# datatypevoid/babble

Hardware: AMD Instinct MI355X
Metric: consensus-ordered events/sec at N=256 peers (1 GPU and 8-GPU batched sims) (higher is better)
Workload: dtype int32

## Files before the change

### babble_amd/_lib.py

```python
from __future__ import annotations

import ctypes as C
import os

import numpy as np

HERE = os.path.dirname(os.path.abspath(__file__))
LIB_PATH = os.path.join(HERE, os.environ.get("HGX_LIB", "libhgx.so"))

_L = None


class HgxError(RuntimeError):

    def __init__(self, code: int, msg: str):
        super().__init__(msg)
        self.code = code
        self.msg = msg


class hgx_error(C.Structure):
    _fields_ = [("code", C.c_int32), ("msg", C.c_char * 252)]


# ... 86 lines not shown
    _sig(L, "hgx_destroy", None, [p])
    _sig(L, "hgx_insert_events", i32, [p, C.POINTER(hgx_events), i64, C.POINTER(C.c_int64), E])
    _sig(L, "hgx_insert_events_device", i32, [p, C.POINTER(hgx_events), i64, C.POINTER(C.c_int64), E])
    _sig(L, "hgx_insert_and_run", i32, [p, C.POINTER(hgx_events), i64, C.POINTER(C.c_int64), E])
    for nm in ("hgx_insert_events32", "hgx_insert_and_run32"):
        _sig(L, nm, i32, [p, C.POINTER(hgx_events32), i64, C.POINTER(C.c_int64), E])
    for nm in ("hgx_insert_events_packed", "hgx_insert_and_run_packed"):
        _sig(L, nm, i32, [p, C.POINTER(hgx_events_packed), i64, C.POINTER(C.c_int64), E])
    _sig(L, "hgx_pack_events32", i32, [C.POINTER(hgx_events32), i64, i64, p, p, p, p, p, p, i64,
                                       C.POINTER(C.c_int64), E])
    _sig(L, "hgx_host_alloc", p, [i64])
    _sig(L, "hgx_host_free", None, [p])
    _sig(L, "hgx_set_participant_keys", i32, [p, p, E])
    for nm in ("hgx_insert_events_verified", "hgx_insert_events_verified_device"):
        _sig(L, nm, i32, [p, C.POINTER(hgx_events), p, p, i64, C.POINTER(C.c_int64), E])
    _sig(L, "hgx_insert_event_bodies", i32, [p, C.POINTER(hgx_event_bodies), i64, p, C.POINTER(C.c_int64), E])
    _sig(L, "hgx_insert_event_bodies_ext", i32, [p, C.POINTER(hgx_event_bodies), p, i64, p, C.POINTER(C.c_int64), E])
    _sig(L, "hgx_event_json_batch", i32, [i32, C.POINTER(hgx_event_bodies), i64, p, i32, p, p, p, i64, p, E])
    _sig(L, "hgx_batch_levels", i32, [p, p, i64, i64, p, C.POINTER(C.c_int32), E])
    _sig(L, "hgx_reset_consensus", i32, [p])
    _sig(L, "hgx_save", i32, [p, C.c_char_p, E])
    _sig(L, "hgx_save_ex", i32, [p, C.c_char_p, p, p, E])
    _sig(L, "hgx_get_event_id", i32, [p, i64, p, E])
    _sig(L, "hgx_get_event_payload", i32, [p, i64, p, i64, C.POINTER(C.c_int64), E])
    _sig(L, "hgx_checksum", u64, [p, i64])
    _sig(L, "hgx_bootstrap", i32, [p, C.c_char_p, E])
    _sig(L, "hgx_clear", i32, [p])
    for nm in ("hgx_divide_rounds", "hgx_decide_fame", "hgx_find_order", "hgx_run_consensus"):
        _sig(L, nm, i32, [p, E])
    _sig(L, "hgx_num_events", i64, [p])
    _sig(L, "hgx_super_majority", i32, [p])
    _sig(L, "hgx_num_undetermined", i64, [p, i32])
    _sig(L, "hgx_undecided_rounds", i32, [p, i32, p, i32])
    _sig(L, "hgx_last_consensus_round", i32, [p, i32, C.POINTER(C.c_int32)])
    _sig(L, "hgx_last_commited_round_events", i32, [p, i32])
    _sig(L, "hgx_consensus_transactions", i64, [p, i32])
    _sig(L, "hgx_pending_loaded_events", i64, [p, i32])
    _sig(L, "hgx_last_round", i32, [p, i32])
    _sig(L, "hgx_round_event_count", i32, [p, i32, i32])
    _sig(L, "hgx_round_witnesses", i32, [p, i32, i32, p, i32])
    _sig(L, "hgx_known", i32, [p, i32, p])
    _sig(L, "hgx_consensus_events_count", i64, [p, i32])
    _sig(L, "hgx_consensus_events", i32, [p, i32, i64, i64, p])
    _sig(L, "hgx_num_blocks", i64, [p, i32])
    _sig(L, "hgx_block_info", i32, [p, i32, i64, p, p, p, p, p, p])
    _sig(L, "hgx_get_block", i32, [p, i32, i32, p, E])
    _sig(L, "hgx_consensus_received", i32, [p, i32, i64, i64, p, p, p])
    _sig(L, "hgx_last_from", i32, [p, i32, p, p, E])
    _sig(L, "hgx_participant_events", i32, [p, i32, i64, p, i64, p, E])
    _sig(L, "hgx_participant_event", i32, [p, i32, i64, p, E])
    _sig(L, "hgx_get_root", i32, [p, i32, p, p, p, p, E])
    _sig(L, "hgx_get_event", i32, [p, i64, p, p, p, p, p, p, p, E])
    _sig(L, "hgx_wire_info", i32, [p, i64, i64, p, p, p])
    _sig(L, "hgx_read_wire_info", i32, [p, i32, i64, i32, i64, p, p, E])
    _sig(L, "hgx_diff_wire", i32, [p, i32, p, i64, p, i64, C.POINTER(C.c_int64), C.POINTER(C.c_int32), E])
    _sig(L, "hgx_get_rounds", i32, [p, i64, i64, p, p, p])
    _sig(L, "hgx_get_received", i32, [p, i64, i64, p, p])
    _sig(L, "hgx_get_coords", i32, [p, i64, p, p])
    for nm in ("hgx_ancestor", "hgx_self_ancestor", "hgx_see", "hgx_strongly_see", "hgx_round", "hgx_witness"):
        _sig(L, nm, i32, [p, i64, i64] if nm not in ("hgx_round", "hgx_witness") else [p, i64])
    _sig(L, "hgx_oldest_self_ancestor_to_see", i64, [p, i64, i64])
    _sig(L, "hgx_block_hash", i32, [i64, i32, p, p, i32, p])
    _sig(L, "hgx_sha256_batch", i32, [i32, p, p, i64, p, p])
    _sig(L, "hgx_sha256_batch_device", i32, [p, p, i64, p, p])
    _sig(L, "hgx_p256_verify_batch", i32, [i32, p, i32, p, p, p, p, i64, p, p])
    _sig(L, "hgx_p256_verify_bench", i32, [i32, p, i32, p, p, p, p, i64, i32, i32, p, C.POINTER(C.c_double)])
    _sig(L, "hgx_sha256_bench", i32, [i32, i64, i32, i32, C.c_uint64, i32, i32, C.POINTER(C.c_double),
                                      C.POINTER(C.c_int64), C.POINTER(C.c_int64), i64, p])
    _sig(L, "hgx_phase_times", i32, [p, p, i32])
    _sig(L, "hgx_kernel_stats", i32, [p, i32, C.c_char_p, i32, C.POINTER(C.c_double), C.POINTER(C.c_int64),
                                      C.POINTER(C.c_double)])
    _sig(L, "hgx_reset_stats", i32, [p])
    _sig(L, "hgx_set_kernel_timing", i32, [p, i32])
    _sig(L, "hgx_set_coord_storage", i32, [p, i32])
    _sig(L, "hgx_set_fame_tally", i32, [p, i32])
    _sig(L, "hgx_set_round_kernel", i32, [p, i32])
    _sig(L, "hgx_set_sort_kernel", i32, [p, i32])
    _sig(L, "hgx_set_round_shards", i32, [p, i32])
    _sig(L, "hgx_set_shard_remote", i32, [p, i32])
    _sig(L, "hgx_exchange_floor_bench", i32, [i32, i32, i32, i32, C.POINTER(C.c_double)])
    _sig(L, "hgx_set_cts_kernel", i32, [p, i32])
    _sig(L, "hgx_set_root_others", i32, [p, p, i64, p])
    _sig(L, "hgx_set_la_kernel", i32, [p, i32])
    _sig(L, "hgx_set_incremental", i32, [p, i32])
    _sig(L, "hgx_find_order_begin", i32, [p, p])
    _sig(L, "hgx_find_order_end", i32, [p, p])
    _sig(L, "hgx_set_shard", i32, [p, i32, i32])
    _sig(L, "hgx_reset", i32, [p, p, p, p, p])
    _sig(L, "hgx_insert_wire_events", i32, [p, p, i64, p, p])
    _sig(L, "hgx_set_commit_callback", i32, [p, C.c_void_p, p])
    _sig(L, "hgx_get_frame", i32, [p, p, i64, p, p, p, p, p, p, p, i64, p, p])
    _sig(L, "hgx_prune_to_frame", i32, [p, p, i64, C.POINTER(C.c_int64), E])
    _sig(L, "hgx_get_root_ids", i32, [p, i32, p, C.POINTER(C.c_int32), p, C.POINTER(C.c_int32), E])
    _sig(L, "hgx_get_root_others", i32, [p, p, p, i64, C.POINTER(C.c_int64), E])
    _sig(L, "hgx_set_root_ids", i32, [p, p, p, p, p, p, p, i64, E])
    _sig(L, "hgx_shard_values", i64, [p, i32])
    _sig(L, "hgx_shard_export", i32, [p, p, i32])
    _sig(L, "hgx_shard_import", i32, [p, i32, p, i32])
    _sig(L, "hgx_reserve_rounds", i32, [p, i32])
    _sig(L, "hgx_device_alloc", i32, [i32, i64, C.POINTER(C.c_void_p)])
    _sig(L, "hgx_device_free", i32, [i32, p])
    _sig(L, "hgx_device_copy", i32, [i32, p, p, i64, i32])
    _L = L
    return L


def check(rc: int, err: hgx_error):
    if rc != 0:
        raise HgxError(int(err.code or rc), err.msg.decode(errors="replace"))
```

### babble_amd/csrc/hgx_api.cpp

```cpp
#include <algorithm>
#include <array>
#include <chrono>
#include <cstdio>
#include <cstring>
#include <mutex>
#include <tuple>
#include <set>
#include <new>
#include <cstdlib>
#include <string>
#include <thread>
#include <vector>

#include "hgx.h"
#include "hgx_bodies.h"
#include "hgx_diff.h"
#include "hgx_engine.h"

namespace {

struct Block {
    int32_t rr;
    int64_t first;
    int32_t nev;
// ... 489 lines not shown
    if (rc) return rc;
    return hgx_find_order(c, err);
}

static bool bad_events32(const hgx_events32* ev, int64_t count) {
    return !ev || count < 0 ||
           (count > 0 && (!ev->creator || !ev->index || !ev->self_parent || !ev->other_parent || !ev->timestamp_ns ||
                          !ev->coin || !ev->sig_s || !ev->ntx));
}

static int32_t insert_events32_one(hgx_ctx* c, const hgx_events32* ev, int64_t count, int64_t* n_inserted, hgx_error* err) {
    if (n_inserted) *n_inserted = 0;
    if (!c || bad_events32(ev, count)) {
        set_err(err, HGX_ERR_INVALID, "hgx_insert_events32: bad arguments");
        return HGX_ERR_INVALID;
    }
    if (c->rooted) {
        set_err(err, HGX_ERR_INVALID, "hgx_insert_events32: a reset context checks Root.Others by event id: use hgx_insert_events");
        return HGX_ERR_INVALID;
    }
    DeviceGuard dg(c);
    hgx::InsertIn in{};
    if (count > 0) {
        hipError_t e = c->eng.stage_host32(ev->creator, ev->index, ev->self_parent, ev->other_parent, ev->timestamp_ns,
                                           ev->coin, ev->sig_s, ev->ntx, count, in);
        if (e != hipSuccess) return dev_err(err, e, "hgx_insert_events32");
    }
    hgx::InsertOut out;
    hipError_t e = c->eng.insert(in, count, out);
    if (e != hipSuccess) return dev_err(err, e, "hgx_insert_events32");
    return finish_insert(c, out, n_inserted, err);
}

int32_t hgx_insert_events32(hgx_ctx* c, const hgx_events32* ev, int64_t count, int64_t* n_inserted, hgx_error* err) {
    if (c && c->grp)
        return on_shards(c, err, [&](hgx_ctx* x, hgx_error* e) {
            return insert_events32_one(x, ev, count, x == c ? n_inserted : nullptr, e);
        });
    return insert_events32_one(c, ev, count, n_inserted, err);
}

static int32_t run_after_split32(hgx_ctx* c, int64_t E0, hgx::InsertOut& out, int64_t* n_inserted, hgx_error* err,
                                 const char* who) {
    hipError_t e;
    struct WaitS {
        hgx::Engine& eng;
        ~WaitS() { (void)eng.payload_wait_S(); }
    } wait_s{c->eng};
    hgx::InsertOut head = out;
    head.graph_loaded.assign(c->g_loaded.begin(), c->g_loaded.end());
    hgx_error ins_err{};
    const int32_t ins_rc = finish_insert(c, head, n_inserted, &ins_err);
    int32_t rc = ins_rc ? ins_rc : hgx_divide_rounds(c, err);
    const bool laid_out = ins_rc == 0 && rc == 0;
    std::vector<uint64_t> loaded;
    e = c->eng.payload_end(E0, out.accepted, laid_out, c->rh.r_lo, loaded);
    if (e != hipSuccess) return dev_err(err, e, who);
    for (int g = 0; g < c->G; g++) {
        const int64_t l = (int64_t)loaded[g];
        c->gs[g].pending_loaded += l - c->g_loaded[g];
        c->g_loaded[g] = l;
    }
    c->mirror_ok = false;
    if (ins_rc) {
        if (err) *err = ins_err;
        return ins_rc;
    }
    if (rc) return rc;
    rc = hgx_decide_fame(c, err);
    if (rc) return rc;
    rc = hgx_find_order(c, err);
    if (rc) return rc;
    e = c->eng.payload_wait_S();
    if (e != hipSuccess) return dev_err(err, e, who);
    return ok(err);
}

int32_t hgx_insert_and_run32(hgx_ctx* c, const hgx_events32* ev, int64_t count, int64_t* n_inserted, hgx_error* err) {
    if (n_inserted) *n_inserted = 0;
    if (!c || bad_events32(ev, count)) {
        set_err(err, HGX_ERR_INVALID, "hgx_insert_and_run32: bad arguments");
        return HGX_ERR_INVALID;
    }
    if (count < 65536 || c->rooted || c->shard_world > 1) {
        int32_t rc = hgx_insert_events32(c, ev, count, n_inserted, err);
        if (rc) return rc;
        return hgx_run_consensus(c, err);
    }
    DeviceGuard dg(c);
    const int64_t E0 = c->eng.E;
    hgx::InsertOut out;
    hipError_t e = c->eng.insert_split_begin32(ev->creator, ev->index, ev->self_parent, ev->other_parent, count, out);
    if (e != hipSuccess) return dev_err(err, e, "hgx_insert_and_run32");
    e = c->eng.payload_begin32(ev->timestamp_ns, ev->coin, ev->sig_s, ev->ntx, out.accepted);
    if (e != hipSuccess) return dev_err(err, e, "hgx_insert_and_run32");
    return run_after_split32(c, E0, out, n_inserted, err, "hgx_insert_and_run32");
}

static bool bad_packed(const hgx_events_packed* ev, int64_t count) {
    if (!ev || count < 0) return true;
    if (count == 0) return false;
    if (!ev->creator || !ev->index || !ev->self_parent_back || !ev->other_parent_back || !ev->timestamp_ns ||
        !ev->coin || !ev->sig_s || !ev->ntx || ev->n_exc < 0 || ev->n_exc > count)
        return true;
    if (ev->n_exc == 0) return false;
    if (!ev->exc_pos || !ev->exc_self_parent || !ev->exc_other_parent) return true;
    std::vector<int64_t> p(ev->exc_pos, ev->exc_pos + ev->n_exc);
    std::sort(p.begin(), p.end());
    return p.front() < 0 || p.back() >= count || std::adjacent_find(p.begin(), p.end()) != p.end();
}

static hgx::Engine::Packed packed_of(const hgx_events_packed* ev) {
    return hgx::Engine::Packed{ev->creator, ev->index, ev->self_parent_back, ev->other_parent_back,
                               ev->n_exc, ev->exc_pos, ev->exc_self_parent, ev->exc_other_parent};
}

static int32_t insert_events_packed_one(hgx_ctx* c, const hgx_events_packed* ev, int64_t count, int64_t* n_inserted,
                                        hgx_error* err) {
    if (n_inserted) *n_inserted = 0;
    if (c->rooted) {
        set_err(err, HGX_ERR_INVALID, "hgx_insert_events_packed: a reset context checks Root.Others by event id: use hgx_insert_events");
        return HGX_ERR_INVALID;
    }
    DeviceGuard dg(c);
    hgx::InsertIn in{};
    if (count > 0) {
        hipError_t e = c->eng.stage_packed(packed_of(ev), count, in, ev->timestamp_ns, ev->coin, ev->sig_s, ev->ntx);
        if (e != hipSuccess) return dev_err(err, e, "hgx_insert_events_packed");
    }
    hgx::InsertOut out;
    hipError_t e = c->eng.insert(in, count, out);
    if (e != hipSuccess) return dev_err(err, e, "hgx_insert_events_packed");
    return finish_insert(c, out, n_inserted, err);
}

int32_t hgx_insert_events_packed(hgx_ctx* c, const hgx_events_packed* ev, int64_t count, int64_t* n_inserted,
                                 hgx_error* err) {
    if (n_inserted) *n_inserted = 0;
    if (!c || bad_packed(ev, count)) {
        set_err(err, HGX_ERR_INVALID, "hgx_insert_events_packed: bad arguments");
        return HGX_ERR_INVALID;
    }
    if (c->grp)
        return on_shards(c, err, [&](hgx_ctx* x, hgx_error* e) {
            return insert_events_packed_one(x, ev, count, x == c ? n_inserted : nullptr, e);
        });
    return insert_events_packed_one(c, ev, count, n_inserted, err);
}

int32_t hgx_insert_and_run_packed(hgx_ctx* c, const hgx_events_packed* ev, int64_t count, int64_t* n_inserted,
                                  hgx_error* err) {
    if (n_inserted) *n_inserted = 0;
    if (!c || bad_packed(ev, count)) {
        set_err(err, HGX_ERR_INVALID, "hgx_insert_and_run_packed: bad arguments");
        return HGX_ERR_INVALID;
    }
    if (count < 65536 || c->rooted || c->shard_world > 1) {
        int32_t rc = hgx_insert_events_packed(c, ev, count, n_inserted, err);
        if (rc) return rc;
        return hgx_run_consensus(c, err);
    }
    DeviceGuard dg(c);
    const int64_t E0 = c->eng.E;
    hgx::InsertOut out;
    hipError_t e = c->eng.insert_split_begin_packed(packed_of(ev), count, out);
    if (e != hipSuccess) return dev_err(err, e, "hgx_insert_and_run_packed");
    e = c->eng.payload_begin32(ev->timestamp_ns, ev->coin, ev->sig_s, ev->ntx, out.accepted);
    if (e != hipSuccess) return dev_err(err, e, "hgx_insert_and_run_packed");
    return run_after_split32(c, E0, out, n_inserted, err, "hgx_insert_and_run_packed");
}

int32_t hgx_pack_events32(const hgx_events32* ev, int64_t count, int64_t base, uint16_t* creator16, uint16_t* sp_back,
                          uint16_t* op_back, int64_t* exc_pos, int32_t* exc_sp, int32_t* exc_op, int64_t exc_cap,
                          int64_t* n_exc, hgx_error* err) {
    if (n_exc) *n_exc = 0;
// ... 1727 lines not shown
            }
            famous[k] = f;
        }
    }
    return HGX_OK;
}

int32_t hgx_get_received(hgx_ctx* c, int64_t first, int64_t count, int32_t* rr, int64_t* cts) {
    if (!c || first < 0 || count < 0 || first + count > c->E) return HGX_ERR_INVALID;
    DeviceGuard dg(c);
    if (ensure_received(c)) return HGX_ERR_DEVICE;
    for (int64_t k = 0; k < count; k++) {
        const size_t x = (size_t)(first + k);
        const bool have = x < c->rr_cache.size();
        if (rr) rr[k] = have ? c->rr_cache[x] : -1;
        if (cts) cts[k] = (have && c->rr_cache[x] >= 0) ? c->cts_cache[x] : 0;
    }
    return HGX_OK;
}

int32_t hgx_get_coords(hgx_ctx* c, int64_t gid, int32_t* la, int32_t* fd) {
    if (!c || gid < 0 || gid >= c->E_div || !c->divided) return HGX_ERR_INVALID;
    DeviceGuard dg(c);
    return c->eng.get_coords(gid, la, fd) == hipSuccess ? HGX_OK : HGX_ERR_DEVICE;
}

static bool known_div(hgx_ctx* c, int64_t x) { return c && x >= 0 && x < c->E_div && c->divided; }
static bool same_graph(hgx_ctx* c, int64_t x, int64_t y) { return graph_of(c, x) == graph_of(c, y); }

int32_t hgx_ancestor(hgx_ctx* c, int64_t x, int64_t y) {
    if (x == y) return 1;
    if (!known_div(c, x) || !known_div(c, y)) return 0;
    DeviceGuard dg(c);
    if (ensure_mirror(c) || !same_graph(c, x, y)) return 0;
    std::vector<int32_t> la(c->n), fd(c->n);
    if (c->eng.get_coords(x, la.data(), fd.data()) != hipSuccess) return 0;
    return la[c->creator[(size_t)y] % c->n] >= c->index32[(size_t)y] ? 1 : 0;
}
int32_t hgx_self_ancestor(hgx_ctx* c, int64_t x, int64_t y) {
    if (x == y) return 1;
    if (!c || x < 0 || y < 0 || x >= c->E || y >= c->E) return 0;
    DeviceGuard dg(c);
    if (ensure_mirror(c)) return 0;
    return (c->creator[(size_t)x] == c->creator[(size_t)y] && c->index32[(size_t)x] >= c->index32[(size_t)y]) ? 1 : 0;
}
int32_t hgx_see(hgx_ctx* c, int64_t x, int64_t y) { return hgx_ancestor(c, x, y); }
int32_t hgx_strongly_see(hgx_ctx* c, int64_t x, int64_t y) {
    if (!known_div(c, x) || !known_div(c, y)) return 0;
    DeviceGuard dg(c);
    if (ensure_mirror(c) || !same_graph(c, x, y)) return 0;
    std::vector<int32_t> lx(c->n), fx(c->n), ly(c->n), fy(c->n);
    if (c->eng.get_coords(x, lx.data(), fx.data()) != hipSuccess) return 0;
    if (c->eng.get_coords(y, ly.data(), fy.data()) != hipSuccess) return 0;
    int cnt = 0;
    for (int i = 0; i < c->n; i++) cnt += lx[i] >= fy[i];
    return cnt >= c->sm ? 1 : 0;
}
int64_t hgx_oldest_self_ancestor_to_see(hgx_ctx* c, int64_t x, int64_t y) {
    if (!known_div(c, x) || !known_div(c, y)) return -1;
    DeviceGuard dg(c);
    if (ensure_chains(c) || !same_graph(c, x, y)) return -1;
    std::vector<int32_t> la(c->n), fd(c->n);
    if (c->eng.get_coords(y, la.data(), fd.data()) != hipSuccess) return -1;
    const int cx = c->creator[(size_t)x];
    const int32_t a = fd[cx % c->n];
    if (a <= c->index32[(size_t)x]) return c->chain_gids[cx][(size_t)(a - c->chain_base[cx])];
    return -1;
}
int32_t hgx_round(hgx_ctx* c, int64_t x) {
    if (!c) return -1;
    DeviceGuard dg(c);
    if (ensure_rounds(c)) return -1;
    return round_of(c, x);
}
int32_t hgx_witness(hgx_ctx* c, int64_t x) {
    if (!c) return 0;
    DeviceGuard dg(c);
    if (ensure_rounds(c) || ensure_mirror(c)) return 0;
    return witness_of(c, x);
}

int32_t hgx_phase_times(hgx_ctx* c, double* out, int32_t cap) {
    if (!c || !out) return 0;
    const int32_t m = std::min<int32_t>(cap, 22);
    double v[22] = {c->eng.phase_ms[0], c->eng.phase_ms[1], c->eng.phase_ms[2], c->eng.phase_ms[3],
                    (double)c->eng.la_sweeps, (double)c->eng.R, (double)c->eng.compact,
                    (double)c->eng.la_rows, c->eng.last_rebuild ? 1.0 : 0.0, (double)c->rh.r_lo,
                    c->eng.la_wave_used ? 1.0 : 0.0, (double)c->eng.la_wave_fallbacks,
                    (double)(c->eng.la_wave_used ? c->eng.la_wave_segs : 0), (double)c->eng.round_p_runs,
                    (double)c->eng.round_p_fallbacks, (double)c->eng.round_p_ovf,
                    (double)c->eng.round_p_fail_round, (double)c->eng.round_p_fail_chain,
                    (double)c->eng.round_g_runs, c->eng.la_small_used ? 1.0 : 0.0,
                    c->eng.la_verified ? 1.0 : 0.0, (double)c->eng.sort_seg_runs};
    for (int32_t i = 0; i < m; i++) out[i] = v[i];
    return m;
}

static const char* kKernelNames[hgx::K_NUM] = {"layout", "la_sweep", "fd_build", "round_gather", "round_search",
                                              "fame", "threshold", "round_received", "cts_median", "order_sort"};

int32_t hgx_kernel_stats(hgx_ctx* c, int32_t k, char* name, int32_t name_cap, double* ms, int64_t* launches,
                         double* bytes) {
    if (!c || k < 0 || k >= hgx::K_NUM) return HGX_ERR_INVALID;
    if (name && name_cap > 0) std::snprintf(name, (size_t)name_cap, "%s", kKernelNames[k]);
    const hgx::KernelStat& ks = c->eng.kstat[k];
    if (ms) *ms = (ks.timed > 0 && ks.timed < ks.launches) ? ks.ms * (double)ks.launches / (double)ks.timed : ks.ms;
    if (launches) *launches = c->eng.kstat[k].launches;
    if (bytes) *bytes = c->eng.kstat[k].bytes;
    return HGX_OK;
}

int32_t hgx_reset_stats(hgx_ctx* c) {
    if (!c) return HGX_ERR_INVALID;
    for (auto& s : c->eng.kstat) s = hgx::KernelStat();
    return HGX_OK;
}

int32_t hgx_set_coord_storage(hgx_ctx* c, int32_t mode) {
    if (!c || mode < 0 || mode > 1) return HGX_ERR_INVALID;
    each_shard(c, [&](hgx_ctx* x) { x->eng.force_coord32 = mode == 1; });
    return HGX_OK;
}

int32_t hgx_set_kernel_timing(hgx_ctx* c, int32_t on) {
    if (!c) return HGX_ERR_INVALID;
    each_shard(c, [&](hgx_ctx* x) { x->eng.time_mask = (uint32_t)on; });
    return HGX_OK;
}

int32_t hgx_set_fame_tally(hgx_ctx* c, int32_t mode) {
    if (!c || mode < 0 || mode > 2) return HGX_ERR_INVALID;
    each_shard(c, [&](hgx_ctx* x) { x->eng.fame_tally = mode; });
    return HGX_OK;
}

int32_t hgx_device_alloc(int32_t device, int64_t bytes, void** ptr) {
    if (!ptr || bytes < 0) return HGX_ERR_INVALID;
    *ptr = nullptr;
    int prev = -1;
    (void)hipGetDevice(&prev);
    if (hipSetDevice(device) != hipSuccess) return HGX_ERR_DEVICE;
    const hipError_t e = hipMalloc(ptr, (size_t)std::max<int64_t>(bytes, 1));
    if (prev >= 0 && prev != device) (void)hipSetDevice(prev);
    return e == hipSuccess ? HGX_OK : HGX_ERR_DEVICE;
}

int32_t hgx_device_free(int32_t device, void* ptr) {
    int prev = -1;
    (void)hipGetDevice(&prev);
    if (hipSetDevice(device) != hipSuccess) return HGX_ERR_DEVICE;
    const hipError_t e = ptr ? hipFree(ptr) : hipSuccess;
    if (prev >= 0 && prev != device) (void)hipSetDevice(prev);
    return e == hipSuccess ? HGX_OK : HGX_ERR_DEVICE;
}

int32_t hgx_device_copy(int32_t device, void* dst, const void* src, int64_t bytes, int32_t to_device) {
    if (bytes < 0 || (bytes > 0 && (!dst || !src))) return HGX_ERR_INVALID;
    int prev = -1;
    (void)hipGetDevice(&prev);
    if (hipSetDevice(device) != hipSuccess) return HGX_ERR_DEVICE;
    const hipError_t e = bytes ? hipMemcpy(dst, src, (size_t)bytes, to_device ? hipMemcpyHostToDevice
                                                                               : hipMemcpyDeviceToHost)
                               : hipSuccess;
    if (prev >= 0 && prev != device) (void)hipSetDevice(prev);
    return e == hipSuccess ? HGX_OK : HGX_ERR_DEVICE;
}

int32_t hgx_set_la_kernel(hgx_ctx* c, int32_t mode) {
    if (!c || mode < 0 || mode > 1026) return HGX_ERR_INVALID;
    each_shard(c, [&](hgx_ctx* x) {
        x->eng.la_kernel = mode == 1 ? 1 : 0;
        x->eng.la_segs_override = (mode >= 2 && mode <= 1024) ? mode : 0;
        x->eng.la_small_override = mode == 1025 ? 0 : -1;
        x->eng.la_verify_always = mode == 1026;
    });
    return HGX_OK;
}

int32_t hgx_set_root_others(hgx_ctx* c, const uint8_t* event_hash32, int64_t count, hgx_error* err) {
    if (!c || count < 0 || (count > 0 && !event_hash32)) {
        set_err(err, HGX_ERR_INVALID, "hgx_set_root_others: bad arguments");
        return HGX_ERR_INVALID;
    }
    if (group_only_one(c, err, "hgx_set_root_others")) return HGX_ERR_INVALID;
    if (!c->rooted && count > 0) {
        set_err(err, HGX_ERR_INVALID, "hgx_set_root_others: no roots installed (hgx_reset)");
        return HGX_ERR_INVALID;
    }
    DeviceGuard dg(c);
    const hipError_t e = c->eng.set_root_others(event_hash32, count);
    if (e != hipSuccess) return dev_err(err, e, "hgx_set_root_others");
    c->others_keys.assign(event_hash32, event_hash32 + (size_t)count * 32);
    return ok(err);
}

int32_t hgx_set_sort_kernel(hgx_ctx* c, int32_t mode) {
    if (!c || mode < 0 || mode > 1) return HGX_ERR_INVALID;
    each_shard(c, [&](hgx_ctx* x) { x->eng.sort_seg_enabled = mode == 0; });
    return HGX_OK;
}

int32_t hgx_set_round_kernel(hgx_ctx* c, int32_t mode) {
    if (!c || mode < 0 || mode > 5) return HGX_ERR_INVALID;
    each_shard(c, [&](hgx_ctx* x) {
        x->eng.round_kernel = mode == 5 ? 0 : mode;
        x->eng.round_pb_enabled = mode != 5;
    });
    return HGX_OK;
}

static int32_t shard_split(int32_t C, int32_t W, int32_t k) {
    return (int32_t)((int64_t)C * k / W);
}

static int32_t setup_group(hgx_ctx* c, int32_t W, const int32_t* devs, hgx_error* err) {
    auto bad = [&](const std::string& why) {
        set_err(err, HGX_ERR_INVALID, "chain-sharded context: " + why);
        return HGX_ERR_INVALID;
    };
    if (W < 1 || W > hgx::kMaxShards) return bad("1 to 8 shards");
    if (c->E != 0) return bad("shards are set up on an empty context (before the first insert)");
    if (W == 1) {
        drop_group(c);
        return ok(err);
    }
    if (c->G != 1) return bad("one graph per context (hgx_create)");
    if (c->rooted) return bad("not after a Reset");
    if (W > c->C || c->n > 256) return bad("at most one shard per chain and n <= 256 (the persistent recurrence)");
    int ndev = 0;
    if (hipGetDeviceCount(&ndev) != hipSuccess) return bad("no HIP device");
    if (devs[0] != c->eng.dev) return bad("shard 0 runs on the context's own device");
    const char* qenv = std::getenv("GPU_MAX_HW_QUEUES");
    const int queues = qenv ? std::max(1, std::atoi(qenv)) : 4;
    for (int k = 0; k < W; k++) {
        if (devs[k] < 0 || devs[k] >= ndev) return bad("invalid device ordinal " + std::to_string(devs[k]));
        int same = 0;
        for (int j = 0; j < W; j++) same += devs[j] == devs[k];
        if (same > 1 && same > queues - 2)
            return bad(std::to_string(same) + " shards on device " + std::to_string(devs[k]) +
                       " need GPU_MAX_HW_QUEUES >= " + std::to_string(same + 2) + " (set before the HIP runtime starts)");
    }
    int prev = -1;
    (void)hipGetDevice(&prev);
    for (int a = 0; a < W; a++)
        for (int b = 0; b < W; b++) {
            if (devs[a] == devs[b]) continue;
            int can = 0;
            if (hipDeviceCanAccessPeer(&can, devs[a], devs[b]) != hipSuccess || !can) {
// ... 117 lines not shown
```

### babble_amd/csrc/hgx_engine.cpp

```cpp
#include "hgx_engine.h"

#include <algorithm>
#include <array>
#include <chrono>
#include <cstdio>
#include <cstdlib>
#include <cstring>
#include <functional>

namespace hgx {

#define HGX_TRY(x)                              \
    do {                                        \
        hipError_t _e = (x);                    \
        if (_e != hipSuccess) return _e;        \
    } while (0)

template <typename T>
hipError_t DBuf<T>::alloc(size_t count) {
    release();
    if (count == 0) count = 1;
    hipError_t e = hipMalloc((void**)&p, count * sizeof(T));
    if (e == hipSuccess) n = count; else p = nullptr;
    return e;
// ... 27 lines not shown
template struct DBuf<uint8_t>;
template struct DBuf<int8_t>;
template struct DBuf<uint32_t>;
template struct DBuf<uint64_t>;
template struct DBuf<unsigned long long>;

static int bitlen(uint64_t v) {
    int b = 0;
    while (v) { b++; v >>= 1; }
    return b;
}

bool ShardGroup::wait() {
    std::unique_lock<std::mutex> lk(m);
    if (broken) return false;
    const uint64_t g = gen;
    if (++count == W) {
        count = 0;
        gen++;
        cv.notify_all();
        return true;
    }
    if (!cv.wait_for(lk, std::chrono::seconds(120), [&] { return gen != g || broken; })) broken = true;
    if (broken) cv.notify_all();
    return !broken;
}

void ShardGroup::fail() {
    std::lock_guard<std::mutex> lk(m);
    broken = true;
    cv.notify_all();
}

void ShardGroup::rearm() {
    std::lock_guard<std::mutex> lk(m);
    broken = false;
    count = 0;
}

hipError_t Engine::share_round_rows(int32_t r_a, int32_t r_b) {
    if (!grp || grp->W < 2) return hipSuccess;
    const int lo = grp->c_split[shard], hi = grp->c_split[shard + 1];
    if (hi <= lo || r_b < r_a) return hipSuccess;
    const int32_t r_s = std::min(r_b, r_cap - 1);
    const size_t Cz = (size_t)C, w = (size_t)(hi - lo);
    for (int k = 0; k < grp->W; k++) {
        if (k == shard) continue;
        Engine* q = grp->eng[k];
        if (q->r_cap != r_cap) return hipErrorInvalidValue;
        HGX_TRY(hipMemcpy2DAsync(q->Bm.p + (size_t)r_a * Cz + lo, Cz * 4, Bm.p + (size_t)r_a * Cz + lo, Cz * 4, w * 4,
                                 (size_t)(r_b - r_a + 1), hipMemcpyDefault, stream));
        if (r_s >= r_a) {
            const size_t rows = (size_t)(r_s - r_a + 1);
            HGX_TRY(hipMemcpy2DAsync(q->Smat.p + ((size_t)r_a * Cz + lo) * nw, Cz * nw * 8, Smat.p + ((size_t)r_a * Cz + lo) * nw,
                                     Cz * nw * 8, w * nw * 8, rows, hipMemcpyDefault, stream));
            HGX_TRY(hipMemcpy2DAsync(q->wstat.p + (size_t)r_a * Cz + lo, Cz, wstat.p + (size_t)r_a * Cz + lo, Cz, w, rows,
                                     hipMemcpyDefault, stream));
            HGX_TRY(hipMemcpy2DAsync(q->wflag.p + (size_t)r_a * Cz + lo, Cz, wflag.p + (size_t)r_a * Cz + lo, Cz, w, rows,
                                     hipMemcpyDefault, stream));
        }
    }
    return hipStreamSynchronize(stream);
}

Engine::~Engine() {
    free_ev_scratch(ev_scratch);
    if (pay_thread.joinable()) pay_thread.join();
    if (stream2) (void)hipStreamSynchronize(stream2);
    if (ev_pay) (void)hipEventDestroy(ev_pay);
    if (stream2) (void)hipStreamDestroy(stream2);
    if (stream) (void)hipStreamSynchronize(stream);
    for (auto e : kev) (void)hipEventDestroy(e);
    if (ph0) (void)hipEventDestroy(ph0);
    if (ph1) (void)hipEventDestroy(ph1);
    if (ph2) (void)hipEventDestroy(ph2);
    if (h_small) (void)hipHostFree(h_small);
    if (h_pack) (void)hipHostFree(h_pack);
    if (h_stage) (void)hipHostFree(h_stage);
    if (h_ins) (void)hipHostFree(h_ins);
    if (h_cpar) (void)hipHostFree(h_cpar);
    if (h_flag) (void)hipHostFree(h_flag);
    if (h_segc) (void)hipHostFree(h_segc);
    if (df_host) (void)hipHostFree(df_host);
    if (stream_o) (void)hipStreamSynchronize(stream_o);
    for (auto e : ev_o)
        if (e) (void)hipEventDestroy(e);
    if (stream_o) (void)hipStreamDestroy(stream_o);
    for (auto e : flag_ev)
        if (e) (void)hipEventDestroy(e);
    for (auto e : la_ev)
        if (e) (void)hipEventDestroy(e);
    drop_step_graph();
    if (stream) (void)hipStreamDestroy(stream);
}

hipError_t Engine::init(int device, int n_graphs, int n_part, int64_t cap_events, std::string& why) {
    int count = 0;
    hipError_t e = hipGetDeviceCount(&count);
    if (e != hipSuccess || count <= 0) {
        why = "no HIP device available (libhgx has no CPU fallback)";
        return e != hipSuccess ? e : hipErrorNoDevice;
    }
    if (device < 0 || device >= count) {
        why = "invalid HIP device ordinal";
        return hipErrorInvalidDevice;
    }
    hipDeviceProp_t prop;
    HGX_TRY(hipGetDeviceProperties(&prop, device));
    num_cus = std::max(1, prop.multiProcessorCount);
    if (std::strncmp(prop.gcnArchName, "gfx950", 6) != 0) {
        why = std::string("device is ") + prop.gcnArchName + ", libhgx is built for gfx950 (MI355X) only";
        return hipErrorInvalidDeviceFunction;
    }
    dev = device;
    HGX_TRY(hipSetDevice(dev));
    HGX_TRY(hipStreamCreateWithFlags(&stream, hipStreamNonBlocking));
    HGX_TRY(hipEventCreate(&ph0));
    HGX_TRY(hipEventCreate(&ph1));
    HGX_TRY(hipEventCreate(&ph2));
    G = n_graphs;
    n = n_part;
    C = G * n;
    sm = 2 * n / 3 + 1;
    shard_lo = 0;
    shard_hi = C;
    nw = (n + 63) / 64;
    cap = std::max<int64_t>(cap_events, 1);
    const size_t P = (size_t)cap;
    Ppos = cap + std::max<int64_t>(cap / 2, (int64_t)256 * C);
    const size_t PP = (size_t)Ppos;
    HGX_TRY(g_creator.alloc(P)); HGX_TRY(g_index.alloc(P)); HGX_TRY(g_sp.alloc(P)); HGX_TRY(g_op.alloc(P));
    HGX_TRY(g_ntx.alloc(P)); HGX_TRY(g_rr.alloc(P)); HGX_TRY(g_pos.alloc(P)); HGX_TRY(g_ts.alloc(P));
    HGX_TRY(g_cts.alloc(P)); HGX_TRY(g_ck.alloc(P)); HGX_TRY(g_S.alloc(P * 32)); HGX_TRY(g_coin.alloc(P)); HGX_TRY(g_loaded.alloc(P));
    HGX_TRY(g_txnil.alloc(P)); HGX_TRY(g_id.alloc(P * 32));
    HGX_TRY(succ.alloc(P)); HGX_TRY(first_none.alloc(C));
    ins_gl_off = ((size_t)3 * C + 1) & ~(size_t)1;
    HGX_TRY(ins_blk.alloc(ins_gl_off + (size_t)2 * G));
    last_gid_d.view(ins_blk.p, C);
    last_index_d.view(ins_blk.p + C, C);
    chain_base_d.view(ins_blk.p + 2 * C, C);
    graph_loaded_d.view((unsigned long long*)(ins_blk.p + ins_gl_off), G);
    HGX_TRY(ins_fail.alloc(1));
    HGX_TRY(hipMemsetAsync(ins_fail.p, 0xFF, 8, stream));
    HGX_TRY(hipHostMalloc((void**)&h_ins, ins_blk.n * sizeof(int32_t), hipHostMallocDefault));
    HGX_TRY(cpar_blk.alloc((size_t)3 * C));
    HGX_TRY(hipHostMalloc((void**)&h_cpar, (size_t)3 * C * sizeof(int32_t), hipHostMallocDefault));
    HGX_TRY(hipMemsetAsync(succ.p, 0xFF, P * 4, stream));
    HGX_TRY(hipMemsetAsync(first_none.p, 0xFF, (size_t)C * 4, stream));
    HGX_TRY(hipMemsetAsync(last_gid_d.p, 0xFF, (size_t)C * 8, stream));
    HGX_TRY(hipMemsetAsync(chain_base_d.p, 0, (ins_blk.n - (size_t)2 * C) * 4, stream));
    HGX_TRY(c_off.alloc(C + 1));
    c_len.view(cpar_blk.p, C);
    c_base.view(cpar_blk.p + C, C);
    c_old.view(cpar_blk.p + 2 * C, C);
    HGX_TRY(fu.alloc(C)); HGX_TRY(rcnt.alloc(C));
    HGX_TRY(root_round_d.alloc(C)); HGX_TRY(root_y_ext_d.alloc(C));
    HGX_TRY(hipMemsetAsync(root_round_d.p, 0xFF, (size_t)C * 4, stream));
    HGX_TRY(hipMemsetAsync(root_y_ext_d.p, 0, (size_t)C, stream));
    HGX_TRY(p_gid.alloc(PP)); HGX_TRY(p_chain.alloc(PP)); HGX_TRY(p_op.alloc(PP)); HGX_TRY(p_opu.alloc(PP));
    HGX_TRY(p_opk.alloc(PP));
    HGX_TRY(p_round.alloc(PP)); HGX_TRY(p_rr.alloc(PP)); HGX_TRY(p_ts.alloc(PP)); HGX_TRY(p_cts.alloc(PP));
    fd_ld = (Ppos + 31) & ~(int64_t)31;
    HGX_TRY(LA.alloc(PP * n));
    HGX_TRY(FDT.alloc((size_t)fd_ld * n + 128));
    HGX_TRY(recv_list.alloc(P)); HGX_TRY(counters.alloc(8 + 4 * kLaRing));
    HGX_TRY(hipMemsetAsync(counters.p, 0, (8 + 4 * kLaRing) * 4, stream)); HGX_TRY(order_gid.alloc(P));
// ... 465 lines not shown
        if (e == hipSuccess) e = hipEventRecord(ev_pay, stream2);
        pay_err_a = e;
        pay_stage.store(1, std::memory_order_release);
        if (c && e == hipSuccess) e = hipMemcpyAsync(S_dst, S, c * 32, hipMemcpyHostToDevice, stream2);
        if (e == hipSuccess) e = hipEventRecord(ev_pay_S, stream2);
        if (e == hipSuccess) e = hipStreamSynchronize(stream2);
        pay_err = e;
    });
    return hipSuccess;
}

hipError_t Engine::payload_begin(const int64_t* ts, const uint8_t* hash, const uint8_t* S, const int32_t* ntx,
                                 const int32_t* nil, int64_t m_ok) {
    if (!stream2) {
        HGX_TRY(hipStreamCreateWithFlags(&stream2, hipStreamNonBlocking));
        HGX_TRY(hipEventCreateWithFlags(&ev_pay, hipEventDisableTiming));
    }
    const size_t c = (size_t)m_ok;
    if (st_ts.n < c) HGX_TRY(st_ts.alloc(c));
    if (st_hash.n < 32 * c) HGX_TRY(st_hash.alloc(32 * c));
    if (st_S.n < 32 * c) HGX_TRY(st_S.alloc(32 * c));
    if (st_ntx.n < c) HGX_TRY(st_ntx.alloc(c));
    if (st_nil.n < c) HGX_TRY(st_nil.alloc(c));
    if (pay_thread.joinable()) pay_thread.join();
    pay_err = hipSuccess;
    pay32 = false;
    pay_S_pending = false;
    pay_thread = std::thread([=]() {
        hipError_t e = hipSetDevice(dev);
        if (c && e == hipSuccess) e = hipMemcpyAsync(st_ts.p, ts, c * 8, hipMemcpyHostToDevice, stream2);
        if (c && e == hipSuccess) e = hipMemcpyAsync(st_hash.p, hash, c * 32, hipMemcpyHostToDevice, stream2);
        if (c && e == hipSuccess) e = hipMemcpyAsync(st_S.p, S, c * 32, hipMemcpyHostToDevice, stream2);
        if (c && e == hipSuccess) e = hipMemcpyAsync(st_ntx.p, ntx, c * 4, hipMemcpyHostToDevice, stream2);
        if (c && e == hipSuccess) e = hipMemcpyAsync(st_nil.p, nil, c * 4, hipMemcpyHostToDevice, stream2);
        if (e == hipSuccess) e = hipEventRecord(ev_pay, stream2);
        if (e == hipSuccess) e = hipStreamSynchronize(stream2);
        pay_err = e;
    });
    return hipSuccess;
}

hipError_t Engine::payload_end(int64_t E0, int64_t m_ok, bool laid_out_new, int32_t wcoin_r0,
                               std::vector<uint64_t>& loaded) {
    if (pay_S_pending) {
        while (pay_stage.load(std::memory_order_acquire) == 0) std::this_thread::yield();
        HGX_TRY(pay_err_a);
    } else {
        if (pay_thread.joinable()) pay_thread.join();
        HGX_TRY(pay_err);
    }
    HGX_TRY(hipStreamWaitEvent(stream, ev_pay, 0));
    InsertIn in{};
    in.creator = st_creator.p; in.ts = st_ts.p; in.S = pay_S_pending ? nullptr : st_S.p; in.ntx = st_ntx.p;
    if (split32) { in.index32 = st_index32.p; in.sp32 = st_sp32.p; in.op32 = st_op32.p; }
    else { in.index = st_index.p; in.sp = st_sp.p; in.op = st_op.p; }
    if (pay32) in.coin = st_coin.p;
    else { in.hash = st_hash.p; in.nil = st_nil.p; }
    split32 = false;
    launch_insert_commit(stream, m_ok, nullptr, nullptr, E0, n, in, insert_state(), kCommitPayload);
    if (laid_out_new) {
        launch_ts_to_pos(stream, E0, m_ok, g_pos.p, g_ts.p, p_ts.p);
        if (R > wcoin_r0) launch_wcoin(stream, arrays(), wcoin_r0, R, C);
    }
    HGX_TRY(hipGetLastError());
    HGX_TRY(hipMemcpyAsync(h_ins, ins_blk.p, ins_blk.n * sizeof(int32_t), hipMemcpyDeviceToHost, stream));
    HGX_TRY(hipStreamSynchronize(stream));
    loaded.resize(G);
    std::memcpy(loaded.data(), h_ins + ins_gl_off, (size_t)G * 8);
    return hipSuccess;
}

hipError_t Engine::payload_wait_S() {
    if (!pay_S_pending) return hipSuccess;
    pay_S_pending = false;
    if (pay_thread.joinable()) pay_thread.join();
    HGX_TRY(pay_err);
    return hipStreamWaitEvent(stream, ev_pay_S, 0);
}

hipError_t Engine::insert_impl(const InsertIn& in, int64_t count, InsertOut& out, const unsigned long long* fail_sig,
                               int commit_mode) {
    out = InsertOut();
    const int64_t E0 = E;
    InsertState st = insert_state();
    if (count > 0) {
        if (!launch_insert_fused(stream, count, fail_sig, E0, cap, C, n, in, st, commit_mode)) {
            launch_insert_claim(stream, count, E0, cap, C, in, st);
            launch_insert_check(stream, count, E0, cap, C, n, in, st);
            launch_insert_commit(stream, count, ins_fail.p, fail_sig, E0, n, in, st, commit_mode);
            launch_insert_unclaim(stream, count, ins_fail.p, fail_sig, E0, cap, C, in, st);
        }
        HGX_TRY(copy_to_pinned(h_small, ins_fail.p, 8, 0xFF));
        if (fail_sig) HGX_TRY(copy_to_pinned(h_small + 2, fail_sig, 8));
    }
    out.last_gid.resize(C);
    out.last_index.resize(C);
    out.chain_base.resize(C);
    out.graph_loaded.resize(G);
    HGX_TRY(copy_to_pinned(h_ins, ins_blk.p, ins_blk.n * sizeof(int32_t)));
    HGX_TRY(stage_issue());
    HGX_TRY(hipStreamSynchronize(stream));
    if (count > 0) {
        unsigned long long fail = 0, fsig = ~0ull;
        std::memcpy(&fail, h_small, 8);
        if (fail_sig) std::memcpy(&fsig, h_small + 2, 8);
        if ((fsig >> 8) <= (fail >> 8) && fsig != ~0ull) fail = fsig;
        const int64_t m_ok = (fail == ~0ull) ? count : (int64_t)(fail >> 8);
        out.accepted = m_ok;
        out.code = (fail == ~0ull) ? 0 : (int)(fail & 0xFF);
        if (out.code) {
            HGX_TRY(hipMemcpyAsync(&out.fail_creator, in.creator + m_ok, 4, hipMemcpyDeviceToHost, stream));
            if (in.index32) {
                int32_t fi = 0;
                HGX_TRY(hipMemcpyAsync(&fi, in.index32 + m_ok, 4, hipMemcpyDeviceToHost, stream));
                HGX_TRY(hipStreamSynchronize(stream));
                out.fail_index = fi;
            } else {
                HGX_TRY(hipMemcpyAsync(&out.fail_index, in.index + m_ok, 8, hipMemcpyDeviceToHost, stream));
            }
            HGX_TRY(hipStreamSynchronize(stream));
        }
        E = E0 + m_ok;
    }
    std::memcpy(out.last_gid.data(), h_ins, (size_t)C * 4);
    std::memcpy(out.last_index.data(), h_ins + C, (size_t)C * 4);
    std::memcpy(out.chain_base.data(), h_ins + 2 * C, (size_t)C * 4);
    std::memcpy(out.graph_loaded.data(), h_ins + ins_gl_off, (size_t)G * 8);
    return hipSuccess;
}

hipError_t Engine::clear() {
    HGX_TRY(payload_wait_S());
    if (E > 0) HGX_TRY(hipMemsetAsync(succ.p, 0xFF, (size_t)E * 4, stream));
    HGX_TRY(hipMemsetAsync(first_none.p, 0xFF, (size_t)C * 4, stream));
    HGX_TRY(hipMemsetAsync(last_gid_d.p, 0xFF, (size_t)C * 8, stream));
    HGX_TRY(hipMemsetAsync(chain_base_d.p, 0, (ins_blk.n - (size_t)2 * C) * 4, stream));
    E = 0;
    E_div = 0;
    R = 0;
    laid_out = false;
    ids_known = true;
    return hipStreamSynchronize(stream);
}

hipError_t Engine::prune_stage(const std::vector<int32_t>& cut, int64_t n_kept, PruneOut& out) {
    out = PruneOut();
    pr_count = -1;
    if ((int)cut.size() != C || n_kept < 0 || n_kept > E || !ids_known) return hipErrorInvalidValue;
    HGX_TRY(payload_wait_S());
    const size_t Ez = (size_t)E, K = (size_t)std::max<int64_t>(n_kept, 1), Cz = (size_t)C;
    const size_t nparts = (Ez + 2047) / 2048 + 1;
    size_t total = 0;
    auto take = [&](size_t bytes) {
        const size_t off = total;
        total += (bytes + 255) & ~(size_t)255;
        return off;
    };
    const size_t o_scan = take(Ez * 4), o_part = take(nparts * 4), o_cut = take(Cz * 4), o_first = take(Cz * 4),
                 o_cnt = take(8), o_cr = take(K * 4), o_idx = take(K * 4), o_sp = take(K * 4), o_op = take(K * 4),
                 o_ntx = take(K * 4), o_old = take(K * 4), o_ts = take(K * 8), o_hash = take(K * 32),
                 o_S = take(K * 32), o_on = take(K * 4), o_oo = take(K * 4), o_ok = take(K * 32),
                 o_opid = take(K * 32), o_rsp = take(Cz * 4), o_rop = take(Cz * 4), o_rid = take(Cz * 96);
    if (pr_buf.n < total) HGX_TRY(pr_buf.alloc(total));
    uint8_t* b = pr_buf.p;
    PruneArgs a{};
    a.E = E; a.n_kept = n_kept; a.C = C;
    a.g_creator = g_creator.p; a.g_index = g_index.p; a.g_sp = g_sp.p; a.g_op = g_op.p; a.g_ntx = g_ntx.p;
    a.g_ts = g_ts.p; a.g_S = g_S.p; a.g_id = g_id.p; a.g_txnil = g_txnil.p;
    a.cut = (const int32_t*)(b + o_cut); a.scan = (uint32_t*)(b + o_scan); a.first_gid = (int32_t*)(b + o_first);
    a.kept_total = (uint32_t*)(b + o_cnt); a.oth_count = (uint32_t*)(b + o_cnt) + 1;
    a.st_creator = (int32_t*)(b + o_cr); a.st_index = (int32_t*)(b + o_idx); a.st_sp = (int32_t*)(b + o_sp);
    a.st_op = (int32_t*)(b + o_op); a.st_ntx = (int32_t*)(b + o_ntx); a.old_gid = (int32_t*)(b + o_old);
    a.st_ts = (int64_t*)(b + o_ts); a.st_hash = b + o_hash; a.st_S = b + o_S;
    a.oth_new = (int32_t*)(b + o_on); a.oth_op = (int32_t*)(b + o_oo); a.oth_key = b + o_ok; a.oth_pid = b + o_opid;
    a.root_sp = (int32_t*)(b + o_rsp); a.root_op = (int32_t*)(b + o_rop); a.root_ids = b + o_rid;
    out.old_gid.resize((size_t)n_kept);
    out.root_sp.resize(Cz);
    out.root_op.resize(Cz);
    out.root_ids.resize(Cz * 96);
    HGX_TRY(hipMemcpyAsync(b + o_cut, cut.data(), Cz * 4, hipMemcpyHostToDevice, stream));
    HGX_TRY(hipMemsetAsync(b + o_first, 0xFF, Cz * 4, stream));
    HGX_TRY(hipMemsetAsync(b + o_cnt, 0, 8, stream));
    launch_prune(stream, a, (uint32_t*)(b + o_part));
    HGX_TRY(hipGetLastError());
    uint32_t cnt[2] = {0, 0};
    HGX_TRY(hipMemcpyAsync(cnt, b + o_cnt, 8, hipMemcpyDeviceToHost, stream));
    if (n_kept) HGX_TRY(hipMemcpyAsync(out.old_gid.data(), a.old_gid, (size_t)n_kept * 4, hipMemcpyDeviceToHost, stream));
    HGX_TRY(hipMemcpyAsync(out.root_sp.data(), a.root_sp, Cz * 4, hipMemcpyDeviceToHost, stream));
    HGX_TRY(hipMemcpyAsync(out.root_op.data(), a.root_op, Cz * 4, hipMemcpyDeviceToHost, stream));
    HGX_TRY(hipMemcpyAsync(out.root_ids.data(), a.root_ids, Cz * 96, hipMemcpyDeviceToHost, stream));
    HGX_TRY(hipStreamSynchronize(stream));
    if ((int64_t)cnt[0] != n_kept || (int64_t)cnt[1] > n_kept) return hipErrorInvalidValue;
    const size_t no = cnt[1];
    out.n_others = (int64_t)no;
    out.oth_new.resize(no);
    out.oth_op.resize(no);
    out.oth_key.resize(no * 32);
    out.oth_pid.resize(no * 32);
    if (no) {
        HGX_TRY(hipMemcpyAsync(out.oth_new.data(), a.oth_new, no * 4, hipMemcpyDeviceToHost, stream));
        HGX_TRY(hipMemcpyAsync(out.oth_op.data(), a.oth_op, no * 4, hipMemcpyDeviceToHost, stream));
        HGX_TRY(hipMemcpyAsync(out.oth_key.data(), a.oth_key, no * 32, hipMemcpyDeviceToHost, stream));
        HGX_TRY(hipMemcpyAsync(out.oth_pid.data(), a.oth_pid, no * 32, hipMemcpyDeviceToHost, stream));
        HGX_TRY(hipStreamSynchronize(stream));
    }
    pr_in = InsertIn{};
    pr_in.creator = a.st_creator; pr_in.index32 = a.st_index; pr_in.sp32 = a.st_sp; pr_in.op32 = a.st_op;
    pr_in.ts = a.st_ts; pr_in.hash = a.st_hash; pr_in.S = a.st_S; pr_in.ntx = a.st_ntx;
    pr_count = n_kept;
    return hipSuccess;
}

hipError_t Engine::prune_to_frame(const std::vector<int32_t>& root_round, const std::vector<uint8_t>& y_ext,
                                  const PruneOut& st, InsertOut& out) {
    if (pr_count < 0) return hipErrorInvalidValue;
    const int64_t count = pr_count;
    pr_count = -1;
    HGX_TRY(clear());
    HGX_TRY(set_roots(root_round, y_ext));
    HGX_TRY(set_root_others(st.oth_key.data(), st.n_others));
    return insert(pr_in, count, out);
}

hipError_t Engine::diff_wire(int graph, const int32_t* known, const int32_t* root_index, int64_t rows, int64_t expect,
                             const DiffCols& out, int64_t* dev_total) {
// ... 180 lines not shown
    S.resize(e * 32);
    coin.resize(e);
    ntx.resize(e);
    txnil.resize(e);
    if (e == 0) return hipSuccess;
    HGX_TRY(hipMemcpyAsync(ts.data(), g_ts.p, e * 8, hipMemcpyDeviceToHost, stream));
    HGX_TRY(hipMemcpyAsync(S.data(), g_S.p, e * 32, hipMemcpyDeviceToHost, stream));
    HGX_TRY(hipMemcpyAsync(coin.data(), g_coin.p, e, hipMemcpyDeviceToHost, stream));
    HGX_TRY(hipMemcpyAsync(ntx.data(), g_ntx.p, e * 4, hipMemcpyDeviceToHost, stream));
    HGX_TRY(hipMemcpyAsync(txnil.data(), g_txnil.p, e, hipMemcpyDeviceToHost, stream));
    return hipStreamSynchronize(stream);
}

hipError_t Engine::get_event_fields(int64_t gid, int64_t* ts, int32_t* ntx, int32_t* tx_nil) {
    uint8_t nil = 0;
    HGX_TRY(hipMemcpyAsync(ts, g_ts.p + gid, 8, hipMemcpyDeviceToHost, stream));
    HGX_TRY(hipMemcpyAsync(ntx, g_ntx.p + gid, 4, hipMemcpyDeviceToHost, stream));
    HGX_TRY(hipMemcpyAsync(&nil, g_txnil.p + gid, 1, hipMemcpyDeviceToHost, stream));
    HGX_TRY(hipStreamSynchronize(stream));
    *tx_nil = nil;
    return hipSuccess;
}

hipError_t Engine::reserve_rounds(int32_t rounds) {
    rounds = std::max<int32_t>(rounds, 1);
    drop_step_graph();
    Bm.release(); WLA.release(); WFD.release(); wflag.release(); wstat.release(); wcoin.release();
    active.release(); Tthr.release(); fw.release(); elig.release(); ur_empty.release(); Smat.release();
    Vbuf.release(); fame.release(); blk_cnt.release(); blk_loaded.release(); blk_ntx.release(); blk_nil.release();
    ovf.release();
    WLAT.release();
    r_cap = 0;
    R = 0;
    E_div = 0;
    HGX_TRY(ensure_round_cap(rounds));
    return hipStreamSynchronize(stream);
}

hipError_t Engine::capture_steps(StepGraph& sgr, const RoundArgs& args, int kern, int nb) {
    sgr.drop();
    sgr.args = args;
    sgr.kernel = kern;
    sgr.compact = compact;
    sgr.nb = nb;
    HGX_TRY(hipStreamBeginCapture(stream, hipStreamCaptureModeThreadLocal));
    hipError_t le = hipSuccess;
    for (int k = 0; k < nb && le == hipSuccess; k++) le = launch_round_step(stream, sgr.args, k, kern);
    const hipError_t ce = hipStreamEndCapture(stream, &sgr.graph);
    if (le != hipSuccess) {
        if (ce == hipSuccess && sgr.graph) (void)hipGraphDestroy(sgr.graph);
        sgr.graph = nullptr;
        return le;
    }
    HGX_TRY(ce);
    HGX_TRY(hipGraphInstantiate(&sgr.exec, sgr.graph, nullptr, nullptr, 0));
    size_t nn = 0;
    HGX_TRY(hipGraphGetNodes(sgr.graph, nullptr, &nn));
    std::vector<hipGraphNode_t> nodes(nn);
    HGX_TRY(hipGraphGetNodes(sgr.graph, nodes.data(), &nn));
    sgr.nodes.clear();
    sgr.params.clear();
    hipGraphNode_t nd_cur = nullptr;
    for (auto nd : nodes) {
        size_t nd_deps = 0;
        HGX_TRY(hipGraphNodeGetDependencies(nd, nullptr, &nd_deps));
        if (nd_deps == 0) nd_cur = nd;
    }
    while (nd_cur) {
        hipKernelNodeParams kp;
        HGX_TRY(hipGraphKernelNodeGetParams(nd_cur, &kp));
        sgr.nodes.push_back(nd_cur);
        sgr.params.push_back(kp);
        size_t nd_out = 0;
        HGX_TRY(hipGraphNodeGetDependentNodes(nd_cur, nullptr, &nd_out));
        if (nd_out == 0) break;
        std::vector<hipGraphNode_t> outs(nd_out);
        HGX_TRY(hipGraphNodeGetDependentNodes(nd_cur, outs.data(), &nd_out));
        nd_cur = outs[0];
    }
    if ((int)sgr.nodes.size() != nb) return hipErrorUnknown;
    return hipSuccess;
}

hipError_t Engine::divide_rounds(int64_t En, const std::vector<int32_t>& chain_len,
                                 const std::vector<int32_t>& chain_base, RoundsHost& out) {
    stage_out.clear();
    pend.clear();
    stage_used = 0;
    int32_t max_index = -1;
    int new_max_len = 0;
    for (int c = 0; c < C; c++) {
        if (chain_len[c] > 0) max_index = std::max(max_index, chain_base[c] + chain_len[c] - 1);
        new_max_len = std::max(new_max_len, chain_len[c]);
    }
    const int new_compact = (!force_coord32 && (n % 2) == 0 && max_index <= 65533) ? 1 : 0;
    bool rebuild = !laid_out || E_div == 0 || new_compact != compact || !incremental;
    if (!rebuild)
        for (int c = 0; c < C; c++)
            if (chain_len[c] > h_off[c + 1] - h_off[c]) { rebuild = true; break; }
    const int64_t E0 = rebuild ? 0 : E_div;
    E = En;
    compact = new_compact;
    max_len = new_max_len;
    const size_t csz = compact ? 2 : 4;
    if (rebuild) {
        int act = 0;
        for (int c = 0; c < C; c++) act += chain_len[c] > 0 ? 1 : 0;
        const int64_t share = (Ppos - En) / (2 * (int64_t)act + (C - act));
        h_off.assign(C + 1, 0);
        for (int c = 0; c < C; c++)
            h_off[c + 1] = h_off[c] + ((chain_len[c] + (int32_t)((chain_len[c] > 0 ? 2 : 1) * share)) & ~31);
        HGX_TRY(hipMemcpyAsync(c_off.p, h_off.data(), (C + 1) * 4, hipMemcpyHostToDevice, stream));
        h_len_div.assign(C, 0);
        last_rebuild = true;
    } else {
        last_rebuild = false;
    }
    std::memcpy(h_cpar, chain_len.data(), (size_t)C * 4);
    std::memcpy(h_cpar + C, chain_base.data(), (size_t)C * 4);
    std::memcpy(h_cpar + 2 * C, h_len_div.data(), (size_t)C * 4);
    HGX_TRY(copy_from_pinned(cpar_blk.p, h_cpar, (size_t)3 * C * 4));
    HGX_TRY(stage_issue());
    int32_t r_lo = 0;
    if (!rebuild) {
        r_lo = 0x7FFFFFFF;
        const int32_t Rp = out.R;
        for (int c = 0; c < C && r_lo > 0; c++) {
            if (chain_len[c] <= h_len_div[c]) continue;
            const int32_t last = h_len_div[c] - 1;
            if (last < 0 || Rp == 0) { r_lo = 0; break; }
            int32_t lo = 0, hi = Rp;
            while (lo < hi) {
                const int32_t mid = (lo + hi + 1) / 2;
                if (out.bm[(size_t)mid * C + c] <= last) lo = mid; else hi = mid - 1;
            }
            r_lo = std::min(r_lo, lo);
        }
        if (r_lo == 0x7FFFFFFF) r_lo = 0;
    }
    int max_new = 0;
    for (int c = 0; c < C; c++) max_new = std::max(max_new, chain_len[c] - h_len_div[c]);
    DevArrays a = arrays();
    HGX_TRY(hipEventRecord(ph0, stream));
    const int seg = kLaSeg;
    kbeg(K_LAYOUT);
    launch_layout(stream, E0, En, a, C, n, seg);
    kend(K_LAYOUT, (double)(En - E0) * 64);
    const size_t nunits = (size_t)((max_len + seg - 1) / seg) * C;
    int64_t u0 = 0;
    int la_na = n;
    const int32_t* la_map = nullptr;
    if (n > 896 && G == 1) {
        h_lmap.clear();
        for (int c = 0; c < C; c++)
            if (chain_len[c] > 0) h_lmap.push_back(c);
        la_na = (int)h_lmap.size();
        if (la_na <= 896) {
            if (la_lmap.n < (size_t)std::max(1, la_na)) HGX_TRY(la_lmap.alloc((size_t)n));
            HGX_TRY(hipMemcpyAsync(la_lmap.p, h_lmap.data(), (size_t)la_na * 4, hipMemcpyHostToDevice, stream));
            la_map = la_lmap.p;
        }
    }
    la_wave_used = la_kernel == 0 && la_wave_ok(n, max_len, la_na) && (n <= 896 || la_map);
    la_wave_segs = 1;
    if (la_wave_used && rebuild && G == 1 && En >= (int64_t)kLaSegMinRows * C) {
        const int cap = (int)std::max<int64_t>(kLaMaxSegs, En / C / (2 * kLaHeadRows));
        la_wave_segs = la_segs_override > 0 ? la_segs_override : la_wave_segments(n, compact, num_cus, cap);
    }
    if (rebuild) {
        if (!la_wave_used) HGX_TRY(hipMemsetAsync(LA.p, compact ? 0x00 : 0xFF, (size_t)h_off[C] * n * csz, stream));
    } else {
        launch_init_new(stream, a, E0, En - E0, n, fd_ld);
        int32_t smin = 0x7FFFFFFF;
        for (int c = 0; c < C; c++)
            if (chain_len[c] > h_len_div[c]) smin = std::min(smin, h_len_div[c] / seg);
        u0 = (int64_t)smin * C;
    }
    if (la_chg.n < nunits) {
        const size_t old = la_chg.n;
        HGX_TRY(la_chg.grow_copy(std::max(nunits, 2 * la_chg.n), old, stream));
        HGX_TRY(hipMemsetAsync(la_chg.p + old, 0, (la_chg.n - old) * 4, stream));
    }
    if (la_usum.n < nunits) HGX_TRY(la_usum.grow_copy(std::max(nunits, 2 * la_usum.n), la_usum.n, stream));
    const int32_t* cold = rebuild ? nullptr : c_old.p;
    la_sweeps = 0;
    la_rows = 0;
    auto run_sweeps = [&](int first_mode) -> hipError_t {
        int launched_s = 0;
        HGX_TRY(hipMemsetAsync(counters.p + 8, 0, 16, stream));
        auto launch_sweep = [&]() -> hipError_t {
            const int slot = launched_s % kLaRing;
            int32_t* cnt = counters.p + 8 + 4 * slot;
            int32_t* cnt_next = counters.p + 8 + 4 * ((launched_s + 1) % kLaRing);
            kbeg(K_LA_SWEEP);
            launch_la_sweep(stream, a, C, n, max_len, seg, launched_s == 0 ? first_mode : 0, la_chg.p, ++la_stamp,
                            la_usum.p, cnt, cnt_next, cold, u0);
            kend(K_LA_SWEEP, 0);
            HGX_TRY(hipMemcpyAsync(h_small + 16 + 4 * slot, cnt, 8, hipMemcpyDeviceToHost, stream));
            HGX_TRY(hipEventRecord(la_ev[slot], stream));
            launched_s++;
            return hipSuccess;
        };
        for (;;) {
            const int ahead = (first_mode == 2 && la_sweeps == 0) ? 1 : kLaAhead;
            while (launched_s < la_sweeps + ahead) HGX_TRY(launch_sweep());
            const int slot = la_sweeps % kLaRing;
            HGX_TRY(hipEventSynchronize(la_ev[slot]));
            const int32_t rows = h_small[16 + 4 * slot], changed = h_small[16 + 4 * slot + 1];
            la_rows += rows;
            kadd_bytes(K_LA_SWEEP, (double)rows * (3.0 * csz * n + 16));
            la_sweeps++;
            if (changed == 0) break;
            if (la_sweeps > 100000) return hipErrorUnknown;
        }
        return hipSuccess;
    };
    if (la_wave_used) {
        kbeg(K_LA_SWEEP);
        int64_t gpos = 0;
        for (int g = 0; g < G && la_wave_segs == 1 && !la_map; g++) {
            int64_t e = 0;
            for (int c = 0; c < n; c++) e += chain_len[(size_t)g * n + c];
            gpos = std::max(gpos, e);
        }
        const size_t small_lds = (la_wave_segs == 1 && !la_map && la_small_override != 0) ? la_small_bytes(n, compact, gpos) : 0;
        la_small_used = small_lds > 0;
        if (la_small_used) HGX_TRY(launch_la_small(stream, a, G, n, cold, small_lds, counters.p + 6));
        else
            HGX_TRY(launch_la_wave(stream, a, G, n, cold, En, la_wave_segs, 0, counters.p + 6, la_map, la_na,
                                   !rebuild && (En - E0) <= 8 * (int64_t)C));
        if (la_wave_segs > 1)
            HGX_TRY(launch_la_wave(stream, a, G, n, nullptr, En, la_wave_segs, kLaHeadRows, counters.p + 6, la_map, la_na));
        const double rows = (double)(En - E0);
        kend(K_LA_SWEEP, rows * (3.0 * csz * n + 16));
        if (rebuild) {
            HGX_TRY(hipMemcpyAsync(h_small + 48, counters.p + 6, 4, hipMemcpyDeviceToHost, stream));
            HGX_TRY(hipMemsetAsync(counters.p + 6, 0, 4, stream));
        }
        if (la_wave_segs > 1) {
            const size_t nt = (size_t)(la_wave_segs + 1) * n;
            if (la_chk.n < nt + 1) HGX_TRY(la_chk.alloc(nt + 1));
            HGX_TRY(hipMemsetAsync(la_chk.p, 0, 4, stream));
            HGX_TRY(launch_la_seg_check(stream, a, n, En, la_wave_segs, kLaHeadRows, la_chk.p + 1, la_chk.p));
            HGX_TRY(hipMemcpyAsync(h_small + 50, la_chk.p, 4, hipMemcpyDeviceToHost, stream));
            HGX_TRY(hipStreamSynchronize(stream));
            la_verified = h_small[50] != 0 || la_verify_always;
            if (la_verified) HGX_TRY(run_sweeps(2));
        }
        la_sweeps++;
        la_rows += (int64_t)rows;
    } else {
        HGX_TRY(run_sweeps(1));
    }
    kbeg(K_FD_BUILD);
    if (grp) {
        launch_fd_build(stream, a, C, n, max_len, fd_ld, cold, max_new, grp->c_split[shard], grp->c_split[shard + 1]);
    } else {
        launch_fd_build(stream, a, C, n, max_len, fd_ld, cold, max_new);
    }
    kend(K_FD_BUILD, (double)(En - E0) * 2.0 * csz * n);
    if (rooted) {
        if (gfl.n < (size_t)Ppos) HGX_TRY(gfl.alloc((size_t)Ppos));
        const size_t need = (size_t)(root_gmax + 1) * C;
        if (gB.n < need) {
            HGX_TRY(gB.alloc(need));
            drop_step_graph();
        }
        launch_root_floor(stream, a, root_round_d.p, gfl.p, gB.p, root_gmax, C, n, max_len);
    }
    if (rebuild) {
        HGX_TRY(hipMemsetAsync(fu.p, 0, (size_t)C * 4, stream));
        launch_fu_count(stream, a, En);
        h_fu.assign(C, 0);
        HGX_TRY(hipMemcpyAsync(h_fu.data(), fu.p, (size_t)C * 4, hipMemcpyDeviceToHost, stream));
    }
    const bool one_trip = !rebuild;
    if (one_trip) {
        HGX_TRY(hipEventRecord(ph2, stream));
    } else {
        HGX_TRY(hipEventRecord(ph1, stream));
        HGX_TRY(hipEventSynchronize(ph1));
        if (la_wave_used && h_small[48] != 0) {
            la_wave_used = false;
            la_wave_fallbacks++;
            HGX_TRY(hipMemsetAsync(LA.p, compact ? 0x00 : 0xFF, (size_t)h_off[C] * n * csz, stream));
            HGX_TRY(run_sweeps(1));
            launch_fd_build(stream, a, C, n, max_len, fd_ld, cold, max_new);
            if (rooted) launch_root_floor(stream, a, root_round_d.p, gfl.p, gB.p, root_gmax, C, n, max_len);
            HGX_TRY(hipEventRecord(ph1, stream));
            HGX_TRY(hipEventSynchronize(ph1));
        }
        float ms = 0;
        HGX_TRY(hipEventElapsedTime(&ms, ph0, ph1));
        phase_ms[0] = ms;
    }
    h_len_div = chain_len;
    E_div = En;
    laid_out = true;

    if (!one_trip) HGX_TRY(hipEventRecord(ph0, stream));
    HGX_TRY(ensure_round_cap(r_lo + 2 * kStepBatch + 2));
    a = arrays();
    {
        FillRange fr[4] = {{lr.p, (uint32_t)((size_t)G * 4), 0xFF},
                           {active.p + r_lo, (uint32_t)((size_t)(r_cap + 1 - r_lo) * 4), 0},
                           {ovf.p + r_lo, (uint32_t)((size_t)(r_cap + 2 - r_lo) * 4), 0},
                           {Bm.p, (uint32_t)((size_t)C * 4), 0}};
        launch_fill_many(stream, fr, r_lo == 0 ? 4 : 3);
        HGX_TRY(hipGetLastError());
    }
    {
// ... 660 lines not shown
```

### babble_amd/csrc/hgx_engine.h

```cpp
#pragma once

#include <hip/hip_runtime.h>

#include <cstdint>
#include <string>
#include <atomic>
#include <condition_variable>
#include <mutex>
#include <thread>
#include <vector>

#include "hgx_kernels.h"

namespace hgx {


constexpr int kStepBatch = 16;
constexpr int kStepBatchSmall = 2;

struct StepGraph {
    hipGraph_t graph = nullptr;
    hipGraphExec_t exec = nullptr;
    std::vector<hipGraphNode_t> nodes;
    std::vector<hipKernelNodeParams> params;
// ... 83 lines not shown
    bool broken = false;
};

class Engine {
   public:
    ~Engine();
    hipError_t init(int device, int n_graphs, int n_part, int64_t cap_events, std::string& why);

    hipError_t insert(const InsertIn& in, int64_t count, InsertOut& out);
    hipError_t insert_verified(const InsertIn& in, const uint8_t* digest, const uint8_t* r, int64_t count,
                               InsertOut& out);
    hipError_t stage_sig(const uint8_t* digest, const uint8_t* r, int64_t count, const uint8_t** d_digest,
                         const uint8_t** d_r);
    hipError_t insert_bodies(const BodiesIn& ev, const std::vector<int64_t>& txi, int64_t count, const uint8_t* op_id32,
                             uint8_t* out_id32, InsertOut& out);
    EvScratch* ev_scratch = nullptr;
    hipError_t set_root_ids(const uint8_t* x_id32, const uint8_t* has_x, const uint8_t* y_id32, const uint8_t* has_y,
                            const uint8_t* pairs64, int64_t n_pairs);
    bool root_ids_set = false;
    DBuf<uint8_t> root_tab_d;
    DBuf<uint64_t> root_pairs_d;
    int64_t n_root_pairs = 0;
    hipError_t set_keys(const uint8_t* keys65);
    bool keys_set = false;
    hipError_t stage_host(const int32_t* creator, const int64_t* index, const int64_t* sp, const int64_t* op,
                          const int64_t* ts, const uint8_t* hash, const uint8_t* S, const int32_t* ntx,
                          const int32_t* nil, int64_t count, InsertIn& in);
    hipError_t insert_split_begin(const int32_t* creator, const int64_t* index, const int64_t* sp, const int64_t* op,
                                  int64_t count, InsertOut& out);
    hipError_t payload_begin(const int64_t* ts, const uint8_t* hash, const uint8_t* S, const int32_t* ntx,
                             const int32_t* nil, int64_t m_ok);
    hipError_t payload_end(int64_t E0, int64_t m_ok, bool laid_out_new, int32_t wcoin_r0, std::vector<uint64_t>& loaded);
    hipError_t payload_wait_S();
    hipError_t stage_host32(const int32_t* creator, const int32_t* index, const int32_t* sp, const int32_t* op,
                            const int64_t* ts, const uint8_t* coin, const uint8_t* S, const int32_t* ntx, int64_t count,
                            InsertIn& in);
    hipError_t insert_split_begin32(const int32_t* creator, const int32_t* index, const int32_t* sp, const int32_t* op,
                                    int64_t count, InsertOut& out);
    hipError_t payload_begin32(const int64_t* ts, const uint8_t* coin, const uint8_t* S, const int32_t* ntx, int64_t m_ok);
    struct Packed {
        const uint16_t* creator;
        const int32_t* index;
        const uint16_t* spb;
        const uint16_t* opb;
        int64_t n_exc;
        const int64_t* exc_pos;
        const int32_t* exc_sp;
        const int32_t* exc_op;
    };
    hipError_t stage_packed(const Packed& pk, int64_t count, InsertIn& in, const int64_t* ts = nullptr,
                            const uint8_t* coin = nullptr, const uint8_t* S = nullptr, const int32_t* ntx = nullptr);
    hipError_t insert_split_begin_packed(const Packed& pk, int64_t count, InsertOut& out);
    hipError_t clear();
    struct PruneOut {
        std::vector<int32_t> old_gid;
        std::vector<int32_t> root_sp, root_op;
        std::vector<uint8_t> root_ids;
        int64_t n_others = 0;
        std::vector<int32_t> oth_new, oth_op;
        std::vector<uint8_t> oth_key, oth_pid;
    };
    hipError_t prune_stage(const std::vector<int32_t>& cut, int64_t n_kept, PruneOut& out);
    hipError_t prune_to_frame(const std::vector<int32_t>& root_round, const std::vector<uint8_t>& y_ext,
                              const PruneOut& st, InsertOut& out);
    struct DiffCols {
        int64_t *gid, *index, *spi, *opi, *ts;
        int32_t *creator, *opc, *ntx, *nil;
        uint8_t *hash, *S, *root;
    };
    hipError_t diff_wire(int graph, const int32_t* known, const int32_t* root_index, int64_t rows, int64_t expect,
                         const DiffCols& out, int64_t* dev_total);
    int32_t len_div(int chain) const { return laid_out && chain < (int)h_len_div.size() ? h_len_div[(size_t)chain] : 0; }
    hipError_t get_events(std::vector<int32_t>& creator, std::vector<int32_t>& index, std::vector<int32_t>& sp,
                          std::vector<int32_t>& op);
    hipError_t get_event_fields(int64_t gid, int64_t* ts, int32_t* ntx, int32_t* tx_nil);
    bool ids_known = true;
    hipError_t get_ids(int64_t first, int64_t count, uint8_t* out32);
    hipError_t get_keys(uint8_t* out65);
    hipError_t get_columns(std::vector<int32_t>& creator, std::vector<int32_t>& index, std::vector<int32_t>& sp,
                           std::vector<int32_t>& op, std::vector<int64_t>& ts, std::vector<uint8_t>& S,
                           std::vector<uint8_t>& coin, std::vector<int32_t>& ntx, std::vector<uint8_t>& txnil);
    hipError_t divide_rounds(int64_t E, const std::vector<int32_t>& chain_len,
                             const std::vector<int32_t>& chain_base, RoundsHost& out);
    hipError_t decide_fame(int32_t r0, std::vector<int8_t>& fame_out);
    hipError_t find_order(const std::vector<uint8_t>& elig, const std::vector<uint8_t>& famous,
                          const std::vector<uint8_t>& ur_empty, int32_t r0, int max_unrecv, OrderHost& out);
    int32_t recv_round_lo(const RoundsHost& rh, int& max_unrecv) const;
    hipError_t find_order_begin(const std::vector<uint8_t>& elig, const std::vector<uint8_t>& famous,
                                const std::vector<uint8_t>& ur_empty, int32_t r0, int max_unrecv, OrderHost& out);
    hipError_t find_order_end(OrderHost& out, int32_t* order_dst = nullptr);
    int64_t shard_values(int lo, int hi) const;
    hipError_t shard_copy(int lo, int hi, void* buf, bool on_device, bool to_buf);
    int shard_lo = 0, shard_hi = 0;
    hipError_t set_roots(const std::vector<int32_t>& round, const std::vector<uint8_t>& y_ext);
    hipError_t set_root_others(const uint8_t* keys32, int64_t count);
    bool others_trust = false;
    bool rooted = false;
    int root_gmax = -1;
    hipError_t round_first_gids(int32_t r0, std::vector<int32_t>& out);
    hipError_t copy_order(int32_t* dst, int64_t first, int64_t count);
    hipError_t sync() { return hipStreamSynchronize(stream); }

    hipError_t reset_received();
    hipError_t reserve_rounds(int32_t rounds);
    hipError_t get_rounds(std::vector<int32_t>& round_by_gid);
    hipError_t get_received(std::vector<int32_t>& rr, std::vector<int64_t>& cts);
    hipError_t get_coords(int64_t gid, int32_t* la, int32_t* fd);

    int n = 0, G = 0, C = 0, sm = 0, nw = 1;
    int64_t cap = 0, E = 0, E_div = 0;
    int64_t Ppos = 0;
    bool incremental = true;
    bool last_rebuild = false;
    int32_t R = 0;
    int la_sweeps = 0;
    int la_kernel = 0;
    bool la_wave_used = false;
    int la_wave_segs = 1;
    int la_segs_override = 0;
    int num_cus = 256;
    static constexpr int kLaMaxSegs = 16;
    static constexpr int kLaHeadRows = 64;
    static constexpr int kLaSegMinRows = 512;
    int64_t la_wave_fallbacks = 0;
    bool la_verified = false;
    bool la_verify_always = false;
    int compact = 0;
    bool force_coord32 = false;
    int64_t la_rows = 0;
    static constexpr int kLaSeg = 16;
    hipStream_t stream = nullptr;
    double phase_ms[4] = {0, 0, 0, 0};
    KernelStat kstat[K_NUM];
    uint32_t time_mask = 0;
    int fame_tally = 0;
    int round_kernel = 0;
    int cts_kernel = 1;
    int64_t round_g_runs = 0;
    ShardGroup* grp = nullptr;
    int shard = 0;
    hipError_t share_round_rows(int32_t r_a, int32_t r_b);
    hipError_t capture_steps(StepGraph& sgr, const RoundArgs& args, int kern, int nb);
    bool la_small_used = false;
    int la_small_override = -1;
    bool sort_seg_enabled = true;
    int64_t sort_seg_runs = 0;
    bool round_pb_enabled = true;
    int64_t round_p_runs = 0, round_p_fallbacks = 0;
    int64_t round_p_ovf = 0;
    int32_t round_p_fail_round = -1, round_p_fail_chain = -1;
    int dev = 0;

   private:
    hipError_t ensure_round_cap(int32_t need);
    hipError_t insert_impl(const InsertIn& in, int64_t count, InsertOut& out, const unsigned long long* fail_sig,
                           int commit_mode = kCommitAll);
    hipStream_t stream2 = nullptr;
    bool pay32 = false;
    bool split32 = false;
    hipEvent_t ev_pay = nullptr;
    hipEvent_t ev_pay_S = nullptr;
    std::atomic<int> pay_stage{0};
    bool pay_S_pending = false;
    std::thread pay_thread;
    hipError_t pay_err = hipSuccess;
    hipError_t pay_err_a = hipSuccess;
    InsertState insert_state();
    void kbeg(int k, bool sample = true, int64_t count = 1);
    void kend(int k, double bytes);
    void kadd_bytes(int k, double bytes);
    hipError_t collect_kernel_times();
    DevArrays arrays();

    int max_len = 0;
    bool laid_out = false;
    std::vector<int32_t> h_off;
    std::vector<int32_t> h_len_div;
    std::vector<int32_t> h_fu;
    int32_t fo_m = 0;
    std::vector<int32_t> fo_cnt;
    DBuf<int32_t> root_round_d, gfl, gB, rfirst;
    DBuf<uint8_t> root_y_ext_d;
    DBuf<uint64_t> others_d;
    int64_t n_others = 0;
    DBuf<int32_t> sh_off;
    DBuf<int64_t> sh_buf;
    DBuf<int32_t> g_creator, g_index, g_sp, g_op, g_ntx, g_rr, g_pos;
    DBuf<int64_t> g_ts, g_cts, g_ck;
    DBuf<uint8_t> g_S, g_coin, g_loaded, g_txnil, g_id;
    DBuf<uint32_t> succ, first_none;
    DBuf<int32_t> ins_blk, cpar_blk;
    int32_t* h_ins = nullptr;
    int32_t* h_cpar = nullptr;
    size_t ins_gl_off = 0;
    DBuf<int32_t> last_gid_d, last_index_d, chain_base_d;
    DBuf<unsigned long long> ins_fail, graph_loaded_d;
    DBuf<int32_t> st_creator, st_ntx, st_nil;
    DBuf<int64_t> st_index, st_sp, st_op, st_ts;
    DBuf<uint8_t> st_hash, st_S, st_dig, st_r;
    DBuf<int32_t> st_index32, st_sp32, st_op32;
    DBuf<uint16_t> st_c16, st_spb, st_opb;
    DBuf<int64_t> st_exc_pos;
    DBuf<int32_t> st_exc_sp, st_exc_op;
    DBuf<uint8_t> st_coin;
    DBuf<uint8_t> pr_buf;
    InsertIn pr_in{};
    int64_t pr_count = -1;
    DBuf<uint8_t> df_buf;
    uint8_t* df_host = nullptr;
    size_t df_host_cap = 0;
    static constexpr int64_t kPackEvents = 65536;
    hipError_t stage_pinned(int k, const void* const* src, const size_t* bytes, size_t* off);
    DBuf<uint8_t> st_pack;
    uint8_t* h_pack = nullptr;
    size_t h_pack_cap = 0;
    DBuf<uint8_t> pk_keys, pk_valid, pk_out;
    DBuf<uint32_t> pk_tab;
    DBuf<unsigned long long> ins_fail_sig;
    DBuf<int32_t> c_off, c_len, c_base, c_old, fu, rcnt;
    DBuf<int32_t> p_gid, p_chain, p_op, p_opu, p_opk, p_round, p_rr;
    DBuf<int32_t> la_chg;
    int32_t la_stamp = 1;
    DBuf<int64_t> la_usum;
    DBuf<int64_t> p_ts, p_cts;
    DBuf<int32_t> LA, FDT;
    int64_t fd_ld = 0;
    int32_t r_cap = 0;
    DBuf<int32_t> Bm, WLA, WFD, WLAT, Tthr, active, lr;
    hipEvent_t flag_ev[2] = {nullptr, nullptr};
    static constexpr int kLaRing = 8, kLaAhead = 3;
    hipEvent_t la_ev[kLaRing] = {};
    StepGraph step_g[3];
    void drop_step_graph();
    DBuf<uint8_t> wflag, wstat, wcoin, elig, fw, ur_empty;
    DBuf<uint64_t> Smat, Vbuf;
    DBuf<uint32_t> FD8;
    DBuf<uint32_t> FD8p;
    DBuf<uint64_t> rp_gran;
    DBuf<int32_t> rp_st;
    DBuf<uint32_t> seg_off, seg_cur;
// ... 58 lines not shown
```

### babble_amd/csrc/hgx_insert.hip

```cpp
#include <hip/hip_runtime.h>

#include <cstdint>

#include "hgx_device.h"
#include "hgx_kernels.h"

namespace hgx {

constexpr uint32_t kNone32 = 0xFFFFFFFFu;

__device__ __forceinline__ void ins_claim(int64_t k, int64_t E0, int64_t cap, int C, const InsertIn& in,
                                          const InsertState& st) {
    const int64_t gid = E0 + k;
    const int cr = in.creator[k];
    const int64_t sp = in.sp_at(k);
    if (sp == -1) {
        if (cr >= 0 && cr < C) atomicMin(&st.first_none[cr], (uint32_t)gid);
    } else if (sp >= 0 && sp < gid && sp < cap) {
        atomicMin(&st.succ[sp], (uint32_t)gid);
    }
}

__global__ void __launch_bounds__(256) k_insert_claim(int64_t m, int64_t E0, int64_t cap, int C, InsertIn in,
                                                      InsertState st) {
// ... 176 lines not shown
    const int64_t sp = in.sp_at(k);
    if (sp == -1) {
        if (cr >= 0 && cr < C && st.first_none[cr] == (uint32_t)gid) st.first_none[cr] = kNone32;
    } else if (sp >= 0 && sp < gid && sp < cap) {
        if (st.succ[sp] == (uint32_t)gid) st.succ[sp] = kNone32;
    }
}

__global__ void __launch_bounds__(256) k_insert_unclaim(int64_t m, const unsigned long long* fail,
                                                        const unsigned long long* fail_sig, int64_t E0, int64_t cap,
                                                        int C, InsertIn in, InsertState st) {
    const int64_t k = (int64_t)blockIdx.x * blockDim.x + threadIdx.x;
    if (k < m && k >= accepted_prefix(m, fail, fail_sig)) ins_unclaim(k, E0, cap, C, in, st);
}

constexpr int kInsertFusedMax = 1024;
__global__ void __launch_bounds__(kInsertFusedMax) k_insert_fused(int64_t m, const unsigned long long* fail_sig,
                                                                  int64_t E0, int64_t cap, int C, int n, InsertIn in,
                                                                  InsertState st, int mode) {
    const int64_t k = threadIdx.x;
    if (k < m) ins_claim(k, E0, cap, C, in, st);
    asm volatile("s_waitcnt vmcnt(0)" ::: "memory");
    __syncthreads();
    if (k < m) ins_check(k, E0, cap, C, n, in, st);
    asm volatile("s_waitcnt vmcnt(0)" ::: "memory");
    __syncthreads();
    ins_commit(m, st.fail, fail_sig, E0, n, in, st, mode, 0, blockDim.x);
    __syncthreads();
    if (k < m && k >= accepted_prefix(m, st.fail, fail_sig)) ins_unclaim(k, E0, cap, C, in, st);
}

bool launch_insert_fused(hipStream_t s, int64_t m, const unsigned long long* fail_sig, int64_t E0, int64_t cap, int C,
                         int n, const InsertIn& in, const InsertState& st, int mode) {
    if (m <= 0 || m > kInsertFusedMax) return false;
    const unsigned thr = (unsigned)((m + 63) / 64 * 64);
    hipLaunchKernelGGL(k_insert_fused, dim3(1), dim3(thr), 0, s, m, fail_sig, E0, cap, C, n, in, st, mode);
    return true;
}

static inline unsigned nblocks(int64_t work) { return (unsigned)((work + 255) / 256); }

void launch_insert_claim(hipStream_t s, int64_t m, int64_t E0, int64_t cap, int C, const InsertIn& in,
                         const InsertState& st) {
    if (m > 0) hipLaunchKernelGGL(k_insert_claim, dim3(nblocks(m)), dim3(256), 0, s, m, E0, cap, C, in, st);
}

void launch_insert_check(hipStream_t s, int64_t m, int64_t E0, int64_t cap, int C, int n, const InsertIn& in,
                         const InsertState& st) {
    if (m > 0) hipLaunchKernelGGL(k_insert_check, dim3(nblocks(m)), dim3(256), 0, s, m, E0, cap, C, n, in, st);
}

void launch_insert_commit(hipStream_t s, int64_t m, const unsigned long long* fail, const unsigned long long* fail_sig,
                          int64_t E0, int n, const InsertIn& in, const InsertState& st, int mode) {
    const unsigned grid = nblocks(m) < 4096u ? nblocks(m) : 4096u;
    if (m > 0)
        hipLaunchKernelGGL(k_insert_commit, dim3(grid), dim3(256), 0, s, m, fail, fail_sig, E0, n, in, st, mode);
}

__global__ void __launch_bounds__(256) k_insert_sig_first(int64_t m, int C, const int32_t* __restrict__ creator,
                                                          const uint8_t* __restrict__ vout,
                                                          unsigned long long* __restrict__ fail) {
    const int64_t k = (int64_t)blockIdx.x * blockDim.x + threadIdx.x;
    unsigned long long w = ~0ull;
    if (k < m) {
        const int cr = creator[k];
        const uint8_t v = vout[k];
        if (cr >= 0 && cr < C && v != 1) w = ((unsigned long long)k << 8) | (v == 2 ? INS_BAD_KEY : INS_BAD_SIG);
    }
    w = wave_min_u64(w);
    if (lane_id() == 0 && w != ~0ull) atomicMin(fail, w);
}

void launch_insert_sig_first(hipStream_t s, int64_t m, int C, const int32_t* creator, const uint8_t* vout,
                             unsigned long long* fail) {
    if (m > 0) hipLaunchKernelGGL(k_insert_sig_first, dim3(nblocks(m)), dim3(256), 0, s, m, C, creator, vout, fail);
}

void launch_insert_unclaim(hipStream_t s, int64_t m, const unsigned long long* fail, const unsigned long long* fail_sig,
                           int64_t E0, int64_t cap, int C, const InsertIn& in, const InsertState& st) {
    if (m > 0)
        hipLaunchKernelGGL(k_insert_unclaim, dim3(nblocks(m)), dim3(256), 0, s, m, fail, fail_sig, E0, cap, C, in, st);
}

constexpr int kEscape = 0xFFFF;
constexpr int kUnknownParent = -2;

__device__ __forceinline__ int32_t unpack_parent(uint32_t d, int64_t gid) {
    return d == 0 ? -1
         : (d == (uint32_t)kEscape || (int64_t)d > gid) ? kUnknownParent
         : (int32_t)(gid - (int64_t)d);
}

__global__ void __launch_bounds__(256) k_unpack_packed(int64_t m, int64_t E0, const uint16_t* __restrict__ c16,
                                                       const uint16_t* __restrict__ spb,
                                                       const uint16_t* __restrict__ opb, int32_t* __restrict__ cr,
                                                       int32_t* __restrict__ sp, int32_t* __restrict__ op) {
    const int64_t pairs = (m + 1) / 2;
    for (int64_t t = (int64_t)blockIdx.x * blockDim.x + threadIdx.x; t < pairs; t += (int64_t)gridDim.x * blockDim.x) {
        const int64_t k = 2 * t;
        if (k + 1 < m) {
            const uint32_t c = *(const uint32_t*)(c16 + k), s = *(const uint32_t*)(spb + k),
                           o = *(const uint32_t*)(opb + k);
            const int64_t g = E0 + k;
            *(int2*)(cr + k) = make_int2((int)(c & 0xFFFF), (int)(c >> 16));
            *(int2*)(sp + k) = make_int2(unpack_parent(s & 0xFFFF, g), unpack_parent(s >> 16, g + 1));
            *(int2*)(op + k) = make_int2(unpack_parent(o & 0xFFFF, g), unpack_parent(o >> 16, g + 1));
        } else {
            cr[k] = c16[k];
            sp[k] = unpack_parent(spb[k], E0 + k);
            op[k] = unpack_parent(opb[k], E0 + k);
        }
    }
}

__global__ void __launch_bounds__(256) k_unpack_exc(int64_t n_exc, const int64_t* __restrict__ pos,
                                                    const int32_t* __restrict__ esp, const int32_t* __restrict__ eop,
                                                    int32_t* __restrict__ sp, int32_t* __restrict__ op) {
    const int64_t j = (int64_t)blockIdx.x * blockDim.x + threadIdx.x;
    if (j < n_exc) {
        sp[pos[j]] = esp[j];
        op[pos[j]] = eop[j];
    }
}

void launch_unpack_packed(hipStream_t s, int64_t m, int64_t E0, const uint16_t* c16, const uint16_t* spb,
                          const uint16_t* opb, int64_t n_exc, const int64_t* exc_pos, const int32_t* exc_sp,
                          const int32_t* exc_op, int32_t* cr, int32_t* sp, int32_t* op) {
    if (m <= 0) return;
    const int64_t pairs = (m + 1) / 2;
    const unsigned grid = nblocks(pairs) < 8192u ? nblocks(pairs) : 8192u;
    hipLaunchKernelGGL(k_unpack_packed, dim3(grid), dim3(256), 0, s, m, E0, c16, spb, opb, cr, sp, op);
    if (n_exc > 0)
        hipLaunchKernelGGL(k_unpack_exc, dim3(nblocks(n_exc)), dim3(256), 0, s, n_exc, exc_pos, exc_sp, exc_op, sp, op);
}

}
```

### babble_amd/csrc/hgx_kernels.h

```cpp
#pragma once

#include <hip/hip_runtime.h>

#include <cstdint>
#include <functional>
#include <vector>

namespace hgx {

constexpr int32_t kMaxI32 = 2147483647;
constexpr int32_t kWlatNotFamous = -2147483647 - 1;
constexpr int kOpkBits = 21;

struct DevArrays {
    const int32_t *g_creator, *g_index, *g_op, *g_ntx;
    const int64_t* g_ts;
    const uint8_t *g_S, *g_coin, *g_loaded, *g_txnil;
    int32_t *g_rr, *g_pos;
    int64_t* g_ck;
    int64_t* g_cts;
    const int32_t *c_off, *c_len, *c_base;
    int32_t *p_gid, *p_chain, *p_op, *p_opu, *p_round, *p_rr;
    int32_t* p_opk;
    int64_t *p_ts, *p_cts;
// ... 18 lines not shown
    int32_t* order_gid;
    int32_t *blk_cnt, *blk_loaded;
    int64_t* blk_ntx;
    uint8_t* blk_nil;
};

struct InsertIn {
    const int32_t* creator;
    const int64_t *index, *sp, *op, *ts;
    const uint8_t *hash, *S;
    const int32_t *ntx, *nil;
    const int32_t *index32 = nullptr, *sp32 = nullptr, *op32 = nullptr;
    const uint8_t* coin = nullptr;
    __host__ __device__ int64_t idx_at(int64_t k) const { return index32 ? (int64_t)index32[k] : index[k]; }
    __host__ __device__ int64_t sp_at(int64_t k) const { return sp32 ? (int64_t)sp32[k] : sp[k]; }
    __host__ __device__ int64_t op_at(int64_t k) const { return op32 ? (int64_t)op32[k] : op[k]; }
    __host__ __device__ int coin_at(int64_t k) const { return coin ? (coin[k] != 0) : (hash[32 * k + 16] != 0); }
    __host__ __device__ int ntx_at(int64_t k) const { return nil ? ntx[k] : (ntx[k] < 0 ? 0 : ntx[k]); }
    __host__ __device__ int nil_at(int64_t k) const { return nil ? (nil[k] ? 1 : 0) : (ntx[k] < 0 ? 1 : 0); }
};

struct InsertState {
    int32_t *g_creator, *g_index, *g_sp, *g_op, *g_ntx, *g_rr;
    int64_t *g_ts, *g_cts;
    uint8_t *g_S, *g_coin, *g_loaded, *g_txnil;
    uint8_t* g_id;
    uint32_t* succ;
    uint32_t* first_none;
    int32_t *last_gid, *last_index, *chain_base;
    unsigned long long* fail;
    unsigned long long* graph_loaded;
    const uint8_t* root_y_ext;
    int rooted;
    const uint64_t* others;
    int64_t n_others;
    int others_trust;
};

constexpr int64_t kRootY = -3, kRootOther = -4;

enum InsertCode {
    INS_OK = 0, INS_KEY_NOT_FOUND = 1, INS_SELF_PARENT = 2, INS_OTHER_PARENT = 3, INS_CAPACITY = 4,
    INS_PASSED_INDEX = 5, INS_SKIPPED_INDEX = 6, INS_INDEX_RANGE = 7,
    INS_BAD_SIG = 8, INS_BAD_KEY = 9
};

struct RoundArgs {
    int n, C, sm, nw;
    int64_t Pcap;
    const int32_t *c_len, *c_off, *c_base, *p_gid;
    uint32_t* FD8;
    int32_t* ovf;
    const void *LA, *FDT;
    int compact;
    const uint8_t* g_coin;
    int32_t *Bm, *WLA, *WFD, *p_round, *active, *lr;
    uint8_t *wflag, *wstat, *wcoin;
    uint64_t* Smat;
    const int32_t* gB;
    int gmax;
    int32_t* hflag;
};

hipError_t ensure_lds_limit(const void* f, size_t bytes);
hipError_t blocks_per_cu(const void* f, int T, size_t lds, int* out);

struct FillRange {
    void* p;
    uint32_t bytes;
    uint8_t value;
};
constexpr int kFillMax = 8;
void launch_fill_many(hipStream_t s, const FillRange* r, int count);
struct CopyRange {
    const void* src;
    void* dst;
    uint32_t bytes;
    int reset = -1;
};
constexpr int kCopyMax = 8;
void launch_copy_many(hipStream_t s, const CopyRange* r, int count);

int fd_tile_rows(int n, int compact);
void launch_layout(hipStream_t s, int64_t E0, int64_t E, const DevArrays& a, int C, int n, int seg);
bool la_wave_ok(int n, int max_len, int n_active);
size_t la_small_bytes(int n, int compact, int64_t P);
hipError_t launch_la_small(hipStream_t s, const DevArrays& a, int G, int n, const int32_t* c_old, size_t lds,
                           int32_t* err);
int la_wave_blocks(int n, int compact);
int la_wave_segments(int n, int compact, int num_cus, int max_segs);
hipError_t launch_la_seg_check(hipStream_t s, const DevArrays& a, int n, int64_t E, int nts, int head, int32_t* tbl,
                               int32_t* flag);
hipError_t launch_la_wave(hipStream_t s, const DevArrays& a, int G, int n, const int32_t* c_old, int64_t E, int nts,
                          int head, int32_t* err, const int32_t* lmap = nullptr, int na = 0,
                          bool narrow = false);
void launch_la_sweep(hipStream_t s, const DevArrays& a, int C, int n, int max_len, int seg, int first, int32_t* chg,
                     int32_t stamp, int64_t* usum, int32_t* out, int32_t* out_next, const int32_t* c_old, int64_t u0);
void launch_fd_build(hipStream_t s, const DevArrays& a, int C, int n, int max_len, int64_t P, const int32_t* c_old,
                     int max_new, int d_lo = 0, int d_hi = -1);
void launch_init_new(hipStream_t s, const DevArrays& a, int64_t E0, int64_t m, int n, int64_t P);
void launch_round_gather(hipStream_t s, const DevArrays& a, int r, int C, int n, int64_t P);
void launch_wcoin(hipStream_t s, const DevArrays& a, int r0, int R, int C);
hipError_t launch_round_step(hipStream_t s, const RoundArgs& A, int r, int block_search);
hipError_t launch_round_k(hipStream_t s, const RoundArgs& A, int r);
void launch_round_k_gather(hipStream_t s, const RoundArgs& A, int r);
int round_k_ndw(int n);
bool round_p_ok(int n, int C, int num_cus);
bool round_g_ok(int n, int nw);
hipError_t launch_round_g(hipStream_t s, const RoundArgs& A, int32_t* status, int32_t* fin, int r0, int r_end);
constexpr int kRoundPBufs = 4;
constexpr int kRoundPShift = 2;
constexpr int kMaxShards = 8;
struct RoundPWindows {
    int nwin = 0;
    uint32_t remote = 0;
    uint32_t* FD8p[kMaxShards] = {};
    uint64_t* gran[kMaxShards] = {};
    int32_t* st[kMaxShards] = {};
    const void* FDT[kMaxShards] = {};
    int32_t c_split[kMaxShards + 1] = {};
};
hipError_t launch_xchg_floor(hipStream_t s, int C, int n, int rounds, uint32_t* rows, uint64_t* gran, int32_t* st);
hipError_t launch_round_p(hipStream_t s, const RoundArgs& A, uint32_t* FD8p, uint64_t* gran, int32_t* status,
                          int32_t* fin, int r0, int r_end, int init, int num_cus, int c_lo = 0, int c_hi = -1,
                          const RoundPWindows* win_dev = nullptr, int nwin = 1);
void launch_round_p_tail(hipStream_t s, const RoundArgs& A, const int32_t* fin, int r_last);
void launch_round_p_post(hipStream_t s, const RoundArgs& A, int r_lo, int r_hi);
bool round_pb_ok(int n, int G);
hipError_t launch_round_pb(hipStream_t s, const RoundArgs& A, uint32_t* FD8p, uint64_t* gran, int32_t* status,
                           int32_t* fin, const int32_t* amap, int na, int r0, int r_end, int num_cus, bool init);
void launch_round_pb_silent(hipStream_t s, const RoundArgs& A, int r_lo, int r_hi);
void launch_root_floor(hipStream_t s, const DevArrays& a, const int32_t* root_round, int32_t* gfl, int32_t* gB,
                       int gmax, int C, int n, int max_len);
void launch_round_first_gid(hipStream_t s, const DevArrays& a, int r0, int R, int C, int32_t* first);
void launch_last_round(hipStream_t s, int rs, int R, int G, int C, int n, const uint8_t* wstat, int32_t* lr);
void step_prof_dump();
void round_k_prof_dump();
void round_p_prof_dump();
void round_pb_prof_dump();
void round_g_prof_dump();
void launch_fame(hipStream_t s, const DevArrays& a, int r0, int R, int C, int n, int nw, int sm, int G, int tally);
void launch_wla_transpose(hipStream_t s, const DevArrays& a, int r0, int R, int G, int C, int n);
void launch_threshold(hipStream_t s, const DevArrays& a, int r0, int R, int C, int n);
void launch_round_received(hipStream_t s, const DevArrays& a, int R, int C, int n, int max_unrecv);
void launch_fu_advance(hipStream_t s, const DevArrays& a, int C);
void launch_fu_count(hipStream_t s, const DevArrays& a, int64_t E);
void launch_cts(hipStream_t s, const DevArrays& a, int c_lo, int c_cnt, int C, int n, int64_t P, int max_cnt);
bool cts_pipe_ok(int n, int C);
bool launch_cts_pipe(hipStream_t s, const DevArrays& a, int c_lo, int c_cnt, int C, int n, int64_t P, int max_cnt);
void launch_cts_shard_copy(hipStream_t s, const DevArrays& a, int lo, int hi, const int32_t* offs, int64_t* buf,
                           int to_buf);
void launch_minmax(hipStream_t s, const DevArrays& a, int32_t m);
void launch_sort(hipStream_t s, const DevArrays& a, int32_t m, int64_t cmin, int cts_bits, int R, int n,
                 int seg_bits, uint32_t** final_vals, uint64_t** final_keys);
int seg_sort_cap();
void launch_seg_count(hipStream_t s, const DevArrays& a, int32_t m, int R, int n, int nseg, uint32_t* segc,
                      unsigned long long* max_out);
hipError_t launch_sort_seg(hipStream_t s, const DevArrays& a, int32_t m, int64_t cmin, int cts_bits, int R, int n, int nseg,
                     uint32_t* segoff, uint32_t* segcur, int max_seg, uint32_t** final_vals, uint64_t** final_keys,
                     const std::vector<int>* cuts = nullptr,
                     const std::function<hipError_t(int)>& after_part = nullptr);
bool sort_small_ok(int32_t m);
void launch_sort_small(hipStream_t s, const DevArrays& a, int32_t m, int n, uint32_t** final_vals);
void launch_finish_order(hipStream_t s, const DevArrays& a, int32_t m, const uint32_t* vals, int R, int n);
void launch_gather_i32(hipStream_t s, int64_t E, const int32_t* src, const int32_t* g_pos, int32_t* dst);

size_t p256_table_bytes(int nk);
void launch_p256_tables(hipStream_t s, int nk, const uint8_t* keys65, uint32_t* tab, uint8_t* valid);
void launch_p256_verify(hipStream_t s, int64_t count, int nk, const int32_t* key_idx, const uint8_t* dig,
                        const uint8_t* r, const uint8_t* sg, const uint32_t* tab, const uint8_t* valid, uint8_t* out);

void launch_insert_claim(hipStream_t s, int64_t m, int64_t E0, int64_t cap, int C, const InsertIn& in,
                         const InsertState& st);
void launch_insert_check(hipStream_t s, int64_t m, int64_t E0, int64_t cap, int C, int n, const InsertIn& in,
                         const InsertState& st);
constexpr int kCommitAll = 0, kCommitStructure = 1, kCommitPayload = 2;
void launch_insert_commit(hipStream_t s, int64_t m, const unsigned long long* fail, const unsigned long long* fail_sig,
                          int64_t E0, int n, const InsertIn& in, const InsertState& st, int mode);
void launch_ts_to_pos(hipStream_t s, int64_t E0, int64_t m, const int32_t* g_pos, const int64_t* g_ts, int64_t* p_ts);
void launch_insert_unclaim(hipStream_t s, int64_t m, const unsigned long long* fail, const unsigned long long* fail_sig,
                           int64_t E0, int64_t cap, int C, const InsertIn& in, const InsertState& st);
bool launch_insert_fused(hipStream_t s, int64_t m, const unsigned long long* fail_sig, int64_t E0, int64_t cap, int C,
                         int n, const InsertIn& in, const InsertState& st, int mode);
void launch_insert_sig_first(hipStream_t s, int64_t m, int C, const int32_t* creator, const uint8_t* vout,
                             unsigned long long* fail);
void launch_unpack_packed(hipStream_t s, int64_t m, int64_t E0, const uint16_t* c16, const uint16_t* spb,
                          const uint16_t* opb, int64_t n_exc, const int64_t* exc_pos, const int32_t* exc_sp,
                          const int32_t* exc_op, int32_t* cr, int32_t* sp, int32_t* op);

void launch_scan_u32(hipStream_t s, uint32_t* buf, int64_t total, uint32_t* part);

struct PruneArgs {
    int64_t E, n_kept;
    int C;
    const int32_t *g_creator, *g_index, *g_sp, *g_op, *g_ntx;
    const int64_t* g_ts;
    const uint8_t *g_S, *g_id, *g_txnil;
    const int32_t* cut;
    uint32_t* scan;
    int32_t* first_gid;
    uint32_t* kept_total;
    int32_t *st_creator, *st_index, *st_sp, *st_op, *st_ntx, *old_gid;
    int64_t* st_ts;
    uint8_t *st_hash, *st_S;
    uint32_t* oth_count;
    int32_t *oth_new, *oth_op;
    uint8_t *oth_key, *oth_pid;
    int32_t *root_sp, *root_op;
    uint8_t* root_ids;
};
void launch_prune(hipStream_t s, const PruneArgs& a, uint32_t* scan_part);

void launch_scan_top(hipStream_t s, uint32_t* part, int nparts);

struct DiffArgs {
    int64_t E;
    int64_t rows;
    int c0, n;
    const int32_t *g_creator, *g_index, *g_sp, *g_op, *g_ntx;
    const int64_t* g_ts;
    const uint8_t *g_S, *g_id, *g_txnil;
    const int32_t* tab;
    uint32_t* part;
    uint32_t* total;
    int64_t *o_gid, *o_index, *o_spi, *o_opi, *o_ts;
    int32_t *o_creator, *o_opc, *o_ntx, *o_nil;
    uint8_t *o_hash, *o_S, *o_root;
};
constexpr int kDiffChunk = 2048;
void launch_diff(hipStream_t s, const DiffArgs& a);

}
```

### babble_amd/csrc/hgx_kernels.hip

```cpp
#include <hip/hip_runtime.h>

#include <algorithm>
#include <cstdint>
#include <cstdlib>
#include <cstring>
#include <map>
#include <mutex>
#include <tuple>

#include "hgx_device.h"
#include "hgx_kernels.h"

namespace hgx {


constexpr int kLayoutB = 4096;
constexpr int kLayoutH = 1024;

__global__ void __launch_bounds__(256) k_ck_pack(int64_t E0, int64_t E, const int32_t* __restrict__ g_creator,
                                                 const int32_t* __restrict__ g_index, const int32_t* __restrict__ c_base,
                                                 int64_t* __restrict__ g_ck) {
    const int64_t gid = E0 + (int64_t)blockIdx.x * blockDim.x + threadIdx.x;
    if (gid >= E) return;
    const int c = g_creator[gid];
    g_ck[gid] = ((int64_t)c << 32) | (uint32_t)(g_index[gid] - c_base[c]);
}

__device__ __forceinline__ void layout_one(int64_t gid, int p, const int32_t* __restrict__ g_creator,
                                           const int64_t* __restrict__ g_ck, const int32_t* __restrict__ g_op,
                                           const int64_t* __restrict__ g_ts, const int32_t* __restrict__ g_rr,
                                           const int64_t* __restrict__ g_cts, const int32_t* __restrict__ c_off,
                                           const int32_t* __restrict__ c_base, int32_t* __restrict__ p_gid,
                                           int32_t* __restrict__ p_chain, int32_t* __restrict__ p_op,
                                           int32_t* __restrict__ p_opu, int32_t* __restrict__ p_opk,
                                           int64_t* __restrict__ p_ts, int32_t* __restrict__ p_rr,
                                           int64_t* __restrict__ p_cts, int C, int n, int seg) {
    const int c = g_creator[gid];
    const int op = g_op[gid];
    int opp = -1, opu = -1, opk = -1;
    if (op >= 0) {
        const int64_t ck = g_ck[op];
        const int oc = (int)(ck >> 32);
        const int ok = (int)(uint32_t)ck;
        opp = c_off[oc] + ok;
        opu = (ok / seg) * C + oc;
        opk = ((oc % n) << kOpkBits) | (ok & ((1 << kOpkBits) - 1));
    }
    p_opk[p] = opk;
    p_gid[p] = (int32_t)gid;
    p_chain[p] = c;
    p_op[p] = opp;
    p_opu[p] = opu;
    p_ts[p] = g_ts[gid];
    p_rr[p] = g_rr[gid];
    p_cts[p] = g_cts[gid];
}

__global__ void __launch_bounds__(256) k_layout_direct(int64_t E0, int64_t E, const int32_t* __restrict__ g_creator,
                                                       const int32_t* __restrict__ g_index, const int64_t* __restrict__ g_ck,
                                                       const int32_t* __restrict__ g_op,
                                                       const int64_t* __restrict__ g_ts, const int32_t* __restrict__ g_rr,
                                                       const int64_t* __restrict__ g_cts, const int32_t* __restrict__ c_off,
                                                       const int32_t* __restrict__ c_base, int32_t* __restrict__ g_pos,
                                                       int32_t* __restrict__ p_gid, int32_t* __restrict__ p_chain,
                                                       int32_t* __restrict__ p_op, int32_t* __restrict__ p_opu,
                                                       int32_t* __restrict__ p_opk, int64_t* __restrict__ p_ts,
                                                       int32_t* __restrict__ p_rr, int64_t* __restrict__ p_cts, int C,
                                                       int n, int seg) {
    const int64_t gid = E0 + (int64_t)blockIdx.x * blockDim.x + threadIdx.x;
    if (gid >= E) return;
    const int c = g_creator[gid];
    const int p = c_off[c] + g_index[gid] - c_base[c];
    g_pos[gid] = p;
    layout_one(gid, p, g_creator, g_ck, g_op, g_ts, g_rr, g_cts, c_off, c_base, p_gid, p_chain, p_op, p_opu, p_opk,
               p_ts, p_rr, p_cts, C, n, seg);
}


constexpr int kLayoutB2 = 2048;
__global__ void __launch_bounds__(256) k_layout_staged(int64_t E0, int64_t E, const int32_t* __restrict__ g_creator,
                                                       const int32_t* __restrict__ g_index, const int64_t* __restrict__ g_ck,
                                                       const int32_t* __restrict__ g_op, const int64_t* __restrict__ g_ts,
                                                       const int32_t* __restrict__ g_rr, const int64_t* __restrict__ g_cts,
                                                       const int32_t* __restrict__ c_off, const int32_t* __restrict__ c_base,
                                                       int32_t* __restrict__ g_pos, int32_t* __restrict__ p_gid,
                                                       int32_t* __restrict__ p_chain, int32_t* __restrict__ p_op,
                                                       int32_t* __restrict__ p_opu, int32_t* __restrict__ p_opk,
                                                       int64_t* __restrict__ p_ts, int32_t* __restrict__ p_rr,
                                                       int64_t* __restrict__ p_cts, int C, int n, int seg) {
    constexpr int B = kLayoutB2, PT = B / 256;
    __shared__ int32_t s_cnt[kLayoutH], s_min[kLayoutH];
    __shared__ int32_t s_slot[B];
    __shared__ int32_t s_cr[B], s_ix[B];
    __shared__ __attribute__((aligned(16))) int64_t s_stg[B];
    __shared__ int32_t s_lo, s_hi;
    const int nbk = (int)gridDim.x, q8 = nbk / 8, r8 = nbk % 8, x8 = (int)blockIdx.x % 8;
    const int lb = x8 * q8 + min(x8, r8) + (int)blockIdx.x / 8;
    const int64_t g0 = E0 + (int64_t)lb * B;
    const int nb = (int)min<int64_t>(B, E - g0);
    const int t0 = threadIdx.x;
    int32_t cr[PT], ix[PT], op[PT], rr[PT];
    int64_t ts[PT], cts[PT], ck[PT];
#pragma unroll
    for (int k = 0; k < PT; k++) {
        const int t = t0 + 256 * k;
        const bool v = t < nb;
        const int64_t gid = g0 + (v ? t : 0);
        cr[k] = g_creator[gid];
        ix[k] = g_index[gid];
        op[k] = g_op[gid];
        rr[k] = g_rr[gid];
        ts[k] = g_ts[gid];
        cts[k] = g_cts[gid];
    }
#pragma unroll
    for (int k = 0; k < PT; k++) ck[k] = op[k] >= 0 ? g_ck[op[k]] : -1ll;
    if (t0 == 0) { s_lo = 0x7FFFFFFF; s_hi = -1; }
    for (int h = t0; h < kLayoutH; h += 256) { s_cnt[h] = 0; s_min[h] = 0x7FFFFFFF; }
    int lo = 0x7FFFFFFF, hi = -1;
#pragma unroll
    for (int k = 0; k < PT; k++) {
        const int t = t0 + 256 * k;
        if (t < nb) {
            s_cr[t] = cr[k];
            s_ix[t] = ix[k];
            lo = min(lo, cr[k]);
            hi = max(hi, cr[k]);
        }
    }
    __syncthreads();
    for (int o = 32; o >= 1; o >>= 1) { lo = min(lo, __shfl_xor(lo, o)); hi = max(hi, __shfl_xor(hi, o)); }
    if ((t0 & 63) == 0) { atomicMin(&s_lo, lo); atomicMax(&s_hi, hi); }
    __syncthreads();
    const int clo = s_lo;
    if (s_hi - clo >= kLayoutH) {
        for (int t = t0; t < nb; t += 256) {
            const int64_t gid = g0 + t;
            const int c = s_cr[t];
            const int p = c_off[c] + s_ix[t] - c_base[c];
            g_pos[gid] = p;
            layout_one(gid, p, g_creator, g_ck, g_op, g_ts, g_rr, g_cts, c_off, c_base, p_gid, p_chain, p_op,
                       p_opu, p_opk, p_ts, p_rr, p_cts, C, n, seg);
        }
        return;
    }
#pragma unroll
    for (int k = 0; k < PT; k++) {
        const int t = t0 + 256 * k;
        if (t < nb) {
            const int h = cr[k] - clo;
            atomicAdd(&s_cnt[h], 1);
            atomicMin(&s_min[h], ix[k]);
        }
    }
    __syncthreads();
    if (t0 < 64) {
        constexpr int PER = kLayoutH / 64;
        int v[PER], sum = 0;
#pragma unroll
        for (int k = 0; k < PER; k++) { v[k] = s_cnt[t0 * PER + k]; sum += v[k]; }
        int incl = sum;
        for (int o = 1; o < 64; o <<= 1) {
            const int y = __shfl_up(incl, o);
            if (t0 >= o) incl += y;
        }
        int run = incl - sum;
#pragma unroll
        for (int k = 0; k < PER; k++) { s_cnt[t0 * PER + k] = run; run += v[k]; }
    }
    __syncthreads();
#pragma unroll
    for (int k = 0; k < PT; k++) {
        const int t = t0 + 256 * k;
// ... 1743 lines not shown
    if (e == hipSuccess) cur = bytes;
    return e;
}

hipError_t blocks_per_cu(const void* f, int T, size_t lds, int* out) {
    int dev = 0;
    hipError_t e = hipGetDevice(&dev);
    if (e != hipSuccess) return e;
    std::lock_guard<std::mutex> lk(g_attr_mu);
    const auto key = std::make_tuple(dev, f, T, lds);
    auto it = g_occ.find(key);
    if (it != g_occ.end()) {
        *out = it->second;
        return hipSuccess;
    }
    int v = 0;
    e = hipOccupancyMaxActiveBlocksPerMultiprocessor(&v, f, T, lds);
    if (e == hipSuccess) g_occ[key] = *out = v;
    return e;
}

void launch_fill_many(hipStream_t s, const FillRange* r, int count) {
    if (count <= 0) return;
    FillArgs f{};
    uint32_t mx = 0;
    for (int i = 0; i < count && i < kFillMax; i++) {
        f.r[i] = r[i];
        mx = std::max(mx, r[i].bytes);
    }
    f.count = std::min(count, kFillMax);
    const unsigned bx = std::max(1u, std::min(256u, (mx / 4 + 255) / 256));
    hipLaunchKernelGGL(k_fill_many, dim3(bx, f.count), dim3(256), 0, s, f);
}

struct CopyArgs {
    CopyRange r[kCopyMax];
};
__global__ void __launch_bounds__(256) k_copy_many(CopyArgs f) {
    const CopyRange r = f.r[blockIdx.y];
    const uint32_t t0 = blockIdx.x * blockDim.x + threadIdx.x, st = gridDim.x * blockDim.x;
    const uintptr_t al = (uintptr_t)r.src | (uintptr_t)r.dst;
    uint32_t done = 0;
    const bool rs = r.reset >= 0;
    const uint32_t f4 = 0x01010101u * (uint32_t)(r.reset & 0xFF);
    if ((al & 15u) == 0) {
        uint4* s4 = (uint4*)r.src;
        uint4* d4 = (uint4*)r.dst;
        const uint32_t nq = r.bytes / 16;
        for (uint32_t t = t0; t < nq; t += st) {
            d4[t] = s4[t];
            if (rs) s4[t] = make_uint4(f4, f4, f4, f4);
        }
        done = nq * 16;
    } else if ((al & 3u) == 0) {
        uint32_t* s1 = (uint32_t*)r.src;
        uint32_t* d1 = (uint32_t*)r.dst;
        const uint32_t nw = r.bytes / 4;
        for (uint32_t t = t0; t < nw; t += st) {
            d1[t] = s1[t];
            if (rs) s1[t] = f4;
        }
        done = nw * 4;
    }
    uint8_t* sb = (uint8_t*)r.src;
    uint8_t* db = (uint8_t*)r.dst;
    for (uint32_t t = done + t0; t < r.bytes; t += st) {
        db[t] = sb[t];
        if (rs) sb[t] = (uint8_t)r.reset;
    }
}

void launch_copy_many(hipStream_t s, const CopyRange* r, int count) {
    if (count <= 0) return;
    CopyArgs f{};
    uint32_t mx = 0;
    for (int i = 0; i < count && i < kCopyMax; i++) {
        f.r[i] = r[i];
        mx = std::max(mx, r[i].bytes);
    }
    const unsigned bx = std::max(1u, std::min(64u, (mx / 16 + 255) / 256));
    hipLaunchKernelGGL(k_copy_many, dim3(bx, std::min(count, kCopyMax)), dim3(256), 0, s, f);
}

void launch_layout(hipStream_t s, int64_t E0, int64_t E, const DevArrays& a, int C, int n, int seg) {
    if (E <= E0) return;
    hipLaunchKernelGGL(k_ck_pack, dim3(nblk(E - E0, 256)), dim3(256), 0, s, E0, E, a.g_creator, a.g_index, a.c_base,
                       a.g_ck);
    if (E - E0 <= 8 * kLayoutB) {
        hipLaunchKernelGGL(k_layout_direct, dim3(nblk(E - E0, 256)), dim3(256), 0, s, E0, E, a.g_creator, a.g_index,
                           a.g_ck, a.g_op, a.g_ts, a.g_rr, a.g_cts, a.c_off, a.c_base, a.g_pos, a.p_gid, a.p_chain, a.p_op,
                           a.p_opu, a.p_opk, a.p_ts, a.p_rr, a.p_cts, C, n, seg);
        return;
    }
    hipLaunchKernelGGL(k_layout_staged, dim3(nblk(E - E0, kLayoutB2)), dim3(256), 0, s, E0, E, a.g_creator, a.g_index,
                       a.g_ck, a.g_op, a.g_ts, a.g_rr, a.g_cts, a.c_off, a.c_base, a.g_pos, a.p_gid, a.p_chain, a.p_op,
                       a.p_opu, a.p_opk, a.p_ts, a.p_rr, a.p_cts, C, n, seg);
}

void launch_la_sweep(hipStream_t s, const DevArrays& a, int C, int n, int max_len, int seg, int first, int32_t* chg,
                     int32_t stamp, int64_t* usum, int32_t* out, int32_t* out_next, const int32_t* c_old, int64_t u0) {
    const int nseg = (max_len + seg - 1) / seg;
    if ((int64_t)nseg * C <= u0) return;
    const int nwd = a.compact ? n / 2 : n;
#define LA_LAUNCH_V(GS, CPL, CT, V)                                                                           \
    {                                                                                                         \
        const int64_t threads = ((int64_t)nseg * C - u0) * GS;                                                \
        hipLaunchKernelGGL((k_la_sweep<GS, CPL, CT, V>), dim3(std::min(nblk(threads, 256), 2048u)), dim3(256), 0, \
                           s, (uint32_t*)a.LA, a.p_op, a.p_opu, a.c_off, a.c_len, a.c_base, C, n, nwd, nseg, seg, \
                           first ? 1 : 0, chg, stamp, usum, out, out_next, c_old, u0);                        \
    }
#define LA_LAUNCH_T(GS, CPL, CT)                                   \
    {                                                              \
        if (first == 2) LA_LAUNCH_V(GS, CPL, CT, true) else LA_LAUNCH_V(GS, CPL, CT, false) \
    }
#define LA_LAUNCH(GS, CPL, NW)                                        \
    {                                                                 \
        if (a.compact) LA_LAUNCH_T(GS, CPL, uint16_t) else LA_LAUNCH_T(GS, CPL, int32_t) \
    }
    HGX_DISPATCH_N(nwd, LA_LAUNCH);
#undef LA_LAUNCH
#undef LA_LAUNCH_T
#undef LA_LAUNCH_V
}

int fd_tile_rows(int n, int compact) {
    (void)compact;
    return n <= 32 ? 256 : 128;
}

int fd_cols(int compact, int ft) { return (compact ? 256 : 128) * 64 / ft; }

void launch_fd_build(hipStream_t s, const DevArrays& a, int C, int n, int max_len, int64_t P, const int32_t* c_old,
                     int max_new, int d_lo, int d_hi) {
    if (d_hi < 0) d_hi = n;
    if (d_hi <= d_lo) return;
    const int ft = fd_tile_rows(n, a.compact);
    const int tiles = c_old ? max(1, (max_new + ft - 1) / ft) : max(1, (max_len + ft - 1) / ft);
    const int nwd = a.compact ? n / 2 : n;
    const int DB = std::min(fd_cols(a.compact, ft), d_hi - d_lo);
    const int ncb = (d_hi - d_lo + DB - 1) / DB;
    const int wdw = DB / (a.compact ? 2 : 1) + 1;
    const size_t lds = ((size_t)(ft + 1) * (wdw + 1) + 1 + 3 * (size_t)DB + 8 * 128) * sizeof(int32_t);
    const int zs = (c_old && max_new <= ft) ? max(1, min(8, DB / 64)) : 1;
    const dim3 grid(C, tiles, ncb * zs);
#define FD_LAUNCH(CT_, RPL_)                                                                                    \
    hipLaunchKernelGGL((k_fd_build<CT_, RPL_>), grid, dim3(512), lds, s, (const uint32_t*)a.LA, (CT_*)a.FDT, a.c_off, \
                       a.c_len, a.c_base, n, nwd, ft, P, c_old, d_lo, d_hi, DB, zs)
    if (a.compact) {
        if (ft == 256) FD_LAUNCH(uint16_t, 4);
        else if (ft == 128) FD_LAUNCH(uint16_t, 2);
        else FD_LAUNCH(uint16_t, 1);
    } else {
        if (ft == 256) FD_LAUNCH(int32_t, 4);
        else if (ft == 128) FD_LAUNCH(int32_t, 2);
        else FD_LAUNCH(int32_t, 1);
    }
#undef FD_LAUNCH
}

void launch_round_gather(hipStream_t s, const DevArrays& a, int r, int C, int n, int64_t P) {
    if (a.compact)
        hipLaunchKernelGGL(k_round_gather<uint16_t>, dim3(nblk((int64_t)C * n, 256)), dim3(256), 0, s, r, a.Bm,
                           a.c_off, a.c_len, (const uint16_t*)a.LA, (const uint16_t*)a.FDT, a.p_gid, a.g_coin, a.WLA,
                           a.WFD, a.wflag, a.wcoin, C, n, P, 1);
    else
        hipLaunchKernelGGL(k_round_gather<int32_t>, dim3(nblk((int64_t)C * n, 256)), dim3(256), 0, s, r, a.Bm,
                           a.c_off, a.c_len, (const int32_t*)a.LA, (const int32_t*)a.FDT, a.p_gid, a.g_coin, a.WLA,
                           a.WFD, a.wflag, a.wcoin, C, n, P, 0);
}

void launch_wcoin(hipStream_t s, const DevArrays& a, int r0, int R, int C) {
    const int64_t RC = (int64_t)(R - r0) * C;
    if (RC <= 0) return;
    const size_t o = (size_t)r0 * C;
    hipLaunchKernelGGL(k_wcoin, dim3(nblk(RC, 256)), dim3(256), 0, s, RC, C, a.Bm + o, a.c_off, a.c_len, a.p_gid,
                       a.g_coin, a.wcoin + o);
}

void launch_fame(hipStream_t s, const DevArrays& a, int r0, int R, int C, int n, int nw, int sm, int G, int tally) {
// ... 296 lines not shown
```

### babble_amd/csrc/hgx_la_wave.hip

```cpp
#include <hip/hip_runtime.h>

#include <algorithm>
#include <cstdint>

#include "hgx_device.h"
#include "hgx_kernels.h"

namespace hgx {

namespace {

template <typename CT>
struct LaW;
template <>
struct LaW<int32_t> {
    static constexpr uint32_t kNone = 0xFFFFFFFFu;
    __device__ __forceinline__ static uint32_t wmax(uint32_t a, uint32_t b) {
        return (uint32_t)max((int32_t)a, (int32_t)b);
    }
    static constexpr int kPerWord = 1;
    __device__ __forceinline__ static uint32_t own_mask(int) { return 0xFFFFFFFFu; }
    __device__ __forceinline__ static uint32_t own_bits(int, int32_t own) { return (uint32_t)own; }
};
template <>
// ... 14 lines not shown
#define HGX_CB() asm volatile("" ::: "memory")
__device__ __forceinline__ int32_t lds_ld(const int32_t* p) {
    HGX_CB();
    const int32_t v = *p;
    HGX_CB();
    return v;
}
__device__ __forceinline__ void lds_st(int32_t* p, int32_t v) {
    HGX_CB();
    *p = v;
    HGX_CB();
}

template <int DW>
__device__ __forceinline__ void settle(uint32_t (&v)[DW]) {
#pragma unroll
    for (int w = 0; w < DW; w++) asm volatile("" : "+v"(v[w]));
}

template <int DW>
__device__ __forceinline__ void ring_load(const uint32_t* p, uint32_t (&v)[DW]) {
    HGX_CB();
    if constexpr (DW % 8 == 0) {
#pragma unroll
        for (int k = 0; k < DW / 4; k++) {
            const uint4 x = ((const uint4*)p)[k];
            v[4 * k] = x.x; v[4 * k + 1] = x.y; v[4 * k + 2] = x.z; v[4 * k + 3] = x.w;
        }
    } else if constexpr (DW == 4) {
        const uint4 x = *(const uint4*)p;
        v[0] = x.x; v[1] = x.y; v[2] = x.z; v[3] = x.w;
    } else if constexpr (DW == 2) {
        const uint2 x = *(const uint2*)p;
        v[0] = x.x; v[1] = x.y;
    } else {
        v[0] = *p;
    }
    HGX_CB();
}
template <int DW>
__device__ __forceinline__ void ring_store(uint32_t* p, const uint32_t (&v)[DW]) {
    HGX_CB();
    if constexpr (DW % 8 == 0) {
#pragma unroll
        for (int k = 0; k < DW / 4; k++) ((uint4*)p)[k] = make_uint4(v[4 * k], v[4 * k + 1], v[4 * k + 2], v[4 * k + 3]);
    } else if constexpr (DW == 4) *(uint4*)p = make_uint4(v[0], v[1], v[2], v[3]);
    else if constexpr (DW == 2) *(uint2*)p = make_uint2(v[0], v[1]);
    else *p = v[0];
    HGX_CB();
}
template <int DW>
__device__ __forceinline__ void row_store(uint32_t* p, const uint32_t (&v)[DW]) {
    if constexpr (DW % 8 == 0) {
#pragma unroll
        for (int k = 0; k < DW / 4; k++) ((uint4*)p)[k] = make_uint4(v[4 * k], v[4 * k + 1], v[4 * k + 2], v[4 * k + 3]);
    } else if constexpr (DW == 4) *(uint4*)p = make_uint4(v[0], v[1], v[2], v[3]);
    else if constexpr (DW == 2) *(uint2*)p = make_uint2(v[0], v[1]);
    else *p = v[0];
}

constexpr int kTagEmpty = -1, kTagBusy = -2;
constexpr int kNoDesc = -2147483647 - 1;
constexpr uint32_t kSpinCap = 1u << 24;

}

__device__ __forceinline__ int chain_lower_bound(const int32_t* __restrict__ p_gid, int off, int len, int64_t x) {
    int lo = 0, hi = len;
    while (lo < hi) {
        const int mid = (lo + hi) >> 1;
        if ((int64_t)p_gid[off + mid] < x) lo = mid + 1;
        else hi = mid;
    }
    return lo;
}

template <typename CT, int DW, int R, int Q, int NLW, int J, int CH, int MODE>
__global__ void __launch_bounds__(1024) k_la_wave(uint32_t* __restrict__ LA, const int32_t* __restrict__ p_opk,
                                                  const int32_t* __restrict__ c_off, const int32_t* __restrict__ c_len,
                                                  const int32_t* __restrict__ c_base,
                                                  const int32_t* __restrict__ c_old,
                                                  const int32_t* __restrict__ p_gid, int64_t E, int nts, int head,
                                                  int n, int lgnp, int nwd, int nblk, int32_t* __restrict__ err,
                                                  const int32_t* __restrict__ lmap, int na) {
    typedef LaW<CT> W;
    extern __shared__ uint32_t smem[];
    const int NP = 1 << lgnp;
    uint32_t* ring_d = smem;
    int32_t* ring_t = (int32_t*)(ring_d + (size_t)R * NP * DW);
    int32_t* q = ring_t + R * NP;
    int32_t* lqv = q + Q * NP;
    int32_t* prog = lqv + n;
    int32_t* s_old = prog + n;
    int32_t* s_off = s_old + n;
    int32_t* s_len = s_off + n;
    int32_t* s_abort = s_len + n;
    const int b = blockIdx.x % nblk, ts = (blockIdx.x / nblk) % nts, g = blockIdx.x / nblk / nts;
    const int c0 = g * n;
    const int wb = b * DW;
    const int tid = threadIdx.x;
    for (int t = tid; t < R * NP; t += blockDim.x) ring_t[t] = kTagEmpty;
    for (int t = tid; t < n; t += blockDim.x) {
        const int off = c_off[c0 + t], len = c_len[c0 + t];
        int o = 0, e = len;
        if constexpr (MODE == 1) o = c_old[c0 + t];
        if constexpr (MODE >= 2) {
            o = ts == 0 ? 0 : chain_lower_bound(p_gid, off, len, E * ts / nts);
            e = ts == nts - 1 ? len : chain_lower_bound(p_gid, off, len, E * (ts + 1) / nts);
            if constexpr (MODE == 3) e = ts == 0 ? o : min(e, o + head);
        }
        lqv[t] = o;
        prog[t] = o;
        s_old[t] = o;
        s_off[t] = off;
        s_len[t] = e;
    }
    if (tid == 0) *s_abort = 0;
    __syncthreads();
    const int nl = lmap ? na : n;
    const int ncw = (nl + 63) & ~63;
    if (tid >= ncw) {
        const int l = tid - ncw;
        uint32_t idle = 0;
        for (;;) {
            bool left = false, need[J];
            int lq[J];
#pragma unroll
            for (int j = 0; j < J; j++) {
                const int i = l + 64 * NLW * j;
                need[j] = false;
                lq[j] = 0;
                if (i < n) {
                    lq[j] = lds_ld(&lqv[i]);
                    if (lq[j] < s_len[i]) {
                        left = true;
                        need[j] = lq[j] + CH <= lds_ld(&prog[i]) + Q;
                    }
                }
            }
            if (!left) break;
            int32_t v[J][CH];
#pragma unroll
            for (int j = 0; j < J; j++)
                if (need[j]) {
                    const int i = l + 64 * NLW * j;
                    const int o = s_off[i] + lq[j], m = s_len[i] - lq[j];
#pragma unroll
                    for (int t = 0; t < CH; t++) v[j][t] = (t < m) ? p_opk[o + t] : -1;
                }
            bool any = false;
#pragma unroll
            for (int j = 0; j < J; j++)
                if (need[j]) {
                    const int i = l + 64 * NLW * j;
#pragma unroll
                    for (int t = 0; t < CH; t++) lds_st(&q[(((unsigned)(lq[j] + t) % Q) << lgnp) + i], v[j][t]);
                    HGX_CB();
                    lds_st(&lqv[i], min(lq[j] + CH, s_len[i]));
                    any = true;
                }
            if (any) {
                idle = 0;
            } else {
                if (lds_ld(s_abort) || ++idle > kSpinCap) break;
                __builtin_amdgcn_s_sleep(1);
            }
        }
        return;
    }
    if (tid >= nl) return;
    const int i = lmap ? lmap[tid] : tid;
    const int len = s_len[i];
    const int off = s_off[i];
    int own0 = c_base[c0 + i];
    asm volatile("" : "+v"(own0));
    const int ow = i / W::kPerWord - wb;
    const uint32_t omask = W::own_mask(i);
    int k = s_old[i];
    uint32_t carry[DW];
#pragma unroll
    for (int w = 0; w < DW; w++)
        carry[w] = (k > 0 && MODE != 2) ? LA[(size_t)(off + k - 1) * nwd + wb + w] : W::kNone;
    settle(carry);
    uint32_t* dst = LA + (size_t)(off + k) * nwd + wb;
    int opv = kNoDesc;
    uint32_t idle = 0;
    while (k < len) {
        const int lv = lds_ld(&lqv[i]);
        const int q0 = lds_ld(&q[(((unsigned)k % Q) << lgnp) + i]);
        const int q1 = lds_ld(&q[(((unsigned)(k + 1) % Q) << lgnp) + i]);
        const bool has_op = opv >= 0;
        const int opc = has_op ? (opv >> kOpkBits) : 0;
        const int opk = has_op ? (opv & ((1 << kOpkBits) - 1)) : 0;
        const int sl = (((unsigned)opk % R) << lgnp) + opc;
        int old = 0;
        int end = 0x7FFFFFFF;
        if constexpr (MODE != 0) old = lds_ld(&s_old[opc]);
        if constexpr (MODE == 3) end = lds_ld(&s_len[opc]);
        const int t1 = lds_ld(&ring_t[sl]);
        uint32_t od[DW];
        ring_load<DW>(ring_d + (size_t)sl * DW, od);
        const int t2 = lds_ld(&ring_t[sl]);
        bool ready = opv == -1 || (has_op && t1 == opk && t2 == opk);
        if (opv == -1) {
#pragma unroll
            for (int w = 0; w < DW; w++) od[w] = W::kNone;
        }
        const bool from_old = MODE != 0 && has_op && (opk < old || opk >= end);
        if (from_old || (has_op && !ready && t1 > opk)) {
            if (MODE == 2 && from_old) {
#pragma unroll
                for (int w = 0; w < DW; w++) od[w] = W::kNone;
            } else {
                uint32_t* src = LA + (size_t)(s_off[opc] + opk) * nwd + wb;
#pragma unroll
                for (int w = 0; w < DW; w++)
                    od[w] = __hip_atomic_load(src + w, __ATOMIC_RELAXED, __HIP_MEMORY_SCOPE_AGENT);
                settle(od);
            }
            ready = true;
        }
        const bool wave_idle = __ballot(ready) == 0;
        if (!ready) {
            if (opv == kNoDesc && lv > k) opv = q0;
            if (wave_idle) __builtin_amdgcn_s_sleep(1);
            if (((++idle) & 4095) == 0 && (idle > kSpinCap || lds_ld(s_abort))) {
                lds_st(s_abort, 1);
                atomicOr(err, 1);
                break;
            }
            continue;
        }
        idle = 0;
        uint32_t v[DW];
#pragma unroll
        for (int w = 0; w < DW; w++) {
            v[w] = W::wmax(carry[w], od[w]);
            v[w] = w == ow ? ((v[w] & ~omask) | W::own_bits(i, own0 + k)) : v[w];
        }
        if constexpr (DW == 16 && R == 8) asm volatile("s_waitcnt vmcnt(23)" ::: "memory");
        else if constexpr (R >= 16) asm volatile("s_waitcnt vmcnt(15)" ::: "memory");
        else asm volatile("s_waitcnt vmcnt(7)" ::: "memory");
        const int ws = (((unsigned)k % R) << lgnp) + i;
        lds_st(&ring_t[ws], kTagBusy);
        ring_store<DW>(ring_d + (size_t)ws * DW, v);
        lds_st(&ring_t[ws], k);
        row_store<DW>(dst, v);
        dst += nwd;
        lds_st(&prog[i], k + 1);
#pragma unroll
        for (int w = 0; w < DW; w++) carry[w] = v[w];
        k++;
        opv = lv > k ? q1 : kNoDesc;
    }
}

namespace {
template <typename CT, int DW, int R, int Q, int NLW, int J, int CH, int MODE>
hipError_t la_wave_launch1(hipStream_t s, const DevArrays& a, int G, int n, const int32_t* c_old, int64_t E, int nts,
                           int head, int32_t* err, const int32_t* lmap, int na) {
    const int nwd = a.compact ? n / 2 : n;
    const int nblk = nwd / DW;
    int lgnp = 0;
    while ((1 << lgnp) < n) lgnp++;
    const size_t np2 = (size_t)1 << lgnp;
    const size_t words = np2 * (R * DW + R + Q) + 5 * (size_t)n + 1;
    auto kern = k_la_wave<CT, DW, R, Q, NLW, J, CH, MODE>;
    {
        const hipError_t e = ensure_lds_limit((const void*)kern, 160 * 1024);
        if (e != hipSuccess) return e;
    }
    const int threads = (((lmap ? na : n) + 63) & ~63) + 64 * NLW;
    if (threads > 1024 || (lmap && G != 1)) return hipErrorInvalidValue;
    hipLaunchKernelGGL(kern, dim3(G * nts * nblk), dim3(threads), words * 4, s, (uint32_t*)a.LA, a.p_opk, a.c_off,
                       a.c_len, a.c_base, c_old, a.p_gid, E, nts, head, n, lgnp, nwd, nblk, err, lmap, na);
    return hipGetLastError();
}
template <typename CT, int DW, int R, int Q, int NLW, int J, int CH>
hipError_t la_wave_launch(hipStream_t s, const DevArrays& a, int G, int n, const int32_t* c_old, int64_t E,
                          int32_t* err, const int32_t* lmap, int na) {
    if (c_old) return la_wave_launch1<CT, DW, R, Q, NLW, J, CH, 1>(s, a, G, n, c_old, E, 1, 0, err, lmap, na);
    return la_wave_launch1<CT, DW, R, Q, NLW, J, CH, 0>(s, a, G, n, nullptr, E, 1, 0, err, lmap, na);
}
struct SegCfg {
    int dw, r, q;
};
inline SegCfg seg_cfg(int n, int nwd) {
    if (n > 128 && n <= 256 && nwd % 16 == 0) return {16, 8, 16};
    if (n <= 256) return {nwd % 8 == 0 ? 8 : (nwd % 4 == 0 ? 4 : 1), 8, 32};
    if (n <= 512) return {nwd % 4 == 0 ? 4 : 1, 8, 16};
    return {nwd % 2 == 0 ? 2 : 1, 8, 8};
}
template <typename CT>
hipError_t la_wave_dispatch(hipStream_t s, const DevArrays& a, int G, int n, const int32_t* c_old, int64_t E, int nts,
                            int head, int32_t* err, const int32_t* lmap, int na, bool narrow) {
    const int nwd = a.compact ? n / 2 : n;
    if (nts > 1) {
        const SegCfg g = seg_cfg(n, nwd);
#define SEG(DW_, R_, Q_, NLW_, J_, CH_)                                                                                \
    return head > 0 ? la_wave_launch1<CT, DW_, R_, Q_, NLW_, J_, CH_, 3>(s, a, G, n, nullptr, E, nts, head, err, lmap, \
                                                                          na)                                          \
                    : la_wave_launch1<CT, DW_, R_, Q_, NLW_, J_, CH_, 2>(s, a, G, n, nullptr, E, nts, 0, err, lmap, na)
        if (n <= 256) {
            if (g.dw == 16) SEG(16, 8, 16, 1, 4, 8);
            if (g.dw == 8) SEG(8, 8, 32, 1, 4, 8);
            if (g.dw == 4) SEG(4, 8, 32, 1, 4, 8);
            SEG(1, 8, 32, 1, 4, 8);
        }
        if (n <= 512) {
            if (g.dw == 4) SEG(4, 8, 16, 1, 8, 4);
            SEG(1, 8, 16, 1, 8, 4);
        }
        if (g.dw == 2) SEG(2, 8, 8, 2, 8, 2);
        SEG(1, 8, 8, 2, 8, 2);
#undef SEG
    }
    if (n <= 128) {
        if (nwd % 4 == 0 && !(narrow && c_old)) return la_wave_launch<CT, 4, 32, 64, 1, 2, 16>(s, a, G, n, c_old, E, err, lmap, na);
        return la_wave_launch<CT, 1, 32, 64, 1, 2, 16>(s, a, G, n, c_old, E, err, lmap, na);
    }
    if (n <= 256) {
        if (nwd % 4 == 0 && !(narrow && c_old))
            return la_wave_launch<CT, 4, 16, 64, 1, 4, 16>(s, a, G, n, c_old, E, err, lmap, na);
        return la_wave_launch<CT, 1, 16, 64, 1, 4, 16>(s, a, G, n, c_old, E, err, lmap, na);
    }
    if (n <= 512) return la_wave_launch<CT, 1, 16, 32, 1, 8, 8>(s, a, G, n, c_old, E, err, lmap, na);
    if (nwd % 2 == 0) return la_wave_launch<CT, 2, 8, 8, 2, 8, 2>(s, a, G, n, c_old, E, err, lmap, na);
    return la_wave_launch<CT, 1, 8, 16, 2, 8, 4>(s, a, G, n, c_old, E, err, lmap, na);
}
}

template <int NW>
__global__ void __launch_bounds__(256) k_la_small(uint32_t* __restrict__ LA, const int32_t* __restrict__ p_opk,
                                                  const int32_t* __restrict__ c_off, const int32_t* __restrict__ c_len,
                                                  const int32_t* __restrict__ c_base, const int32_t* __restrict__ c_old,
                                                  int n, int nwd, int compact, int32_t* __restrict__ err) {
    extern __shared__ __attribute__((aligned(16))) uint32_t smem[];
    const int g = blockIdx.x, c0 = g * n, tid = threadIdx.x, nt = blockDim.x;
    __shared__ int32_t s_P;
    int32_t* prog = (int32_t*)smem;
    int32_t* cpos = prog + 64;
    if (tid == 0) {
        int acc = 0;
        for (int c = 0; c < n; c++) {
            cpos[c] = acc;
            acc += c_len[c0 + c];
        }
        s_P = acc;
    }
    for (int c = tid; c < n; c += nt) prog[c] = c_old ? c_old[c0 + c] : 0;
    __syncthreads();
    const int P = s_P;
    int2* desc = (int2*)(cpos + 64);
    uint32_t* rows = (uint32_t*)(desc + ((P + 2) & ~1));
    for (int c = 0; c < n; c++) {
        const int o = cpos[c], len = c_len[c0 + c], off = c_off[c0 + c];
        for (int x = tid; x < len; x += nt) {
            const int v = p_opk[off + x];
            desc[o + x] = make_int2(v >= 0 ? cpos[v >> kOpkBits] + (v & ((1 << kOpkBits) - 1)) : -1, v);
        }
        if (c_old) {
            const int m = c_old[c0 + c];
            for (int x = tid; x < m * nwd; x += nt) rows[(size_t)(o + x / nwd) * NW + x % nwd] = LA[(size_t)off * nwd + x];
        }
    }
    if (tid == 0) desc[P] = make_int2(-1, -1);
    __syncthreads();
    if (tid < 64) {
        const int c = tid;
        const bool live = c < n;
        const int len = live ? c_len[c0 + c] : 0, base = live ? cpos[c] : 0;
        int k = live ? prog[c] : 0;
        const int own0 = live ? c_base[c0 + c] : 0;
        const int ow = compact ? c >> 1 : c;
        const uint32_t omask = compact ? (0xFFFFu << ((c & 1) * 16)) : 0xFFFFFFFFu;
        const uint32_t none = compact ? 0u : 0xFFFFFFFFu;
        uint32_t carry[NW];
#pragma unroll
        for (int w = 0; w < NW; w++) carry[w] = (k > 0) ? rows[(size_t)(base + k - 1) * NW + w] : none;
        int2 d = k < len ? desc[base + k] : make_int2(-1, -1);
        uint32_t guard = 0;
        while (__any(k < len)) {
            if (k < len) {
                const int opc = d.y >= 0 ? d.y >> kOpkBits : 0, opk = d.y & ((1 << kOpkBits) - 1);
                const int pr = prog[opc];
// ... 88 lines not shown
        case 4: return la_small_launch<4>(s, a, G, n, c_old, lds, err);
        case 8: return la_small_launch<8>(s, a, G, n, c_old, lds, err);
        case 16: return la_small_launch<16>(s, a, G, n, c_old, lds, err);
        default: return hipErrorInvalidValue;
    }
}

int la_wave_blocks(int n, int compact) {
    const int nwd = compact ? n / 2 : n;
    return nwd / seg_cfg(n, nwd).dw;
}

int la_wave_segments(int n, int compact, int num_cus, int max_segs) {
    const int nwd = compact ? n / 2 : n;
    const SegCfg g = seg_cfg(n, nwd);
    int np2 = 1;
    while (np2 < n) np2 <<= 1;
    const size_t bytes = ((size_t)np2 * (g.r * g.dw + g.r + g.q) + 5 * (size_t)n + 1) * 4;
    const int per_cu = std::max(1, std::min(4, (int)((160 * 1024) / bytes)));
    return std::max(1, std::min(max_segs, per_cu * num_cus / la_wave_blocks(n, compact)));
}

__global__ void __launch_bounds__(256) k_la_seg_bounds(const int32_t* __restrict__ p_gid, const int32_t* __restrict__ c_off,
                                                       const int32_t* __restrict__ c_len, int64_t E, int nts, int n,
                                                       int32_t* __restrict__ tbl) {
    const int t = blockIdx.x;
    for (int c = threadIdx.x; c < n; c += blockDim.x) {
        const int len = c_len[c];
        tbl[(size_t)t * n + c] = t == 0 ? 0 : t == nts ? len : chain_lower_bound(p_gid, c_off[c], len, E * t / nts);
    }
}

template <typename CT>
__global__ void __launch_bounds__(256) k_la_seg_check(const CT* __restrict__ LA, const int32_t* __restrict__ p_gid,
                                                      const int32_t* __restrict__ p_op, const int32_t* __restrict__ p_chain,
                                                      const int32_t* __restrict__ c_off, const int32_t* __restrict__ tbl,
                                                      int64_t E, int nts, int n, int head, int32_t* __restrict__ flag) {
    const int t = 1 + (int)blockIdx.x / n, c = (int)blockIdx.x % n;
    const int o = tbl[(size_t)t * n + c], e = tbl[(size_t)(t + 1) * n + c], off = c_off[c];
    bool bad = false;
    if (e - o > head) {
        const CT* __restrict__ row = LA + (size_t)(off + o + head) * n;
        for (int i = threadIdx.x; i < n; i += blockDim.x)
            if (Coord<CT>::la(row[i]) < 0 && tbl[(size_t)t * n + i] > 0) bad = true;
    }
    const int kh = min(e, o + head);
    for (int k = o + (int)threadIdx.x; k < kh; k += blockDim.x) {
        if (k == o && k > 0) {
            int tz = t - 1;
            while (tz > 0 && tbl[(size_t)tz * n + c] > k - 1) tz--;
            if (tz >= 1 && k - 1 < tbl[(size_t)tz * n + c] + head) bad = true;
        }
        const int opp = p_op[off + k];
        if (opp >= 0) {
            const int d = p_chain[opp], r = opp - c_off[d];
            const int64_t gz = p_gid[opp];
            int tz = (int)min<int64_t>(nts - 1, gz * nts / E);
            while (tz > 0 && E * tz / nts > gz) tz--;
            while (tz + 1 < nts && E * (tz + 1) / nts <= gz) tz++;
            if (tz >= 1 && tz < t && r < tbl[(size_t)tz * n + d] + head) bad = true;
        }
    }
    if (bad) atomicOr(flag, 1);
}

hipError_t launch_la_seg_check(hipStream_t s, const DevArrays& a, int n, int64_t E, int nts, int head, int32_t* tbl,
                               int32_t* flag) {
    if (nts < 2) return hipSuccess;
    hipLaunchKernelGGL(k_la_seg_bounds, dim3(nts + 1), dim3(256), 0, s, a.p_gid, a.c_off, a.c_len, E, nts, n, tbl);
    if (a.compact)
        hipLaunchKernelGGL(k_la_seg_check<uint16_t>, dim3((nts - 1) * n), dim3(256), 0, s, (const uint16_t*)a.LA,
                           a.p_gid, a.p_op, a.p_chain, a.c_off, tbl, E, nts, n, head, flag);
    else
        hipLaunchKernelGGL(k_la_seg_check<int32_t>, dim3((nts - 1) * n), dim3(256), 0, s, (const int32_t*)a.LA,
                           a.p_gid, a.p_op, a.p_chain, a.c_off, tbl, E, nts, n, head, flag);
    return hipGetLastError();
}

bool la_wave_ok(int n, int max_len, int n_active) {
    return n >= 1 && n <= 1024 && n_active <= 896 && max_len < (1 << kOpkBits);
}

hipError_t launch_la_wave(hipStream_t s, const DevArrays& a, int G, int n, const int32_t* c_old, int64_t E, int nts,
                          int head, int32_t* err, const int32_t* lmap, int na, bool narrow) {
    if (nts > 1 && (G != 1 || c_old)) return hipErrorInvalidValue;
    return a.compact ? la_wave_dispatch<uint16_t>(s, a, G, n, c_old, E, nts, head, err, lmap, na, narrow)
                     : la_wave_dispatch<int32_t>(s, a, G, n, c_old, E, nts, head, err, lmap, na, narrow);
}

}
```

### babble_amd/hashgraph.py

```python
from __future__ import annotations

import ctypes as C
import os
from typing import List, Optional, Sequence

import numpy as np

from . import _lib
from ._lib import HgxError, hgx_error, hgx_events, ptr

UNKNOWN_PARENT = -2


def compact_columns(t) -> dict:
    ntx = np.where(np.asarray(t.txnil) != 0, -1, np.asarray(t.ntx)).astype(np.int32)
    return dict(creator=np.ascontiguousarray(t.creator, np.int32), index=np.ascontiguousarray(t.index, np.int32),
                sp=np.ascontiguousarray(t.sp, np.int32), op=np.ascontiguousarray(t.op, np.int32),
                ts=np.ascontiguousarray(t.ts, np.int64),
                coin=np.ascontiguousarray(np.asarray(t.hash)[:, 16] != 0, np.uint8),
                s=np.ascontiguousarray(t.s, np.uint8), ntx=ntx)


class HostBuffer:

# ... 640 lines not shown
        m = 0 if over.value else min(rows, cnt.value)
        return {nm: a[:m] for nm, a in cols.items()}, cnt.value, bool(over.value)

    def ReadWireInfo(self, creator: int, sp_index: int, op_creator: int, op_index: int):
        sp, op, err = C.c_int64(), C.c_int64(), hgx_error()
        _lib.check(self.L.hgx_read_wire_info(self.ctx, creator, sp_index, op_creator, op_index, C.byref(sp),
                                             C.byref(op), C.byref(err)), err)
        return sp.value, op.value

    def Blocks(self, graph: int = 0) -> List[dict]:
        res = []
        for b in range(int(self.L.hgx_num_blocks(self.ctx, graph))):
            rr, nev, nil, com = C.c_int32(), C.c_int32(), C.c_int32(), C.c_int32()
            first, ntx = C.c_int64(), C.c_int64()
            self.L.hgx_block_info(self.ctx, graph, b, C.byref(rr), C.byref(first), C.byref(nev), C.byref(ntx),
                                  C.byref(nil), C.byref(com))
            res.append(dict(rr=rr.value, first=first.value, n_events=nev.value, ntx=ntx.value,
                            tx_nil=bool(nil.value), committed=bool(com.value)))
        return res

    def Ancestor(self, x: int, y: int) -> bool:
        return bool(self.L.hgx_ancestor(self.ctx, x, y))

    def SelfAncestor(self, x: int, y: int) -> bool:
        return bool(self.L.hgx_self_ancestor(self.ctx, x, y))

    def See(self, x: int, y: int) -> bool:
        return bool(self.L.hgx_see(self.ctx, x, y))

    def StronglySee(self, x: int, y: int) -> bool:
        return bool(self.L.hgx_strongly_see(self.ctx, x, y))

    def OldestSelfAncestorToSee(self, x: int, y: int) -> int:
        return int(self.L.hgx_oldest_self_ancestor_to_see(self.ctx, x, y))

    def Round(self, x: int) -> int:
        return int(self.L.hgx_round(self.ctx, x))

    def Witness(self, x: int) -> bool:
        return bool(self.L.hgx_witness(self.ctx, x))

    def coords(self, x: int):
        la = np.zeros(self.n, np.int32)
        fd = np.zeros(self.n, np.int32)
        rc = self.L.hgx_get_coords(self.ctx, x, ptr(la), ptr(fd))
        if rc:
            raise HgxError(rc, "hgx_get_coords failed")
        return la, fd

    def num_events(self) -> int:
        return int(self.L.hgx_num_events(self.ctx))

    def rounds(self):
        E = self.num_events()
        rnd = np.zeros(max(E, 1), np.int32)
        wit = np.zeros(max(E, 1), np.int8)
        fam = np.zeros(max(E, 1), np.int8)
        if E:
            rc = self.L.hgx_get_rounds(self.ctx, 0, E, ptr(rnd), ptr(wit), ptr(fam))
            if rc:
                raise HgxError(rc, "hgx_get_rounds failed")
        return rnd[:E], wit[:E], fam[:E]

    def received(self):
        E = self.num_events()
        rr = np.zeros(max(E, 1), np.int32)
        cts = np.zeros(max(E, 1), np.int64)
        if E:
            rc = self.L.hgx_get_received(self.ctx, 0, E, ptr(rr), ptr(cts))
            if rc:
                raise HgxError(rc, "hgx_get_received failed")
        return rr[:E], cts[:E]

    def results(self, graph: int = 0) -> dict:
        rnd, wit, fam = self.rounds()
        rr, cts = self.received()
        return dict(round=rnd, witness=wit, famous=fam, rr=rr, cts=np.where(rr >= 0, cts, 0),
                    order=self.ConsensusEvents(graph), last_round=self.LastRound(graph),
                    undecided=self.UndecidedRounds(graph), lcr=self.LastConsensusRound(graph),
                    lcre=self.LastCommitedRoundEvents(graph), consensus_tx=self.ConsensusTransactions(graph),
                    pending_loaded=self.PendingLoadedEvents(graph), blocks=self.Blocks(graph))

    def phase_times(self):
        out = np.zeros(22, np.float64)
        self.L.hgx_phase_times(self.ctx, ptr(out), 22)
        return dict(coords_ms=out[0], rounds_ms=out[1], fame_ms=out[2], order_ms=out[3],
                    la_sweeps=int(out[4]), rounds=int(out[5]), compact=int(out[6]),
                    la_rows=int(out[7]), rebuild=int(out[8]), r_lo=int(out[9]),
                    la_wave=int(out[10]), la_wave_fallbacks=int(out[11]), la_wave_segs=int(out[12]),
                    round_p_runs=int(out[13]), round_p_fallbacks=int(out[14]), round_p_ovf=int(out[15]),
                    round_p_fail_round=int(out[16]), round_p_fail_chain=int(out[17]),
                    round_g_runs=int(out[18]), la_small=int(out[19]), la_verify=int(out[20]),
                    sort_seg=int(out[21]))

    def set_fame_tally(self, mode):
        m = {"popc": 0, "vote": 1, "mfma": 2}[mode] if isinstance(mode, str) else int(mode)
        if self.L.hgx_set_fame_tally(self.ctx, m) != 0:
            raise ValueError(f"invalid fame tally {mode}")

    def set_la_kernel(self, mode):
        m = {"wave": 0, "sweep": 1, "ring": 1025, "wave+verify": 1026}[mode] if isinstance(mode, str) else int(mode)
        if self.L.hgx_set_la_kernel(self.ctx, m) != 0:
            raise ValueError(f"invalid lastAncestors kernel {mode}")

    def set_round_kernel(self, mode):
        m = ({"auto": 0, "block": 1, "candidate": 2, "persistent": 3, "graph": 4, "auto-steps": 5}[mode]
             if isinstance(mode, str) else int(mode))
        if self.L.hgx_set_round_kernel(self.ctx, m) != 0:
            raise ValueError(f"invalid round kernel {mode}")

    def set_sort_kernel(self, mode):
        m = {"auto": 0, "radix": 1}[mode] if isinstance(mode, str) else int(mode)
        if self.L.hgx_set_sort_kernel(self.ctx, m) != 0:
            raise ValueError(f"invalid sort kernel {mode}")

    def set_round_shards(self, shards: int):
        if self.L.hgx_set_round_shards(self.ctx, int(shards)) != 0:
            raise ValueError(f"invalid shard count {shards} (an empty context, 1..8 shards, "
                             f"GPU_MAX_HW_QUEUES >= shards + 2 for shards sharing a device)")

    def set_shard_remote(self, on: bool = True):
        if self.L.hgx_set_shard_remote(self.ctx, 1 if on else 0) != 0:
            raise ValueError("hgx_set_shard_remote: not a chain-sharded context")

    def set_cts_kernel(self, mode):
        m = {"auto": 0, "tile": 1, "pipe": 2}[mode] if isinstance(mode, str) else int(mode)
        if self.L.hgx_set_cts_kernel(self.ctx, m) != 0:
            raise ValueError(f"invalid timestamp kernel {mode}")

    def set_incremental(self, on: bool):
        if self.L.hgx_set_incremental(self.ctx, 1 if on else 0) != 0:
            raise ValueError("invalid schedule")

    def reserve_rounds(self, rounds: int):
        if self.L.hgx_reserve_rounds(self.ctx, int(rounds)) != 0:
            raise ValueError("hgx_reserve_rounds failed")

    def set_coord_storage(self, mode):
        if self.L.hgx_set_coord_storage(self.ctx, int(mode)) != 0:
            raise ValueError(f"invalid coordinate storage mode {mode}")

    def kernel_stats(self):
        res = {}
        for k in range(10):
            name = C.create_string_buffer(32)
            ms, launches, nbytes = C.c_double(), C.c_int64(), C.c_double()
            if self.L.hgx_kernel_stats(self.ctx, k, name, 32, C.byref(ms), C.byref(launches), C.byref(nbytes)):
                break
            res[name.value.decode()] = dict(ms=ms.value, launches=launches.value, bytes=nbytes.value)
        return res

    KERNELS = ("layout", "la_sweep", "fd_build", "round_gather", "round_search", "fame", "threshold",
               "round_received", "cts_median", "order_sort")

    def set_kernel_timing(self, which=True):
        if which is True:
            mask = -1
        elif not which:
            mask = 0
        else:
            mask = 1 << self.KERNELS.index(which)
        self.L.hgx_set_kernel_timing(self.ctx, mask)

    def reset_stats(self):
        self.L.hgx_reset_stats(self.ctx)


class DeviceBuffer:

    def __init__(self, a: np.ndarray, device: int = 0):
        self.L = _lib.lib()
        self.device = device
        a = np.ascontiguousarray(a)
        self.nbytes = a.nbytes
        self.p = C.c_void_p()
        if self.L.hgx_device_alloc(device, max(1, a.nbytes), C.byref(self.p)) != 0:
# ... 155 lines not shown
```

### include/hgx.h

```cpp
#ifndef HGX_H
#define HGX_H

#include <stdint.h>

#ifdef __cplusplus
extern "C" {
#endif

#define HGX_ABI_VERSION 6

enum {
    HGX_OK = 0,
    HGX_ERR_KEY_NOT_FOUND = 1,
    HGX_ERR_TOO_LATE = 2,
    HGX_ERR_PASSED_INDEX = 3,
    HGX_ERR_SKIPPED_INDEX = 4,
    HGX_ERR_NO_ROOT = 5,
    HGX_ERR_SELF_PARENT = 100,
    HGX_ERR_OTHER_PARENT = 101,
    HGX_ERR_INVALID = 102,
    HGX_ERR_CAPACITY = 103,
    HGX_ERR_SIGNATURE = 104,
    HGX_ERR_DEVICE = 200,
    HGX_ERR_PANIC = 300
// ... 165 lines not shown
int32_t hgx_consensus_events(hgx_ctx* ctx, int32_t graph, int64_t first, int64_t count, int64_t* gids);
int64_t hgx_num_blocks(hgx_ctx* ctx, int32_t graph);
int32_t hgx_block_info(hgx_ctx* ctx, int32_t graph, int64_t b, int32_t* round_received, int64_t* first,
                       int32_t* n_events, int64_t* n_tx, int32_t* tx_nil, int32_t* committed);
typedef void (*hgx_commit_fn)(void* user, int32_t graph, int64_t b, int32_t round_received, int64_t first,
                              int32_t n_events, int64_t n_tx);
int32_t hgx_set_commit_callback(hgx_ctx* ctx, hgx_commit_fn fn, void* user);
int32_t hgx_get_block(hgx_ctx* ctx, int32_t graph, int32_t round_received, int64_t* b, hgx_error* err);
int32_t hgx_consensus_received(hgx_ctx* ctx, int32_t graph, int64_t first, int64_t count, int64_t* gids,
                               int32_t* round_received, int64_t* consensus_ts);

int32_t hgx_last_from(hgx_ctx* ctx, int32_t participant, int64_t* gid, int32_t* is_root, hgx_error* err);
int32_t hgx_participant_events(hgx_ctx* ctx, int32_t participant, int64_t skip, int64_t* gids, int64_t cap,
                               int64_t* count, hgx_error* err);
int32_t hgx_participant_event(hgx_ctx* ctx, int32_t participant, int64_t index, int64_t* gid, hgx_error* err);
int32_t hgx_get_root(hgx_ctx* ctx, int32_t participant, int64_t* x, int64_t* y, int32_t* index, int32_t* round,
                     hgx_error* err);
int32_t hgx_get_event(hgx_ctx* ctx, int64_t gid, int32_t* creator, int64_t* index, int64_t* self_parent,
                      int64_t* other_parent, int64_t* timestamp_ns, int32_t* ntx, int32_t* tx_nil, hgx_error* err);
int32_t hgx_wire_info(hgx_ctx* ctx, int64_t first, int64_t count, int32_t* self_parent_index,
                      int32_t* other_parent_creator, int32_t* other_parent_index);
int32_t hgx_read_wire_info(hgx_ctx* ctx, int32_t creator, int64_t self_parent_index, int32_t other_parent_creator,
                           int64_t other_parent_index, int64_t* self_parent, int64_t* other_parent, hgx_error* err);

typedef struct {
    int64_t* gid;
    int32_t* creator_id;
    int64_t* index;
    int64_t* self_parent_index;
    int32_t* other_parent_creator;
    int64_t* other_parent_index;
    int64_t* timestamp_ns;
    uint8_t* hash;
    uint8_t* sig_s;
    int32_t* ntx;
    int32_t* tx_nil;
    uint8_t* root_parent;
} hgx_wire_out;
int32_t hgx_diff_wire(hgx_ctx* ctx, int32_t graph, const int32_t* known, int64_t sync_limit,
                      hgx_wire_out* out, int64_t cap, int64_t* count, int32_t* over_limit, hgx_error* err);

int32_t hgx_get_rounds(hgx_ctx* ctx, int64_t first, int64_t count, int32_t* round, int8_t* witness,
                       int8_t* famous);
int32_t hgx_get_received(hgx_ctx* ctx, int64_t first, int64_t count, int32_t* round_received,
                         int64_t* consensus_ts);
int32_t hgx_get_coords(hgx_ctx* ctx, int64_t gid, int32_t* last_ancestors, int32_t* first_descendants);

int32_t hgx_ancestor(hgx_ctx* ctx, int64_t x, int64_t y);
int32_t hgx_self_ancestor(hgx_ctx* ctx, int64_t x, int64_t y);
int32_t hgx_see(hgx_ctx* ctx, int64_t x, int64_t y);
int32_t hgx_strongly_see(hgx_ctx* ctx, int64_t x, int64_t y);
int64_t hgx_oldest_self_ancestor_to_see(hgx_ctx* ctx, int64_t x, int64_t y);
int32_t hgx_round(hgx_ctx* ctx, int64_t x);
int32_t hgx_witness(hgx_ctx* ctx, int64_t x);

int32_t hgx_block_hash(int64_t round_received, int32_t ntx, const uint8_t* const* tx, const int64_t* tx_len,
                       int32_t tx_nil, uint8_t* out32);

int32_t hgx_sha256_batch(int32_t device, const uint8_t* data, const int64_t* offsets, int64_t count,
                         uint8_t* out32, hgx_error* err);
int32_t hgx_sha256_batch_device(const uint8_t* d_data, const int64_t* d_offsets, int64_t count,
                                uint8_t* d_out32, void* stream);
int32_t hgx_sha256_bench(int32_t device, int64_t count, int32_t min_len, int32_t max_len, uint64_t seed,
                         int32_t warmup, int32_t iters, double* ms_per_launch, int64_t* total_bytes,
                         int64_t* n_blocks, int64_t n_sample, uint8_t* sample32);

int32_t hgx_exchange_floor_bench(int32_t device, int32_t chains, int32_t n, int32_t rounds, double* us_per_round);

int32_t hgx_p256_verify_batch(int32_t device, const uint8_t* keys65, int32_t n_keys, const int32_t* key_idx,
                              const uint8_t* digest32, const uint8_t* r32, const uint8_t* s32, int64_t count,
                              uint8_t* out, hgx_error* err);
int32_t hgx_p256_verify_bench(int32_t device, const uint8_t* keys65, int32_t n_keys, const int32_t* key_idx,
                              const uint8_t* digest32, const uint8_t* r32, const uint8_t* s32, int64_t count,
                              int32_t warmup, int32_t iters, uint8_t* out, double* ms_per_launch);

int32_t hgx_phase_times(hgx_ctx* ctx, double* out, int32_t cap);
int32_t hgx_kernel_stats(hgx_ctx* ctx, int32_t k, char* name, int32_t name_cap, double* ms, int64_t* launches,
                         double* bytes);
int32_t hgx_reset_stats(hgx_ctx* ctx);
int32_t hgx_set_kernel_timing(hgx_ctx* ctx, int32_t mask);

int32_t hgx_set_coord_storage(hgx_ctx* ctx, int32_t mode);
int32_t hgx_set_fame_tally(hgx_ctx* ctx, int32_t mode);
int32_t hgx_set_la_kernel(hgx_ctx* ctx, int32_t mode);
int32_t hgx_set_round_kernel(hgx_ctx* ctx, int32_t mode);
int32_t hgx_set_sort_kernel(hgx_ctx* ctx, int32_t mode);
int32_t hgx_set_round_shards(hgx_ctx* ctx, int32_t shards);
int32_t hgx_set_shard_remote(hgx_ctx* ctx, int32_t on);
int32_t hgx_set_cts_kernel(hgx_ctx* ctx, int32_t mode);
int32_t hgx_set_incremental(hgx_ctx* ctx, int32_t on);
int32_t hgx_reserve_rounds(hgx_ctx* ctx, int32_t rounds);

int32_t hgx_device_alloc(int32_t device, int64_t bytes, void** ptr);
int32_t hgx_device_free(int32_t device, void* ptr);
int32_t hgx_device_copy(int32_t device, void* dst, const void* src, int64_t bytes, int32_t to_device);

int32_t hgx_trace_gossip(int32_t n_participants, int32_t n_silent, int64_t n_events, uint64_t seed,
                         double stale_prob, int32_t stale_depth,
                         int32_t* creator, int64_t* index, int64_t* self_parent, int64_t* other_parent,
                         int64_t* timestamp_ns, uint8_t* hash, uint8_t* sig_s, int32_t* ntx, int32_t* tx_nil,
                         int64_t* tx_seq);
int32_t hgx_trace_tx_payload(int32_t creator, int64_t seq, uint8_t* out, int32_t cap);

#ifdef __cplusplus
}
#endif
#endif
```

Baseline: 248.8 million.

## Pipeline first bulk ingest: overlap H2D copies with insert, layout and lastAncestors waves

Adds a pipelined path for a fresh 32-bit bulk insert. A helper thread streams the index and parent arrays to the device in pieces on a side stream. Meanwhile the main stream runs insert and layout for each finished piece, and segmented lastAncestors wave kernels run per piece on two alternating side streams, bounded by per-piece chain limits. The later coordinate phase detects the precomputed layout and wave work and skips relaunching them. The aim is to hide host-to-device transfer and serial layout time behind compute. The cost is an extra histogram round trip, thread synchronisation, and a more complex plan that falls back when its guesses do not hold.

```diff
diff --git a/babble_amd/_lib.py b/babble_amd/_lib.py
--- a/babble_amd/_lib.py
+++ b/babble_amd/_lib.py
@@ -192,6 +192,7 @@
     _sig(L, "hgx_set_cts_kernel", i32, [p, i32])
     _sig(L, "hgx_set_root_others", i32, [p, p, i64, p])
     _sig(L, "hgx_set_la_kernel", i32, [p, i32])
+    _sig(L, "hgx_set_ingest_pipeline", i32, [p, i32, i64])
     _sig(L, "hgx_set_incremental", i32, [p, i32])
     _sig(L, "hgx_find_order_begin", i32, [p, p])
     _sig(L, "hgx_find_order_end", i32, [p, p])
diff --git a/babble_amd/csrc/hgx_api.cpp b/babble_amd/csrc/hgx_api.cpp
--- a/babble_amd/csrc/hgx_api.cpp
+++ b/babble_amd/csrc/hgx_api.cpp
@@ -595,6 +595,7 @@
         set_err(err, HGX_ERR_INVALID, "hgx_insert_and_run32: bad arguments");
         return HGX_ERR_INVALID;
     }
+    c->eng.pipe_used = 0;
     if (count < 65536 || c->rooted || c->shard_world > 1) {
         int32_t rc = hgx_insert_events32(c, ev, count, n_inserted, err);
         if (rc) return rc;
@@ -603,7 +604,11 @@
     DeviceGuard dg(c);
     const int64_t E0 = c->eng.E;
     hgx::InsertOut out;
-    hipError_t e = c->eng.insert_split_begin32(ev->creator, ev->index, ev->self_parent, ev->other_parent, count, out);
+    bool piped = false;
+    hipError_t e = c->grp ? hipSuccess
+                          : c->eng.insert_pipe32(ev->creator, ev->index, ev->self_parent, ev->other_parent, count, out, piped);
+    if (e != hipSuccess) return dev_err(err, e, "hgx_insert_and_run32");
+    if (!piped) e = c->eng.insert_split_begin32(ev->creator, ev->index, ev->self_parent, ev->other_parent, count, out);
     if (e != hipSuccess) return dev_err(err, e, "hgx_insert_and_run32");
     e = c->eng.payload_begin32(ev->timestamp_ns, ev->coin, ev->sig_s, ev->ntx, out.accepted);
     if (e != hipSuccess) return dev_err(err, e, "hgx_insert_and_run32");
@@ -2497,8 +2502,8 @@
 
 int32_t hgx_phase_times(hgx_ctx* c, double* out, int32_t cap) {
     if (!c || !out) return 0;
-    const int32_t m = std::min<int32_t>(cap, 22);
-    double v[22] = {c->eng.phase_ms[0], c->eng.phase_ms[1], c->eng.phase_ms[2], c->eng.phase_ms[3],
+    const int32_t m = std::min<int32_t>(cap, 23);
+    double v[23] = {c->eng.phase_ms[0], c->eng.phase_ms[1], c->eng.phase_ms[2], c->eng.phase_ms[3],
                     (double)c->eng.la_sweeps, (double)c->eng.R, (double)c->eng.compact,
                     (double)c->eng.la_rows, c->eng.last_rebuild ? 1.0 : 0.0, (double)c->rh.r_lo,
                     c->eng.la_wave_used ? 1.0 : 0.0, (double)c->eng.la_wave_fallbacks,
@@ -2506,7 +2511,7 @@
                     (double)c->eng.round_p_fallbacks, (double)c->eng.round_p_ovf,
                     (double)c->eng.round_p_fail_round, (double)c->eng.round_p_fail_chain,
                     (double)c->eng.round_g_runs, c->eng.la_small_used ? 1.0 : 0.0,
-                    c->eng.la_verified ? 1.0 : 0.0, (double)c->eng.sort_seg_runs};
+                    c->eng.la_verified ? 1.0 : 0.0, (double)c->eng.sort_seg_runs, (double)c->eng.pipe_used};
     for (int32_t i = 0; i < m; i++) out[i] = v[i];
     return m;
 }
@@ -2579,6 +2584,15 @@
                                : hipSuccess;
     if (prev >= 0 && prev != device) (void)hipSetDevice(prev);
     return e == hipSuccess ? HGX_OK : HGX_ERR_DEVICE;
+}
+
+int32_t hgx_set_ingest_pipeline(hgx_ctx* c, int32_t pieces, int64_t min_events) {
+    if (!c || pieces < 0 || pieces > hgx::kPipeMaxPieces || min_events < 0) return HGX_ERR_INVALID;
+    each_shard(c, [&](hgx_ctx* x) {
+        x->eng.pipe_pieces = pieces;
+        x->eng.pipe_min = min_events;
+    });
+    return HGX_OK;
 }
 
 int32_t hgx_set_la_kernel(hgx_ctx* c, int32_t mode) {
diff --git a/babble_amd/csrc/hgx_engine.cpp b/babble_amd/csrc/hgx_engine.cpp
--- a/babble_amd/csrc/hgx_engine.cpp
+++ b/babble_amd/csrc/hgx_engine.cpp
@@ -133,6 +133,14 @@
     if (h_flag) (void)hipHostFree(h_flag);
     if (h_segc) (void)hipHostFree(h_segc);
     if (df_host) (void)hipHostFree(df_host);
+    if (pipe_thread.joinable()) pipe_thread.join();
+    if (stream_p) {
+        (void)hipStreamSynchronize(stream_p);
+        (void)hipStreamDestroy(stream_p);
+    }
+    for (hipEvent_t e : ev_pc) if (e) (void)hipEventDestroy(e);
+    for (hipEvent_t e : ev_lay) if (e) (void)hipEventDestroy(e);
+    for (hipEvent_t e : ev_side) if (e) (void)hipEventDestroy(e);
     if (stream_o) (void)hipStreamSynchronize(stream_o);
     for (auto e : ev_o)
         if (e) (void)hipEventDestroy(e);
@@ -764,6 +772,7 @@
                                int commit_mode) {
     out = InsertOut();
     const int64_t E0 = E;
+    pipe_ready = false;
     InsertState st = insert_state();
     if (count > 0) {
         if (!launch_insert_fused(stream, count, fail_sig, E0, cap, C, n, in, st, commit_mode)) {
@@ -822,7 +831,181 @@
     R = 0;
     laid_out = false;
     ids_known = true;
+    pipe_ready = false;
     return hipStreamSynchronize(stream);
+}
+
+hipError_t Engine::insert_pipe32(const int32_t* creator, const int32_t* index, const int32_t* sp, const int32_t* op,
+                                 int64_t count, InsertOut& out, bool& taken) {
+    taken = false;
+    pipe_used = 0;
+    if (pipe_pieces <= 0 || count < pipe_min || count < 2 || count > cap || E != 0 || rooted || G != 1 || grp ||
+        time_mask != 0 || la_kernel != 0 || n > 896)
+        return hipSuccess;
+    const int guess = (!force_coord32 && (n % 2) == 0 && count / C <= 65533) ? 1 : 0;
+    const int base = rebuild_segments(count, guess);
+    if (base < 2) return hipSuccess;
+    const int nts = la_segs_override > 0
+                        ? base
+                        : std::max(base, (int)std::min<int64_t>((int64_t)kPipeSegMult * base, count / C / (2 * kLaHeadRows)));
+    const int pieces = std::min(std::min(pipe_pieces, (int)kPipeMaxPieces), nts);
+    int seg_cut[kPipeMaxPieces + 1];
+    int64_t cut[kPipeMaxPieces + 1];
+    for (int k = 0; k <= pieces; k++) {
+        seg_cut[k] = (int)((int64_t)nts * k / pieces);
+        cut[k] = count * seg_cut[k] / nts;
+    }
+    const size_t c = (size_t)count, Cz = (size_t)C;
+    if (st_creator.n < c) HGX_TRY(st_creator.alloc(c));
+    if (st_index32.n < c) HGX_TRY(st_index32.alloc(c));
+    if (st_sp32.n < c) HGX_TRY(st_sp32.alloc(c));
+    if (st_op32.n < c) HGX_TRY(st_op32.alloc(c));
+    const size_t o_hist = 64, o_lim = o_hist + kPipeMaxPieces * Cz;
+    if (pipe_buf.n < o_lim + kPipeMaxPieces * Cz) HGX_TRY(pipe_buf.alloc(o_lim + kPipeMaxPieces * Cz));
+    if (!stream2) {
+        HGX_TRY(hipStreamCreateWithFlags(&stream2, hipStreamNonBlocking));
+        HGX_TRY(hipEventCreateWithFlags(&ev_pay, hipEventDisableTiming));
+    }
+    if (!stream_o) {
+        HGX_TRY(hipStreamCreateWithFlags(&stream_o, hipStreamNonBlocking));
+        for (int k = 0; k <= kOrderParts; k++) HGX_TRY(hipEventCreateWithFlags(&ev_o[k], hipEventDisableTiming));
+    }
+    if (!stream_p) {
+        HGX_TRY(hipStreamCreateWithFlags(&stream_p, hipStreamNonBlocking));
+        for (hipEvent_t& e : ev_pc) HGX_TRY(hipEventCreateWithFlags(&e, hipEventDisableTiming));
+        for (hipEvent_t& e : ev_lay) HGX_TRY(hipEventCreateWithFlags(&e, hipEventDisableTiming));
+        for (hipEvent_t& e : ev_side) HGX_TRY(hipEventCreateWithFlags(&e, hipEventDisableTiming));
+    }
+    HGX_TRY(payload_wait_S());
+    if (pay_thread.joinable()) pay_thread.join();
+    if (pipe_thread.joinable()) pipe_thread.join();
+    pipe_err = hipSuccess;
+    pipe_stage = 0;
+    pipe_stop = 0;
+    std::vector<int64_t> cuts(cut, cut + pieces + 1);
+    pipe_thread = std::thread([=]() {
+        hipError_t e = hipSetDevice(dev);
+        if (e == hipSuccess) e = hipMemcpyAsync(st_creator.p, creator, c * 4, hipMemcpyHostToDevice, stream2);
+        if (e == hipSuccess) e = hipEventRecord(ev_pc[0], stream2);
+        if (e != hipSuccess) pipe_err = e;
+        pipe_stage.store(1, std::memory_order_release);
+        for (int k = 0; k < pieces; k++) {
+            if (pipe_stop.load(std::memory_order_acquire)) break;
+            const size_t g0 = (size_t)cuts[k], m = (size_t)(cuts[k + 1] - cuts[k]);
+            if (e == hipSuccess) e = hipMemcpyAsync(st_index32.p + g0, index + g0, m * 4, hipMemcpyHostToDevice, stream2);
+            if (e == hipSuccess) e = hipMemcpyAsync(st_sp32.p + g0, sp + g0, m * 4, hipMemcpyHostToDevice, stream2);
+            if (e == hipSuccess) e = hipMemcpyAsync(st_op32.p + g0, op + g0, m * 4, hipMemcpyHostToDevice, stream2);
+            if (e == hipSuccess) e = hipEventRecord(ev_pc[k + 1], stream2);
+            if (e != hipSuccess) pipe_err = e;
+            pipe_stage.store(k + 2, std::memory_order_release);
+        }
+        const hipError_t es = hipStreamSynchronize(stream2);
+        if (e == hipSuccess && es != hipSuccess) pipe_err = es;
+    });
+    auto stop = [&](hipError_t e) {
+        pipe_stop.store(1, std::memory_order_release);
+        if (pipe_thread.joinable()) pipe_thread.join();
+        return e != hipSuccess ? e : pipe_err;
+    };
+    auto wait_stage = [&](int want) {
+        while (pipe_stage.load(std::memory_order_acquire) < want) std::this_thread::yield();
+        return pipe_err;
+    };
+#define PIPE_TRY(x)                                  \
+    do {                                             \
+        const hipError_t e_ = (x);                   \
+        if (e_ != hipSuccess) return stop(e_);       \
+    } while (0)
+    int32_t* gate = pipe_buf.p;
+    PIPE_TRY(hipMemsetAsync(pipe_buf.p, 0, (o_hist + (size_t)pieces * Cz) * 4, stream));
+    PIPE_TRY(wait_stage(1));
+    PIPE_TRY(hipStreamWaitEvent(stream, ev_pc[0], 0));
+    launch_pipe_hist(stream, pieces, cut, C, st_creator.p, pipe_buf.p + o_hist);
+    PIPE_TRY(hipGetLastError());
+    pipe_hist.resize((size_t)pieces * Cz);
+    PIPE_TRY(hipMemcpyAsync(pipe_hist.data(), pipe_buf.p + o_hist, pipe_hist.size() * 4, hipMemcpyDeviceToHost, stream));
+    PIPE_TRY(hipStreamSynchronize(stream));
+    pipe_lim.assign((size_t)pieces * Cz, 0);
+    std::vector<int32_t> len(Cz, 0);
+    int64_t known = 0;
+    int mlen = 0;
+    for (int k = 0; k < pieces; k++)
+        for (size_t ch = 0; ch < Cz; ch++) {
+            len[ch] += pipe_hist[(size_t)k * Cz + ch];
+            pipe_lim[(size_t)k * Cz + ch] = len[ch];
+        }
+    for (size_t ch = 0; ch < Cz; ch++) {
+        known += len[ch];
+        mlen = std::max(mlen, len[ch]);
+    }
+    const int plan_compact = (!force_coord32 && (n % 2) == 0 && mlen - 1 <= 65533) ? 1 : 0;
+    if (known != count || plan_compact != guess || !la_wave_ok(n, mlen, n)) {
+        PIPE_TRY(stop(hipSuccess));
+        return hipSuccess;
+    }
+    compact = plan_compact;
+    layout_slots(count, len, pipe_off);
+    std::memcpy(h_cpar, len.data(), Cz * 4);
+    std::memset(h_cpar + C, 0, 2 * Cz * 4);
+    PIPE_TRY(hipMemcpyAsync(c_off.p, pipe_off.data(), (Cz + 1) * 4, hipMemcpyHostToDevice, stream));
+    PIPE_TRY(hipMemcpyAsync(cpar_blk.p, h_cpar, 3 * Cz * 4, hipMemcpyHostToDevice, stream));
+    PIPE_TRY(hipMemcpyAsync(pipe_buf.p + o_lim, pipe_lim.data(), pipe_lim.size() * 4, hipMemcpyHostToDevice, stream));
+    const DevArrays a = arrays();
+    const InsertState st = insert_state();
+    for (int k = 0; k < pieces; k++) {
+        const int64_t g0 = cut[k], g1 = cut[k + 1];
+        PIPE_TRY(wait_stage(k + 2));
+        PIPE_TRY(hipStreamWaitEvent(stream, ev_pc[k + 1], 0));
+        InsertIn in{};
+        in.creator = st_creator.p + g0; in.index32 = st_index32.p + g0; in.sp32 = st_sp32.p + g0; in.op32 = st_op32.p + g0;
+        launch_pipe_insert(stream, g1 - g0, g0, cap, C, n, in, st, gate);
+        launch_layout(stream, g0, g1, a, C, n, kLaSeg, gate);
+        PIPE_TRY(hipGetLastError());
+        PIPE_TRY(hipEventRecord(ev_lay[k], stream));
+        hipStream_t side = (k & 1) ? stream_p : stream_o;
+        PIPE_TRY(hipStreamWaitEvent(side, ev_lay[k], 0));
+        LaSubset sub;
+        sub.first = seg_cut[k]; sub.count = seg_cut[k + 1] - seg_cut[k];
+        sub.c_lim = pipe_buf.p + o_lim + (size_t)k * Cz; sub.gate = gate;
+        PIPE_TRY(launch_la_wave(side, a, 1, n, nullptr, count, nts, 0, counters.p + 6, nullptr, n, false, sub));
+    }
+    PIPE_TRY(hipEventRecord(ev_side[0], stream_o));
+    PIPE_TRY(hipStreamWaitEvent(stream, ev_side[0], 0));
+    if (pieces > 1) {
+        PIPE_TRY(hipEventRecord(ev_side[1], stream_p));
+        PIPE_TRY(hipStreamWaitEvent(stream, ev_side[1], 0));
+    }
+    PIPE_TRY(copy_to_pinned(h_small, ins_fail.p, 8, 0xFF));
+    PIPE_TRY(copy_to_pinned(h_ins, ins_blk.p, ins_blk.n * sizeof(int32_t)));
+    PIPE_TRY(stage_issue());
+    PIPE_TRY(hipStreamSynchronize(stream));
+    PIPE_TRY(stop(hipSuccess));
+#undef PIPE_TRY
+    unsigned long long fail = 0;
+    std::memcpy(&fail, h_small, 8);
+    if (fail != ~0ull) {
+        E = count;
+        return clear();
+    }
+    E = count;
+    split32 = true;
+    out = InsertOut();
+    out.accepted = count;
+    out.last_gid.resize(C);
+    out.last_index.resize(C);
+    out.chain_base.resize(C);
+    out.graph_loaded.resize(G);
+    std::memcpy(out.last_gid.data(), h_ins, Cz * 4);
+    std::memcpy(out.last_index.data(), h_ins + C, Cz * 4);
+    std::memcpy(out.chain_base.data(), h_ins + 2 * C, Cz * 4);
+    std::memcpy(out.graph_loaded.data(), h_ins + ins_gl_off, (size_t)G * 8);
+    pipe_ready = true;
+    pipe_En = count;
+    pipe_nts = nts;
+    pipe_compact = plan_compact;
+    pipe_used = pieces;
+    taken = true;
+    return hipSuccess;
 }
 
 hipError_t Engine::prune_stage(const std::vector<int32_t>& cut, int64_t n_kept, PruneOut& out) {
@@ -1169,6 +1352,21 @@
     return hipSuccess;
 }
 
+void Engine::layout_slots(int64_t En, const std::vector<int32_t>& chain_len, std::vector<int32_t>& off) const {
+    int act = 0;
+    for (int c = 0; c < C; c++) act += chain_len[c] > 0 ? 1 : 0;
+    const int64_t share = (Ppos - En) / (2 * (int64_t)act + (C - act));
+    off.assign(C + 1, 0);
+    for (int c = 0; c < C; c++)
+        off[c + 1] = off[c] + ((chain_len[c] + (int32_t)((chain_len[c] > 0 ? 2 : 1) * share)) & ~31);
+}
+
+int Engine::rebuild_segments(int64_t En, int coord_compact) const {
+    if (G != 1 || En < (int64_t)kLaSegMinRows * C) return 1;
+    const int cap_segs = (int)std::max<int64_t>(kLaMaxSegs, En / C / (2 * kLaHeadRows));
+    return la_segs_override > 0 ? la_segs_override : la_wave_segments(n, coord_compact, num_cus, cap_segs);
+}
+
 hipError_t Engine::divide_rounds(int64_t En, const std::vector<int32_t>& chain_len,
                                  const std::vector<int32_t>& chain_base, RoundsHost& out) {
     stage_out.clear();
@@ -1191,12 +1389,7 @@
     max_len = new_max_len;
     const size_t csz = compact ? 2 : 4;
     if (rebuild) {
-        int act = 0;
-        for (int c = 0; c < C; c++) act += chain_len[c] > 0 ? 1 : 0;
-        const int64_t share = (Ppos - En) / (2 * (int64_t)act + (C - act));
-        h_off.assign(C + 1, 0);
-        for (int c = 0; c < C; c++)
-            h_off[c + 1] = h_off[c] + ((chain_len[c] + (int32_t)((chain_len[c] > 0 ? 2 : 1) * share)) & ~31);
+        layout_slots(En, chain_len, h_off);
         HGX_TRY(hipMemcpyAsync(c_off.p, h_off.data(), (C + 1) * 4, hipMemcpyHostToDevice, stream));
         h_len_div.assign(C, 0);
         last_rebuild = true;
@@ -1230,9 +1423,6 @@
     DevArrays a = arrays();
     HGX_TRY(hipEventRecord(ph0, stream));
     const int seg = kLaSeg;
-    kbeg(K_LAYOUT);
-    launch_layout(stream, E0, En, a, C, n, seg);
-    kend(K_LAYOUT, (double)(En - E0) * 64);
     const size_t nunits = (size_t)((max_len + seg - 1) / seg) * C;
     int64_t u0 = 0;
     int la_na = n;
@@ -1249,11 +1439,13 @@
         }
     }
     la_wave_used = la_kernel == 0 && la_wave_ok(n, max_len, la_na) && (n <= 896 || la_map);
-    la_wave_segs = 1;
-    if (la_wave_used && rebuild && G == 1 && En >= (int64_t)kLaSegMinRows * C) {
-        const int cap = (int)std::max<int64_t>(kLaMaxSegs, En / C / (2 * kLaHeadRows));
-        la_wave_segs = la_segs_override > 0 ? la_segs_override : la_wave_segments(n, compact, num_cus, cap);
-    }
+    const bool piped = pipe_ready && rebuild && la_wave_used && !la_map && pipe_nts > 1 && En == pipe_En &&
+                       compact == pipe_compact && h_off == pipe_off;
+    pipe_ready = false;
+    la_wave_segs = piped ? pipe_nts : (la_wave_used && rebuild) ? rebuild_segments(En, compact) : 1;
+    kbeg(K_LAYOUT);
+    if (!piped) launch_layout(stream, E0, En, a, C, n, seg);
+    kend(K_LAYOUT, (double)(En - E0) * 64);
     if (rebuild) {
         if (!la_wave_used) HGX_TRY(hipMemsetAsync(LA.p, compact ? 0x00 : 0xFF, (size_t)h_off[C] * n * csz, stream));
     } else {
@@ -1313,7 +1505,7 @@
         const size_t small_lds = (la_wave_segs == 1 && !la_map && la_small_override != 0) ? la_small_bytes(n, compact, gpos) : 0;
         la_small_used = small_lds > 0;
         if (la_small_used) HGX_TRY(launch_la_small(stream, a, G, n, cold, small_lds, counters.p + 6));
-        else
+        else if (!piped)
             HGX_TRY(launch_la_wave(stream, a, G, n, cold, En, la_wave_segs, 0, counters.p + 6, la_map, la_na,
                                    !rebuild && (En - E0) <= 8 * (int64_t)C));
         if (la_wave_segs > 1)
diff --git a/babble_amd/csrc/hgx_engine.h b/babble_amd/csrc/hgx_engine.h
--- a/babble_amd/csrc/hgx_engine.h
+++ b/babble_amd/csrc/hgx_engine.h
@@ -189,6 +189,12 @@
                            std::vector<uint8_t>& coin, std::vector<int32_t>& ntx, std::vector<uint8_t>& txnil);
     hipError_t divide_rounds(int64_t E, const std::vector<int32_t>& chain_len,
                              const std::vector<int32_t>& chain_base, RoundsHost& out);
+    hipError_t insert_pipe32(const int32_t* creator, const int32_t* index, const int32_t* sp, const int32_t* op,
+                             int64_t count, InsertOut& out, bool& taken);
+    static constexpr int kPipeSegMult = 2;
+    int pipe_pieces = 4;
+    int64_t pipe_min = 4000000;
+    int pipe_used = 0;
     hipError_t decide_fame(int32_t r0, std::vector<int8_t>& fame_out);
     hipError_t find_order(const std::vector<uint8_t>& elig, const std::vector<uint8_t>& famous,
                           const std::vector<uint8_t>& ur_empty, int32_t r0, int max_unrecv, OrderHost& out);
@@ -263,6 +269,19 @@
     hipError_t insert_impl(const InsertIn& in, int64_t count, InsertOut& out, const unsigned long long* fail_sig,
                            int commit_mode = kCommitAll);
     hipStream_t stream2 = nullptr;
+    void layout_slots(int64_t En, const std::vector<int32_t>& chain_len, std::vector<int32_t>& off) const;
+    int rebuild_segments(int64_t En, int coord_compact) const;
+    hipStream_t stream_p = nullptr;
+    hipEvent_t ev_pc[kPipeMaxPieces + 1] = {}, ev_lay[kPipeMaxPieces] = {}, ev_side[2] = {};
+    std::atomic<int> pipe_stage{0};
+    std::atomic<int> pipe_stop{0};
+    std::thread pipe_thread;
+    hipError_t pipe_err = hipSuccess;
+    DBuf<int32_t> pipe_buf;
+    std::vector<int32_t> pipe_hist, pipe_lim, pipe_off;
+    bool pipe_ready = false;
+    int64_t pipe_En = 0;
+    int pipe_nts = 0, pipe_compact = 0;
     bool pay32 = false;
     bool split32 = false;
     hipEvent_t ev_pay = nullptr;
diff --git a/babble_amd/csrc/hgx_insert.hip b/babble_amd/csrc/hgx_insert.hip
--- a/babble_amd/csrc/hgx_insert.hip
+++ b/babble_amd/csrc/hgx_insert.hip
@@ -282,6 +282,73 @@
         hipLaunchKernelGGL(k_insert_unclaim, dim3(nblocks(m)), dim3(256), 0, s, m, fail, fail_sig, E0, cap, C, in, st);
 }
 
+
+struct PipeCuts {
+    int64_t cut[kPipeMaxPieces + 1];
+};
+__global__ void __launch_bounds__(256) k_pipe_hist(PipeCuts pc, int C, const int32_t* __restrict__ creator,
+                                                   int32_t* __restrict__ hist) {
+    extern __shared__ int32_t s_h[];
+    const int piece = blockIdx.y;
+    for (int c = threadIdx.x; c < C; c += blockDim.x) s_h[c] = 0;
+    __syncthreads();
+    const int64_t k1 = pc.cut[piece + 1];
+    for (int64_t k = pc.cut[piece] + (int64_t)blockIdx.x * blockDim.x + threadIdx.x; k < k1;
+         k += (int64_t)gridDim.x * blockDim.x) {
+        const int cr = creator[k];
+        if (cr >= 0 && cr < C) atomicAdd(&s_h[cr], 1);
+    }
+    __syncthreads();
+    for (int c = threadIdx.x; c < C; c += blockDim.x)
+        if (s_h[c]) atomicAdd(&hist[(size_t)piece * C + c], s_h[c]);
+}
+
+void launch_pipe_hist(hipStream_t s, int pieces, const int64_t* cut, int C, const int32_t* creator, int32_t* hist) {
+    PipeCuts pc{};
+    int64_t most = 0;
+    for (int k = 0; k <= pieces; k++) pc.cut[k] = cut[k];
+    for (int k = 0; k < pieces; k++) most = cut[k + 1] - cut[k] > most ? cut[k + 1] - cut[k] : most;
+    int64_t blocks = (most + 4095) / 4096;
+    blocks = blocks < 1 ? 1 : blocks > 256 ? 256 : blocks;
+    const unsigned bx = (unsigned)blocks;
+    hipLaunchKernelGGL(k_pipe_hist, dim3(bx, (unsigned)pieces), dim3(256), (size_t)C * 4, s, pc, C, creator, hist);
+}
+
+__global__ void __launch_bounds__(256) k_pipe_claim(int64_t m, int64_t E0, int64_t cap, int C, InsertIn in,
+                                                    InsertState st, const int32_t* __restrict__ gate) {
+    if (*gate) return;
+    const int64_t k = (int64_t)blockIdx.x * blockDim.x + threadIdx.x;
+    if (k < m) ins_claim(k, E0, cap, C, in, st);
+}
+
+__global__ void __launch_bounds__(256) k_pipe_check(int64_t m, int64_t E0, int64_t cap, int C, int n, InsertIn in,
+                                                    InsertState st, const int32_t* __restrict__ gate) {
+    if (*gate) return;
+    const int64_t k = (int64_t)blockIdx.x * blockDim.x + threadIdx.x;
+    if (k >= m) return;
+    ins_check(k, E0, cap, C, n, in, st);
+    if (in.sp_at(k) == -1 && in.idx_at(k) != 0) atomicMin(st.fail, ((unsigned long long)k << 8) | 0xFFull);
+}
+
+__global__ void __launch_bounds__(256) k_pipe_commit(int64_t m, int64_t E0, int n, InsertIn in, InsertState st,
+                                                     int32_t* __restrict__ gate) {
+    if (*st.fail != ~0ull) {
+        if (blockIdx.x == 0 && threadIdx.x == 0) *gate = 1;
+        return;
+    }
+    ins_commit(m, nullptr, nullptr, E0, n, in, st, kCommitStructure, (int64_t)blockIdx.x * blockDim.x,
+               (int64_t)gridDim.x * blockDim.x);
+}
+
+void launch_pipe_insert(hipStream_t s, int64_t m, int64_t E0, int64_t cap, int C, int n, const InsertIn& in,
+                        const InsertState& st, int32_t* gate) {
+    if (m <= 0) return;
+    hipLaunchKernelGGL(k_pipe_claim, dim3(nblocks(m)), dim3(256), 0, s, m, E0, cap, C, in, st, gate);
+    hipLaunchKernelGGL(k_pipe_check, dim3(nblocks(m)), dim3(256), 0, s, m, E0, cap, C, n, in, st, gate);
+    const unsigned grid = nblocks(m) < 4096u ? nblocks(m) : 4096u;
+    hipLaunchKernelGGL(k_pipe_commit, dim3(grid), dim3(256), 0, s, m, E0, n, in, st, gate);
+}
+
 constexpr int kEscape = 0xFFFF;
 constexpr int kUnknownParent = -2;
 
diff --git a/babble_amd/csrc/hgx_kernels.h b/babble_amd/csrc/hgx_kernels.h
--- a/babble_amd/csrc/hgx_kernels.h
+++ b/babble_amd/csrc/hgx_kernels.h
@@ -124,7 +124,8 @@
 void launch_copy_many(hipStream_t s, const CopyRange* r, int count);
 
 int fd_tile_rows(int n, int compact);
-void launch_layout(hipStream_t s, int64_t E0, int64_t E, const DevArrays& a, int C, int n, int seg);
+void launch_layout(hipStream_t s, int64_t E0, int64_t E, const DevArrays& a, int C, int n, int seg,
+                   const int32_t* gate = nullptr);
 bool la_wave_ok(int n, int max_len, int n_active);
 size_t la_small_bytes(int n, int compact, int64_t P);
 hipError_t launch_la_small(hipStream_t s, const DevArrays& a, int G, int n, const int32_t* c_old, size_t lds,
@@ -133,9 +134,14 @@
 int la_wave_segments(int n, int compact, int num_cus, int max_segs);
 hipError_t launch_la_seg_check(hipStream_t s, const DevArrays& a, int n, int64_t E, int nts, int head, int32_t* tbl,
                                int32_t* flag);
+struct LaSubset {
+    int first = 0, count = 0;
+    const int32_t* c_lim = nullptr;
+    const int32_t* gate = nullptr;
+};
 hipError_t launch_la_wave(hipStream_t s, const DevArrays& a, int G, int n, const int32_t* c_old, int64_t E, int nts,
                           int head, int32_t* err, const int32_t* lmap = nullptr, int na = 0,
-                          bool narrow = false);
+                          bool narrow = false, const LaSubset& sub = LaSubset());
 void launch_la_sweep(hipStream_t s, const DevArrays& a, int C, int n, int max_len, int seg, int first, int32_t* chg,
                      int32_t stamp, int64_t* usum, int32_t* out, int32_t* out_next, const int32_t* c_old, int64_t u0);
 void launch_fd_build(hipStream_t s, const DevArrays& a, int C, int n, int max_len, int64_t P, const int32_t* c_old,
@@ -219,6 +225,10 @@
 constexpr int kCommitAll = 0, kCommitStructure = 1, kCommitPayload = 2;
 void launch_insert_commit(hipStream_t s, int64_t m, const unsigned long long* fail, const unsigned long long* fail_sig,
                           int64_t E0, int n, const InsertIn& in, const InsertState& st, int mode);
+constexpr int kPipeMaxPieces = 8;
+void launch_pipe_hist(hipStream_t s, int pieces, const int64_t* cut, int C, const int32_t* creator, int32_t* hist);
+void launch_pipe_insert(hipStream_t s, int64_t m, int64_t E0, int64_t cap, int C, int n, const InsertIn& in,
+                        const InsertState& st, int32_t* gate);
 void launch_ts_to_pos(hipStream_t s, int64_t E0, int64_t m, const int32_t* g_pos, const int64_t* g_ts, int64_t* p_ts);
 void launch_insert_unclaim(hipStream_t s, int64_t m, const unsigned long long* fail, const unsigned long long* fail_sig,
                            int64_t E0, int64_t cap, int C, const InsertIn& in, const InsertState& st);
diff --git a/babble_amd/csrc/hgx_kernels.hip b/babble_amd/csrc/hgx_kernels.hip
--- a/babble_amd/csrc/hgx_kernels.hip
+++ b/babble_amd/csrc/hgx_kernels.hip
@@ -19,7 +19,8 @@
 
 __global__ void __launch_bounds__(256) k_ck_pack(int64_t E0, int64_t E, const int32_t* __restrict__ g_creator,
                                                  const int32_t* __restrict__ g_index, const int32_t* __restrict__ c_base,
-                                                 int64_t* __restrict__ g_ck) {
+                                                 int64_t* __restrict__ g_ck, const int32_t* __restrict__ gate) {
+    if (gate && *gate) return;
     const int64_t gid = E0 + (int64_t)blockIdx.x * blockDim.x + threadIdx.x;
     if (gid >= E) return;
     const int c = g_creator[gid];
@@ -66,7 +67,8 @@
                                                        int32_t* __restrict__ p_op, int32_t* __restrict__ p_opu,
                                                        int32_t* __restrict__ p_opk, int64_t* __restrict__ p_ts,
                                                        int32_t* __restrict__ p_rr, int64_t* __restrict__ p_cts, int C,
-                                                       int n, int seg) {
+                                                       int n, int seg, const int32_t* __restrict__ gate) {
+    if (gate && *gate) return;
     const int64_t gid = E0 + (int64_t)blockIdx.x * blockDim.x + threadIdx.x;
     if (gid >= E) return;
     const int c = g_creator[gid];
@@ -87,8 +89,10 @@
                                                        int32_t* __restrict__ p_chain, int32_t* __restrict__ p_op,
                                                        int32_t* __restrict__ p_opu, int32_t* __restrict__ p_opk,
                                                        int64_t* __restrict__ p_ts, int32_t* __restrict__ p_rr,
-                                                       int64_t* __restrict__ p_cts, int C, int n, int seg) {
+                                                       int64_t* __restrict__ p_cts, int C, int n, int seg,
+                                                       const int32_t* __restrict__ gate) {
     constexpr int B = kLayoutB2, PT = B / 256;
+    if (gate && *gate) return;
     __shared__ int32_t s_cnt[kLayoutH], s_min[kLayoutH];
     __shared__ int32_t s_slot[B];
     __shared__ int32_t s_cr[B], s_ix[B];
@@ -1998,19 +2002,19 @@
     hipLaunchKernelGGL(k_copy_many, dim3(bx, std::min(count, kCopyMax)), dim3(256), 0, s, f);
 }
 
-void launch_layout(hipStream_t s, int64_t E0, int64_t E, const DevArrays& a, int C, int n, int seg) {
+void launch_layout(hipStream_t s, int64_t E0, int64_t E, const DevArrays& a, int C, int n, int seg, const int32_t* gate) {
     if (E <= E0) return;
     hipLaunchKernelGGL(k_ck_pack, dim3(nblk(E - E0, 256)), dim3(256), 0, s, E0, E, a.g_creator, a.g_index, a.c_base,
-                       a.g_ck);
+                       a.g_ck, gate);
     if (E - E0 <= 8 * kLayoutB) {
         hipLaunchKernelGGL(k_layout_direct, dim3(nblk(E - E0, 256)), dim3(256), 0, s, E0, E, a.g_creator, a.g_index,
                            a.g_ck, a.g_op, a.g_ts, a.g_rr, a.g_cts, a.c_off, a.c_base, a.g_pos, a.p_gid, a.p_chain, a.p_op,
-                           a.p_opu, a.p_opk, a.p_ts, a.p_rr, a.p_cts, C, n, seg);
+                           a.p_opu, a.p_opk, a.p_ts, a.p_rr, a.p_cts, C, n, seg, gate);
         return;
     }
     hipLaunchKernelGGL(k_layout_staged, dim3(nblk(E - E0, kLayoutB2)), dim3(256), 0, s, E0, E, a.g_creator, a.g_index,
                        a.g_ck, a.g_op, a.g_ts, a.g_rr, a.g_cts, a.c_off, a.c_base, a.g_pos, a.p_gid, a.p_chain, a.p_op,
-                       a.p_opu, a.p_opk, a.p_ts, a.p_rr, a.p_cts, C, n, seg);
+                       a.p_opu, a.p_opk, a.p_ts, a.p_rr, a.p_cts, C, n, seg, gate);
 }
 
 void launch_la_sweep(hipStream_t s, const DevArrays& a, int C, int n, int max_len, int seg, int first, int32_t* chg,
diff --git a/babble_amd/csrc/hgx_la_wave.hip b/babble_amd/csrc/hgx_la_wave.hip
--- a/babble_amd/csrc/hgx_la_wave.hip
+++ b/babble_amd/csrc/hgx_la_wave.hip
@@ -120,8 +120,11 @@
                                                   const int32_t* __restrict__ c_old,
                                                   const int32_t* __restrict__ p_gid, int64_t E, int nts, int head,
                                                   int n, int lgnp, int nwd, int nblk, int32_t* __restrict__ err,
-                                                  const int32_t* __restrict__ lmap, int na) {
+                                                  const int32_t* __restrict__ lmap, int na, int ts0,
+                                                  const int32_t* __restrict__ c_lim,
+                                                  const int32_t* __restrict__ gate) {
     typedef LaW<CT> W;
+    if (gate && *gate) return;
     extern __shared__ uint32_t smem[];
     const int NP = 1 << lgnp;
     uint32_t* ring_d = smem;
@@ -133,7 +136,7 @@
     int32_t* s_off = s_old + n;
     int32_t* s_len = s_off + n;
     int32_t* s_abort = s_len + n;
-    const int b = blockIdx.x % nblk, ts = (blockIdx.x / nblk) % nts, g = blockIdx.x / nblk / nts;
+    const int b = blockIdx.x % nblk, ts = ts0 + (blockIdx.x / nblk) % nts, g = blockIdx.x / nblk / nts;
     const int c0 = g * n;
     const int wb = b * DW;
     const int tid = threadIdx.x;
@@ -143,8 +146,9 @@
         int o = 0, e = len;
         if constexpr (MODE == 1) o = c_old[c0 + t];
         if constexpr (MODE >= 2) {
-            o = ts == 0 ? 0 : chain_lower_bound(p_gid, off, len, E * ts / nts);
-            e = ts == nts - 1 ? len : chain_lower_bound(p_gid, off, len, E * (ts + 1) / nts);
+            const int lim = c_lim ? c_lim[c0 + t] : len;
+            o = ts == 0 ? 0 : chain_lower_bound(p_gid, off, lim, E * ts / nts);
+            e = ts == nts - 1 ? lim : chain_lower_bound(p_gid, off, lim, E * (ts + 1) / nts);
             if constexpr (MODE == 3) e = ts == 0 ? o : min(e, o + head);
         }
         lqv[t] = o;
@@ -296,7 +300,7 @@
 namespace {
 template <typename CT, int DW, int R, int Q, int NLW, int J, int CH, int MODE>
 hipError_t la_wave_launch1(hipStream_t s, const DevArrays& a, int G, int n, const int32_t* c_old, int64_t E, int nts,
-                           int head, int32_t* err, const int32_t* lmap, int na) {
+                           int head, int32_t* err, const int32_t* lmap, int na, const LaSubset& sub = LaSubset()) {
     const int nwd = a.compact ? n / 2 : n;
     const int nblk = nwd / DW;
     int lgnp = 0;
@@ -310,8 +314,10 @@
     }
     const int threads = (((lmap ? na : n) + 63) & ~63) + 64 * NLW;
     if (threads > 1024 || (lmap && G != 1)) return hipErrorInvalidValue;
-    hipLaunchKernelGGL(kern, dim3(G * nts * nblk), dim3(threads), words * 4, s, (uint32_t*)a.LA, a.p_opk, a.c_off,
-                       a.c_len, a.c_base, c_old, a.p_gid, E, nts, head, n, lgnp, nwd, nblk, err, lmap, na);
+    const int nseg = sub.count > 0 ? sub.count : nts;
+    hipLaunchKernelGGL(kern, dim3(G * nseg * nblk), dim3(threads), words * 4, s, (uint32_t*)a.LA, a.p_opk, a.c_off,
+                       a.c_len, a.c_base, c_old, a.p_gid, E, nts, head, n, lgnp, nwd, nblk, err, lmap, na, sub.first,
+                       sub.c_lim, sub.gate);
     return hipGetLastError();
 }
 template <typename CT, int DW, int R, int Q, int NLW, int J, int CH>
@@ -331,14 +337,15 @@
 }
 template <typename CT>
 hipError_t la_wave_dispatch(hipStream_t s, const DevArrays& a, int G, int n, const int32_t* c_old, int64_t E, int nts,
-                            int head, int32_t* err, const int32_t* lmap, int na, bool narrow) {
+                            int head, int32_t* err, const int32_t* lmap, int na, bool narrow, const LaSubset& sub) {
     const int nwd = a.compact ? n / 2 : n;
     if (nts > 1) {
         const SegCfg g = seg_cfg(n, nwd);
 #define SEG(DW_, R_, Q_, NLW_, J_, CH_)                                                                                \
     return head > 0 ? la_wave_launch1<CT, DW_, R_, Q_, NLW_, J_, CH_, 3>(s, a, G, n, nullptr, E, nts, head, err, lmap, \
                                                                           na)                                          \
-                    : la_wave_launch1<CT, DW_, R_, Q_, NLW_, J_, CH_, 2>(s, a, G, n, nullptr, E, nts, 0, err, lmap, na)
+                    : la_wave_launch1<CT, DW_, R_, Q_, NLW_, J_, CH_, 2>(s, a, G, n, nullptr, E, nts, 0, err, lmap, na, \
+                                                                          sub)
         if (n <= 256) {
             if (g.dw == 16) SEG(16, 8, 16, 1, 4, 8);
             if (g.dw == 8) SEG(8, 8, 32, 1, 4, 8);
@@ -593,10 +600,12 @@
 }
 
 hipError_t launch_la_wave(hipStream_t s, const DevArrays& a, int G, int n, const int32_t* c_old, int64_t E, int nts,
-                          int head, int32_t* err, const int32_t* lmap, int na, bool narrow) {
+                          int head, int32_t* err, const int32_t* lmap, int na, bool narrow, const LaSubset& sub) {
     if (nts > 1 && (G != 1 || c_old)) return hipErrorInvalidValue;
-    return a.compact ? la_wave_dispatch<uint16_t>(s, a, G, n, c_old, E, nts, head, err, lmap, na, narrow)
-                     : la_wave_dispatch<int32_t>(s, a, G, n, c_old, E, nts, head, err, lmap, na, narrow);
-}
-
-}
+    if (sub.count > 0 && (nts < 2 || head > 0 || sub.first < 0 || sub.first + sub.count > nts || !sub.c_lim))
+        return hipErrorInvalidValue;
+    return a.compact ? la_wave_dispatch<uint16_t>(s, a, G, n, c_old, E, nts, head, err, lmap, na, narrow, sub)
+                     : la_wave_dispatch<int32_t>(s, a, G, n, c_old, E, nts, head, err, lmap, na, narrow, sub);
+}
+
+}
diff --git a/babble_amd/hashgraph.py b/babble_amd/hashgraph.py
--- a/babble_amd/hashgraph.py
+++ b/babble_amd/hashgraph.py
@@ -746,8 +746,8 @@
                     pending_loaded=self.PendingLoadedEvents(graph), blocks=self.Blocks(graph))
 
     def phase_times(self):
-        out = np.zeros(22, np.float64)
-        self.L.hgx_phase_times(self.ctx, ptr(out), 22)
+        out = np.zeros(23, np.float64)
+        self.L.hgx_phase_times(self.ctx, ptr(out), 23)
         return dict(coords_ms=out[0], rounds_ms=out[1], fame_ms=out[2], order_ms=out[3],
                     la_sweeps=int(out[4]), rounds=int(out[5]), compact=int(out[6]),
                     la_rows=int(out[7]), rebuild=int(out[8]), r_lo=int(out[9]),
@@ -755,7 +755,11 @@
                     round_p_runs=int(out[13]), round_p_fallbacks=int(out[14]), round_p_ovf=int(out[15]),
                     round_p_fail_round=int(out[16]), round_p_fail_chain=int(out[17]),
                     round_g_runs=int(out[18]), la_small=int(out[19]), la_verify=int(out[20]),
-                    sort_seg=int(out[21]))
+                    sort_seg=int(out[21]), ingest_pieces=int(out[22]))
+
+    def set_ingest_pipeline(self, pieces, min_events=4_000_000):
+        if self.L.hgx_set_ingest_pipeline(self.ctx, int(pieces), int(min_events)) != 0:
+            raise ValueError(f"invalid ingest pipeline {pieces}, {min_events}")
 
     def set_fame_tally(self, mode):
         m = {"popc": 0, "vote": 1, "mfma": 2}[mode] if isinstance(mode, str) else int(mode)
diff --git a/include/hgx.h b/include/hgx.h
--- a/include/hgx.h
+++ b/include/hgx.h
@@ -271,6 +271,7 @@
 
 int32_t hgx_set_coord_storage(hgx_ctx* ctx, int32_t mode);
 int32_t hgx_set_fame_tally(hgx_ctx* ctx, int32_t mode);
+int32_t hgx_set_ingest_pipeline(hgx_ctx* ctx, int32_t pieces, int64_t min_events);
 int32_t hgx_set_la_kernel(hgx_ctx* ctx, int32_t mode);
 int32_t hgx_set_round_kernel(hgx_ctx* ctx, int32_t mode);
 int32_t hgx_set_sort_kernel(hgx_ctx* ctx, int32_t mode);
```

Result: faster. 253.1 million (median of 6 runs) (+1.7%).
